# Sun-Sir/BSARec

Measured on AMD Instinct MI355X. Metric: train sequences/sec, ML-1M L=50 d=64 2-layer, higher is better.
Workload: dtype f32

## Files before the change

bsarec_amd/_lib.py:

```python
import ctypes as C
import os

HERE = os.path.dirname(os.path.abspath(__file__))
LIB_PATH = os.environ.get("BSAREC_LIB") or os.path.join(HERE, "libbsarec_hip.so")
MAX_LAYERS = 16
ABI_VERSION = 10
TOPK_MAX = 1024
NEG_MAX = 1024
NEG_MAX_DRAWS = 1 << 20
TRAIN_NEG_MAX = 8192
TRAIN_NEG_SITE = 0x4E454753

(BUF_LAYER_OUT, BUF_LOGITS, BUF_LOSS, BUF_DSP, BUF_HMIX, BUF_PROBS, BUF_DLAYER_IN, BUF_LOSS_ROWS, BUF_CTX,
 BUF_DLOGITS, BUF_TRAIN_CAND, BUF_TRAIN_CORR, BUF_TRAIN_LOGITS, BUF_TRAIN_DLOGITS) = range(14)
K_NONE, K_FFN1, K_FFN2, K_QKV, K_LOGITS, K_DU, K_DW1, K_FUSED_FWD, K_FUSED_BWD = range(9)

LAYER_FIELDS = ["sqrt_beta", "filter_ln_w", "filter_ln_b", "query_w", "query_b", "key_w", "key_b", "value_w", "value_b",
                "dense_w", "dense_b", "attn_ln_w", "attn_ln_b", "ffn1_w", "ffn1_b", "ffn2_w", "ffn2_b", "ffn_ln_w",
                "ffn_ln_b"]
LAYER_KEYS = {
    "sqrt_beta": "layer.filter_layer.sqrt_beta",
    "filter_ln_w": "layer.filter_layer.LayerNorm.weight", "filter_ln_b": "layer.filter_layer.LayerNorm.bias",
    "query_w": "layer.attention_layer.query.weight", "query_b": "layer.attention_layer.query.bias",
    "key_w": "layer.attention_layer.key.weight", "key_b": "layer.attention_layer.key.bias",
    "value_w": "layer.attention_layer.value.weight", "value_b": "layer.attention_layer.value.bias",
    "dense_w": "layer.attention_layer.dense.weight", "dense_b": "layer.attention_layer.dense.bias",
    "attn_ln_w": "layer.attention_layer.LayerNorm.weight", "attn_ln_b": "layer.attention_layer.LayerNorm.bias",
    "ffn1_w": "feed_forward.dense_1.weight", "ffn1_b": "feed_forward.dense_1.bias",
    "ffn2_w": "feed_forward.dense_2.weight", "ffn2_b": "feed_forward.dense_2.bias",
    "ffn_ln_w": "feed_forward.LayerNorm.weight", "ffn_ln_b": "feed_forward.LayerNorm.bias",
}
OPTIONAL_LAYER_KEYS = {"filter_cw": "layer.filter_layer.complex_weight"}
TOP_KEYS = {"item_emb": "item_embeddings.weight", "pos_emb": "position_embeddings.weight",
            "ln_w": "LayerNorm.weight", "ln_b": "LayerNorm.bias"}


class Config(C.Structure):
    _fields_ = [("batch", C.c_int), ("seq_len", C.c_int), ("hidden", C.c_int), ("heads", C.c_int), ("layers", C.c_int),
                ("item_size", C.c_int), ("cutoff_bins", C.c_int), ("alpha", C.c_float), ("ln_eps", C.c_float),
                ("p_hidden", C.c_float), ("p_attn", C.c_float), ("filter_kind", C.c_int),
                ("hidden_act", C.c_int), ("storage", C.c_int), ("no_fused", C.c_int), ("no_prune_top", C.c_int),
                ("dw_tiled", C.c_int), ("splits", C.c_int), ("top_slabs", C.c_int), ("separate_embed", C.c_int),
                ("separate_top", C.c_int), ("chain_kernels", C.c_int), ("x3_products", C.c_int),
                ("train_negatives", C.c_int), ("train_sampler", C.c_int), ("train_no_logq", C.c_int),
                ("train_lazy_adam", C.c_int),
                ("weight_image", C.c_int)]


TRAIN_FIELDS = ("train_negatives", "train_sampler", "train_no_logq")
TRAIN_SAMPLERS = {"uniform": 0, "popularity": 1}


OPTION_FIELDS = ("storage", "no_fused", "no_prune_top", "dw_tiled", "splits", "top_slabs", "separate_embed", "separate_top", "chain_kernels", "x3_products",
                 "weight_image")
HIDDEN_ACTS = {"gelu": 0, "relu": 1, "swish": 2, "tanh": 3, "sigmoid": 4}

_defaults = {k: 0 for k in OPTION_FIELDS}
_defaults["weight_image"] = 1


def _env_defaults():
    e = os.environ
    d = {}
    if e.get("BSAREC_DW") == "tiled":
        d["dw_tiled"] = 1
    if e.get("BSAREC_PRUNE_TOP") == "0":
        d["no_prune_top"] = 1
    if e.get("BSAREC_EMBED_IN_BLOCK") == "0":
        d["separate_embed"] = 1
    if e.get("BSAREC_TOP_TAIL") == "0":
        d["separate_top"] = 1
    if e.get("BSAREC_FUSED") == "0":
        d["no_fused"] = 1
    if e.get("BSAREC_BLOCK_KERNELS") == "chain":
        d["chain_kernels"] = 1
    if e.get("BSAREC_PRODUCTS") == "bf16x3":
        d["x3_products"] = 1
    for env, key, hi in (("BSAREC_TOP_SLABS", "top_slabs", 16), ("BSAREC_SPLITS", "splits", 1024)):
        if e.get(env, "").isdigit() and 1 <= int(e[env]) <= hi:
            d[key] = int(e[env])
    if e.get("BSAREC_STORAGE") == "bf16":
        d["storage"] = 1
    if e.get("BSAREC_WEIGHT_IMAGE") == "0":
        d["weight_image"] = 0
    return d


def set_default_options(**kw):
    old = {}
    for k, v in kw.items():
        if k not in _defaults:
            raise KeyError(k)
        old[k] = _defaults[k]
        _defaults[k] = int(v)
    return old


def default_options():
    d = dict(_defaults)
    d.update(_env_defaults())
    return d


class Layer(C.Structure):
    _fields_ = [(f, C.c_void_p) for f in LAYER_FIELDS] + [("filter_cw", C.c_void_p)]


class Tensors(C.Structure):
    _fields_ = [("item_emb", C.c_void_p), ("pos_emb", C.c_void_p), ("ln_w", C.c_void_p), ("ln_b", C.c_void_p),
                ("layer", Layer * MAX_LAYERS)]


class Adam(C.Structure):
    _fields_ = [("params", C.c_void_p), ("grads", C.c_void_p), ("exp_avg", C.c_void_p), ("exp_avg_sq", C.c_void_p),
                ("n", C.c_long), ("lr", C.c_float), ("beta1", C.c_float), ("beta2", C.c_float), ("eps", C.c_float),
                ("weight_decay", C.c_float), ("grad_scale", C.c_float), ("shadow_bf16", C.c_void_p), ("shadow_from", C.c_long),
                ("grads2", C.c_void_p), ("grads2_n", C.c_long), ("n_grad_srcs", C.c_int), ("grad_srcs", C.c_void_p * 8),
                ("wimage_plan", C.c_void_p)]


class Comm(C.Structure):
    _fields_ = [("rank", C.c_int), ("world", C.c_int), ("flags", C.c_void_p * 8), ("epoch", C.c_void_p),
                ("error", C.c_void_p), ("timeout_ms", C.c_int)]


HOOK = C.CFUNCTYPE(None, C.c_void_p, C.c_void_p)


EXPORTS = {
    "bsarec_abi_version": (C.c_int, []),
    "bsarec_workspace_bytes": (C.c_size_t, [C.POINTER(Config)]),
    "bsarec_plan_create": (C.c_int, [C.POINTER(C.c_void_p), C.POINTER(Config), C.POINTER(Tensors), C.POINTER(Tensors),
                                     C.POINTER(Tensors), C.c_void_p, C.c_size_t, C.c_void_p, C.c_void_p, C.c_void_p]),
    "bsarec_shadow_refresh": (C.c_int, [C.c_void_p, C.c_void_p]),
    "bsarec_wimage_refresh": (C.c_int, [C.c_void_p, C.c_void_p]),
    "bsarec_wimage_floats": (C.c_long, [C.POINTER(Config)]),
    "bsarec_wimage_offset": (C.c_long, [C.c_int] * 5),
    "bsarec_plan_set_dense_grad_hook": (C.c_int, [C.c_void_p, HOOK, C.c_void_p, C.c_void_p]),
    "bsarec_plan_set_train_sampler": (C.c_int, [C.c_void_p, C.c_void_p]),
    "bsarec_buffer_is_bf16": (C.c_int, [C.c_void_p, C.c_int, C.c_int]),
    "bsarec_plan_is_fused": (C.c_int, [C.c_void_p]),
    "bsarec_config_is_fused": (C.c_int, [C.c_void_p]),
    "bsarec_plan_destroy": (None, [C.c_void_p]),
    "bsarec_buffer_offset": (C.c_long, [C.c_void_p, C.c_int, C.c_int]),
    "bsarec_step_begin": (C.c_int, [C.c_void_p, C.c_void_p]),
    "bsarec_forward": (C.c_int, [C.c_void_p, C.c_void_p, C.c_int, C.c_void_p]),
    "bsarec_forward_last": (C.c_int, [C.c_void_p, C.c_void_p, C.c_int, C.c_void_p]),
    "bsarec_loss": (C.c_int, [C.c_void_p, C.c_void_p, C.c_void_p]),
    "bsarec_loss_bce": (C.c_int, [C.c_void_p, C.c_void_p, C.c_void_p, C.c_void_p]),
    "bsarec_loss_logsig": (C.c_int, [C.c_void_p, C.c_void_p, C.c_void_p, C.c_void_p]),
    "bsarec_logits": (C.c_int, [C.c_void_p, C.c_void_p]),
    "bsarec_backward": (C.c_int, [C.c_void_p, C.c_void_p]),
    "bsarec_backward_seq": (C.c_int, [C.c_void_p, C.c_void_p, C.c_void_p]),
    "bsarec_backward_seq_multi": (C.c_int, [C.c_void_p, C.c_void_p, C.c_void_p]),
    "bsarec_adam_step": (C.c_int, [C.POINTER(Adam), C.c_void_p, C.c_void_p]),
    "bsarec_train_step": (C.c_int, [C.c_void_p, C.c_void_p, C.c_void_p, C.POINTER(Adam), C.c_void_p]),
    "bsarec_gather_batch": (C.c_int, [C.c_void_p, C.c_void_p, C.c_void_p, C.c_long, C.c_void_p, C.c_int, C.c_int,
                                      C.c_void_p, C.c_void_p, C.c_void_p]),
    "bsarec_train_step_indexed": (C.c_int, [C.c_void_p] * 4 + [C.c_long] + [C.c_void_p] * 3 + [C.POINTER(Adam), C.c_void_p]),
    "bsarec_grad_step_indexed": (C.c_int, [C.c_void_p] * 4 + [C.c_long] + [C.c_void_p] * 3 + [C.c_float] * 3 + [C.c_void_p]),
    "bsarec_adam_apply": (C.c_int, [C.POINTER(Adam), C.c_void_p, C.c_void_p]),
    "bsarec_mask_seen": (C.c_int, [C.c_void_p, C.c_long, C.c_int, C.c_void_p, C.c_void_p, C.c_void_p, C.c_void_p]),
    "bsarec_topk_seen": (C.c_int, [C.c_void_p, C.c_long, C.c_int, C.c_int, C.c_void_p, C.c_void_p, C.c_void_p, C.c_int, C.c_void_p,
                                   C.c_void_p, C.c_void_p]),
    "bsarec_sampled_rank": (C.c_int, [C.c_void_p, C.c_long, C.c_void_p, C.c_int, C.c_int, C.c_int] + [C.c_void_p] * 5 +
                            [C.c_int, C.c_uint64, C.c_uint32] + [C.c_void_p] * 4),
    "bsarec_topk_full_workspace_bytes": (C.c_long, [C.c_int] * 5),
    "bsarec_topk_full": (C.c_int, [C.c_void_p, C.c_long, C.c_void_p, C.c_int, C.c_int, C.c_int] + [C.c_void_p] * 3 +
                         [C.c_int, C.c_int, C.c_void_p, C.c_long, C.c_void_p, C.c_void_p, C.c_void_p]),
    "bsarec_topk_full_range": (C.c_int, [C.c_void_p, C.c_long, C.c_void_p, C.c_int, C.c_int, C.c_long, C.c_int] + [C.c_void_p] * 3 +
                               [C.c_int, C.c_int, C.c_void_p, C.c_long, C.c_void_p, C.c_void_p, C.c_void_p]),
    "bsarec_answer_rank": (C.c_int, [C.c_void_p, C.c_long, C.c_void_p, C.c_int, C.c_int, C.c_int] + [C.c_void_p] * 7),
    "bsarec_answer_rank_range": (C.c_int, [C.c_void_p, C.c_long, C.c_void_p, C.c_int, C.c_int, C.c_long, C.c_int] +
                                 [C.c_void_p] * 8),
    "bsarec_answer_score_range": (C.c_int, [C.c_void_p, C.c_long, C.c_void_p, C.c_int, C.c_int, C.c_long, C.c_int] +
                                  [C.c_void_p] * 6),
    "bsarec_info_nce_workspace_bytes": (C.c_long, [C.c_int] * 3),
    "bsarec_info_nce_fwd": (C.c_int, [C.c_void_p, C.c_long, C.c_void_p, C.c_long, C.c_int, C.c_int, C.c_float, C.c_int,
                                      C.c_void_p, C.c_void_p, C.c_void_p, C.c_long, C.c_void_p]),
    "bsarec_info_nce_bwd": (C.c_int, [C.c_void_p, C.c_long, C.c_void_p, C.c_long, C.c_int, C.c_int, C.c_float, C.c_int,
                                      C.c_void_p, C.c_void_p, C.c_long, C.c_void_p, C.c_void_p, C.c_void_p]),
    "bsarec_freq_layer_fwd": (C.c_int, [C.c_void_p] * 5 + [C.c_int] * 4 + [C.c_float, C.c_float, C.c_void_p, C.c_int,
                                                                          C.c_void_p, C.c_void_p, C.c_void_p, C.c_void_p]),
    "bsarec_freq_layer_bwd_scratch_floats": (C.c_long, [C.c_int, C.c_int, C.c_int]),
    "bsarec_freq_layer_bwd": (C.c_int, [C.c_void_p] * 7 + [C.c_int] * 4 + [C.c_float, C.c_void_p, C.c_int] +
                              [C.c_void_p] * 6),
    "bsarec_profile_select": (C.c_int, [C.c_void_p, C.c_int]),
    "bsarec_debug_stamps": (C.c_int, [C.c_void_p, C.c_void_p]),
    "bsarec_profile_read": (C.c_int, [C.c_void_p, C.POINTER(C.c_double), C.POINTER(C.c_int)]),
    "bsarec_profile_event_overhead": (C.c_int, [C.c_void_p, C.c_int, C.POINTER(C.c_double)]),
}

COMM_EXPORTS = {
    "bsarec_comm_alloc": (C.c_int, [C.POINTER(C.c_void_p), C.c_size_t, C.c_int]),
    "bsarec_comm_free": (C.c_int, [C.c_void_p]),
    "bsarec_comm_export": (C.c_int, [C.c_void_p, C.c_char_p]),
    "bsarec_comm_import": (C.c_int, [C.c_char_p, C.POINTER(C.c_void_p)]),
    "bsarec_comm_release": (C.c_int, [C.c_void_p]),
    "bsarec_comm_barrier": (C.c_int, [C.POINTER(Comm), C.c_void_p]),
}

PTRS8 = C.c_void_p * 8
SHARD_EXPORTS = {
    "bsarec_shard_gather_rows": (C.c_int, [C.c_void_p, C.c_long, C.POINTER(PTRS8), C.c_int, C.c_long, C.c_long, C.c_int,
                                           C.c_void_p, C.c_void_p, C.c_void_p]),
    "bsarec_shard_logits": (C.c_int, [C.c_void_p, C.c_long, C.c_int, C.c_void_p, C.c_int, C.c_int, C.c_void_p, C.c_long,
                                      C.c_void_p]),
    "bsarec_shard_ce_stats": (C.c_int, [C.c_void_p, C.c_long, C.c_int, C.c_int, C.c_void_p, C.c_long, C.c_long, C.c_void_p,
                                        C.c_void_p]),
    "bsarec_shard_ce_grad": (C.c_int, [C.c_void_p, C.c_long, C.c_int, C.c_int, C.c_void_p, C.c_long, C.c_long, C.c_void_p,
                                       C.c_int, C.c_void_p, C.c_void_p, C.c_void_p]),
    "bsarec_shard_head_bwd_scratch_floats": (C.c_long, [C.c_int, C.c_int, C.c_int]),
    "bsarec_shard_head_bwd": (C.c_int, [C.c_void_p, C.c_long, C.c_int, C.c_int, C.c_void_p, C.c_long, C.c_void_p, C.c_int,
                                        C.c_void_p, C.c_void_p, C.c_void_p, C.c_void_p]),
    "bsarec_shard_scatter_rows": (C.c_int, [C.c_void_p, C.c_long, C.c_int, C.POINTER(PTRS8), C.c_long, C.c_long, C.c_long,
                                            C.c_int, C.c_void_p, C.c_void_p]),
    "bsarec_shard_ssm_draw": (C.c_int, [C.c_uint64, C.c_void_p, C.c_int, C.c_long, C.c_void_p, C.c_int, C.c_void_p, C.c_void_p,
                                        C.c_void_p, C.c_void_p]),
    "bsarec_shard_ssm_gather": (C.c_int, [C.c_void_p, C.c_int, C.c_void_p, C.c_int, C.POINTER(PTRS8), C.c_int, C.c_long, C.c_long,
                                          C.c_int, C.c_void_p, C.c_void_p]),
    "bsarec_shard_ssm_head": (C.c_int, [C.c_void_p, C.c_long, C.c_int, C.c_int, C.c_void_p, C.c_void_p, C.c_void_p, C.c_void_p,
                                        C.c_int, C.c_long, C.c_void_p, C.c_int, C.c_int, C.c_void_p, C.c_void_p, C.c_void_p,
                                        C.c_void_p]),
    "bsarec_shard_ssm_loss": (C.c_int, [C.c_void_p, C.c_int, C.c_void_p, C.c_void_p]),
    "bsarec_shard_ssm_bwd_scratch_floats": (C.c_long, [C.c_int, C.c_int, C.c_int]),
    "bsarec_shard_ssm_bwd": (C.c_int, [C.c_void_p, C.c_int, C.c_int, C.c_void_p, C.c_long, C.c_void_p, C.c_int, C.c_void_p,
                                       C.c_long, C.c_void_p, C.c_void_p, C.c_void_p]),
    "bsarec_shard_ssm_pull": (C.c_int, [C.c_void_p, C.c_int, C.c_int, C.c_void_p, C.c_int, C.POINTER(PTRS8), C.c_long, C.c_long,
                                        C.c_long, C.c_int, C.c_void_p, C.c_void_p]),
    "bsarec_shard_lazy_mark": (C.c_int, [C.c_void_p, C.c_long, C.c_void_p, C.c_int, C.c_void_p, C.c_int, C.c_long, C.c_long,
                                         C.c_long, C.c_void_p, C.c_void_p, C.c_void_p, C.c_int, C.c_void_p]),
    "bsarec_shard_lazy_adam": (C.c_int, [C.c_void_p, C.c_void_p, C.c_void_p, C.c_void_p, C.c_int, C.c_float, C.c_float, C.c_float,
                                         C.c_float, C.c_void_p, C.c_void_p, C.c_void_p, C.c_int, C.c_void_p, C.c_void_p]),
}

_lib = None


def source_sha16() -> str:
    import hashlib
    h = hashlib.sha256()
    src = os.path.join(HERE, "csrc")
    for f in sorted(os.listdir(src)) + [os.path.join(os.path.dirname(HERE), "include", "bsarec_hip.h"),
                                         os.path.join(HERE, "build.py")]:
        with open(f if os.path.isabs(f) else os.path.join(src, f), "rb") as fh:
            h.update(fh.read())
    return h.hexdigest()[:16]


def load():
    global _lib
    if _lib is not None:
        return _lib
    if not os.path.exists(LIB_PATH):
        raise RuntimeError(
            f"{LIB_PATH} is missing: build it with `python -m bsarec_amd.build` (hipcc, gfx950). "
            "bsarec_amd has no fallback path.")
    lib = C.CDLL(LIB_PATH)
    for name, (res, args) in list(EXPORTS.items()) + list(COMM_EXPORTS.items()) + list(SHARD_EXPORTS.items()):
        fn = getattr(lib, name)
        fn.restype = res
        fn.argtypes = args
    if lib.bsarec_abi_version() != ABI_VERSION:
        raise RuntimeError("libbsarec_hip.so ABI version mismatch: rebuild with `python -m bsarec_amd.build --force`")
    _lib = lib
    return lib


def check(rc, what):
    if rc != 0:
        kind = "invalid argument / unsupported shape" if rc < 0 else "hipError_t"
        raise RuntimeError(f"{what} failed: {kind} {rc}")
```

bsarec_amd/csrc/bsarec_hip.hip:

```cpp
#include <cmath>
#include "../../include/bsarec_hip.h"
#include "../../include/bsarec_shard.h"
#include "epilogues.h"
#include "kernels.h"
#include "fused_layer.h"
#include "dw_direct.h"
#include "fused_top.h"
#include "fused_chain.h"
#include "comm.h"
#include "catalogue_shard.h"
#include "rank.h"
#include "sampled_rank.h"
#include "full_rank.h"
#include "answer_rank.h"
#include "info_nce.h"
#include "sampled_softmax.h"
#include "lazy_adam.h"

#include <hip/hip_runtime.h>
#include <math.h>
#include <stdio.h>
#include <stdlib.h>
#include <string.h>
#include <vector>
#include <algorithm>

#define HIPCHK(x) do { hipError_t e_ = (x); if (e_ != hipSuccess) return (int)e_; } while (0)
#define RET(x) do { int r_ = (x); if (r_ != 0) return r_; } while (0)

static thread_local bool g_dry = false;
#define LAUNCH(...) do { if (!g_dry) hipLaunchKernelGGL(__VA_ARGS__); } while (0)

struct bsarec_plan;
static thread_local bsarec_plan* t_plan = nullptr;

static inline int cdiv(long a, long b) { return (int)((a + b - 1) / b); }
static inline long rup(long a, long b) { return (a + b - 1) / b * b; }

struct ProfState {
    int kclass = BSAREC_K_NONE;
    std::vector<std::pair<hipEvent_t, hipEvent_t>> events;
    size_t used = 0;
    ~ProfState() { for (auto& e : events) { (void)hipEventDestroy(e.first); (void)hipEventDestroy(e.second); } }
};

struct LayerBufs {
    float *dsp, *xhat_f, *rstd_f, *q, *k, *v, *probs, *ctx, *xhat_a, *rstd_a, *hmix, *u, *xhat_ff, *rstd_ff;
    float* gp;
};

struct bsarec_plan {
    bsarec_config_t cfg;
    bsarec_tensors_t P, G, S;
    bool bf;
    bool bf_products;
    char* ws; size_t ws_bytes;
    uint64_t* state;
    const float* twiddle;
    int T, Lp, Vp, dh, nblk, rows_pb, nsplit, kchunk, vsplit, vchunk;
    bool fused;
    bool train;
    int* ids32;
    float* X[BSAREC_MAX_LAYERS + 1];
    float *xhat0, *rstd0;
    LayerBufs lb[BSAREC_MAX_LAYERS];
    float *logits, *dlogits, *loss_rows, *loss;
    float *dXa, *dXb, *dz, *dT, *dU, *dH, *dXacc, *dO, *dF, *dC, *dS, *dq, *dk, *dv, *dXtmp, *dlast_slab;
    float *slab_wL[BSAREC_MAX_LAYERS], *slab_bL[BSAREC_MAX_LAYERS], *part_lnL[BSAREC_MAX_LAYERS], *part_betaL[BSAREC_MAX_LAYERS];
    float *part_ln0, *part_pos, *trash;
    int pos_slices;
    ReduceJob* jobs; int jobs_per_layer;
    ReduceJob* jobs_pruned;
    bool prune_ok;
    bool pruned;
    int loss_kind;
    const float* ext_dy = nullptr;
    const float* ext_mid[BSAREC_MAX_LAYERS] = {};
    const int64_t *bce_pos, *bce_neg;
    float *part_kvb, *slab_dummy;
    float* part_cwL[BSAREC_MAX_LAYERS];
    float *top_dq, *top_dO, *top_dT, *top_dU, *top_ak, *top_rk, *top_av, *top_rv;
    int* blockmap; int red_blocks;
    long red_elems; const float *red_lo, *red_hi;
    int top_slabs; bool embed_in_block, direct_dw;
    bool scatter_in_block;
    ProfState prof;
    long long* stamps = nullptr;
    bsarec_hook_t dense_hook = nullptr; void* dense_hook_user = nullptr;
    float* lookup_grad = nullptr;
    unsigned long long* lookup_acc = nullptr;
    int* ssm_cand = nullptr; float *ssm_corr = nullptr, *ssm_logits = nullptr, *ssm_dlogits = nullptr;
    const int64_t* pop_cum = nullptr;
    const int64_t* ssm_answers = nullptr;
    int ssm_nslab = 0;
    LazyRows lazy = {};
    bool lazy_now = false;
    float* wimg = nullptr;
};
struct PlanScope {
    bsarec_plan* prev;
    explicit PlanScope(bsarec_plan* p) : prev(t_plan) { t_plan = p; }
    ~PlanScope() { t_plan = prev; }
};

struct ProfScope {
    hipStream_t s; bool on; hipEvent_t stop;
    ProfScope(int kclass, hipStream_t st) : s(st), on(false) {
        ProfState* ps = t_plan ? &t_plan->prof : nullptr;
        on = ps && kclass != BSAREC_K_NONE && kclass == ps->kclass;
        if (!on) return;
        if (ps->used == ps->events.size()) {
            hipEvent_t a, b;
            (void)hipEventCreate(&a); (void)hipEventCreate(&b);
            ps->events.push_back({a, b});
        }
        (void)hipEventRecord(ps->events[ps->used].first, s);
        stop = ps->events[ps->used].second;
        ++ps->used;
    }
    ~ProfScope() { if (on) (void)hipEventRecord(stop, s); }
};

template <auto Kernel, class... A>
static int launch_lds(dim3 grid, dim3 block, size_t smem, hipStream_t s, const A&... a) {
    static size_t raised = 0;
    if (smem > 48 * 1024 && smem > raised) {
        HIPCHK(hipFuncSetAttribute(reinterpret_cast<const void*>(Kernel), hipFuncAttributeMaxDynamicSharedMemorySize, (int)smem));
        raised = smem;
    }
    if (g_dry) return 0;
    hipLaunchKernelGGL(Kernel, grid, block, smem, s, a...);
    return (int)hipGetLastError();
}

static GemmP gemm_defaults(int M, int N, int K) {
    GemmP P;
    memset(&P, 0, sizeof(P));
    P.M = M; P.N = N; P.K = K; P.Nb = N; P.Kv = K;
    P.nseg = 1; P.nprob = 1; P.nsplit = 1; P.kchunk = K; P.nh = 1;
    return P;
}

template <int BM, int BN, int WM, int WN, bool AKM, bool BKM, int AXF, int BXF, bool BG, bool BF, class Epi>
static int launch_gemm_as(const GemmP& P, const XformP& X, const Epi& epi, float* bgrad, int nbatch, hipStream_t s, int kclass) {
    if (P.M <= 0 || P.N <= 0) return 0;
    const dim3 grid(cdiv(P.M, BM), cdiv(P.N, BN), nbatch * P.nprob * P.nsplit);
    ProfScope prof(g_dry ? BSAREC_K_NONE : kclass, s);
    return launch_lds<gemm_kernel<BM, BN, WM, WN, AKM, BKM, AXF, BXF, BG, BF, Epi>>(grid, dim3(64 * WM * WN),
                                                                                  GemmSmem<BM, BN, AKM, BKM, BF>::BYTES, s, P, X, epi, bgrad);
}

template <int BM, int BN, int WM, int WN, bool AKM, bool BKM, int AXF, int BXF, bool BG, class Epi>
static int launch_gemm(const GemmP& P, const XformP& X, const Epi& epi, float* bgrad, int nbatch, hipStream_t s,
                       int kclass = BSAREC_K_NONE, bool fp32_only = false) {
    if (!fp32_only && t_plan && t_plan->bf_products) {
        if constexpr (BM == 64 && BN == 64 && !BG)
            if (P.M >= 8192 && P.N >= 128 && nbatch == 1)
                return launch_gemm_as<128, 128, WM, WN, AKM, BKM, AXF, BXF, BG, true, Epi>(P, X, epi, bgrad, nbatch, s, kclass);
        return launch_gemm_as<BM, BN, WM, WN, AKM, BKM, AXF, BXF, BG, true, Epi>(P, X, epi, bgrad, nbatch, s, kclass);
    }
    if constexpr (BN == 256 && WM * WN == 4)
        return launch_gemm_as<BM, BN, 2, 4, AKM, BKM, AXF, BXF, BG, false, Epi>(P, X, epi, bgrad, nbatch, s, kclass);
    else
        return launch_gemm_as<BM, BN, WM, WN, AKM, BKM, AXF, BXF, BG, false, Epi>(P, X, epi, bgrad, nbatch, s, kclass);
}

static XformP no_xform() { XformP X; memset(&X, 0, sizeof(X)); return X; }

template <bool BIAS, bool ADD, bool GGRAD>
static EpiLinear<BIAS, ADD, GGRAD> epi_linear(float* C, long ldc) {
    EpiLinear<BIAS, ADD, GGRAD> e;
    memset(&e, 0, sizeof(e));
    e.C[0] = C; e.ldc = ldc;
    return e;
}

struct Carver {
    char* base; size_t off;
    explicit Carver(char* b) : base(b), off(0) {}
    template <class T> T* take(size_t n) {
        T* p = base ? reinterpret_cast<T*>(base + off) : nullptr;
        off += rup((long)(n * sizeof(T)), 256);
        return p;
    }
};

static int check_cfg(const bsarec_config_t& c) {
    if (c.batch < 1 || c.seq_len < 1 || c.seq_len > 256) return -1;
    if (c.hidden < 4 || c.hidden > 256 || c.hidden % 4) return -2;
    if (c.heads < 1 || c.hidden % c.heads || (c.hidden / c.heads) % 4) return -3;
    if (c.layers < 1 || c.layers > BSAREC_MAX_LAYERS) return -4;
    if (c.item_size < 2) return -5;
    if (c.cutoff_bins < 1 || c.cutoff_bins > c.seq_len / 2 + 1) return -6;
    if ((long)c.cutoff_bins * c.hidden > 8192) return -7;
    if (c.p_hidden < 0.f || c.p_hidden >= 1.f || c.p_attn < 0.f || c.p_attn >= 1.f) return -8;
    if (c.filter_kind != 0 && c.filter_kind != 1) return -9;
    if (c.filter_kind == 1 && c.cutoff_bins != c.seq_len / 2 + 1) return -9;
    if (c.hidden_act < 0 || c.hidden_act > 4) return -14;
    if (c.storage < 0 || c.storage > 1) return -15;
    if (c.splits < 0 || c.splits > 1024 || c.top_slabs < 0 || c.top_slabs > 16) return -16;
    if (c.train_negatives < 0 || c.train_negatives > BSAREC_TRAIN_NEG_MAX) return -17;
    if (c.train_sampler < 0 || c.train_sampler > 1 || c.train_no_logq < 0 || c.train_no_logq > 1) return -17;
    if (c.train_negatives > 0 && c.storage != 0) return -18;
    if (c.train_lazy_adam < 0 || c.train_lazy_adam > 1 || (c.train_lazy_adam && c.train_negatives == 0)) return -19;
    if (c.weight_image < 0 || c.weight_image > 1) return -20;
    return 0;
}

static bool fused_shape_ok(const bsarec_config_t& c);
static bool wimage_wanted(const bsarec_config_t& c) {
    return c.weight_image && fused_shape_ok(c) && c.storage == 0 && !c.x3_products && !c.chain_kernels && c.filter_kind == 0;
}

static bool fused_shape_ok(const bsarec_config_t& c) {
    const int dh = c.hidden / c.heads;
    if (c.no_fused || c.hidden_act != 0 || c.hidden != 64 || c.seq_len > 64 || !(dh == 16 || dh == 32 || dh == 64)) return false;
    if (c.filter_kind == 1) return c.storage == 0 && c.alpha == 1.0f && c.cutoff_bins <= 36;
    return c.cutoff_bins <= FUSED_MAX_CB;
}

#define SSM_SLAB_MAX 32
static void ssm_split(int N, int cap, int* nslab, int* chunk) {
    const int want = std::max(1, std::min(cap, N / 256));
    *chunk = (int)rup(cdiv(N, want), SSM_KS);
    *nslab = cdiv(N, *chunk);
}

static void derive(bsarec_plan& p) {
    const bsarec_config_t& c = p.cfg;
    p.fused = fused_shape_ok(c);
    p.bf = c.storage == 1 && p.fused;
    p.bf_products = c.storage == 1 && !p.fused;
    p.T = c.batch * c.seq_len;
    p.Lp = (int)rup(c.seq_len, 4);
    p.Vp = (int)rup(c.item_size, 4);
    p.dh = c.hidden / c.heads;
    p.nblk = p.fused ? c.batch : cdiv(p.T, 64);
    p.rows_pb = p.fused ? c.seq_len : 64;
    const int want_splits = c.splits > 0 ? c.splits : (p.fused ? 32 : 40);
    p.top_slabs = c.top_slabs > 0 ? c.top_slabs : 2;
    p.embed_in_block = !c.separate_embed || p.bf;
    p.direct_dw = !c.dw_tiled && (long)p.T * 4 * c.hidden * 4 < (1L << 31);
    p.scatter_in_block = p.fused && p.direct_dw && !c.separate_embed;
    long ch = rup(cdiv(p.T, want_splits), p.bf ? 2 * GEMM_BK : GEMM_BK);
    if (ch < 64) ch = 64;
    if (ch > 2048) ch = 2048;
    p.kchunk = (int)ch;
    p.nsplit = cdiv(p.T, p.kchunk);
    long vc = rup(cdiv(p.Vp, p.fused ? 32 : 16), GEMM_BK);
    if (vc < 64) vc = 64;
    p.vchunk = (int)vc;
    p.vsplit = cdiv(p.Vp, p.vchunk);
    int chunk;
    if (c.train_negatives > 0) ssm_split(c.train_negatives, std::min(p.vsplit, SSM_SLAB_MAX), &p.ssm_nslab, &chunk);
}

static void carve(bsarec_plan& p, char* base, size_t* total) {
    const bsarec_config_t& c = p.cfg;
    const long T = p.T, d = c.hidden, B = c.batch, L = c.seq_len, h = c.heads, N = c.layers;
    const long Td = T * d;
    Carver cv(base);
    p.jobs = cv.take<ReduceJob>((size_t)(N * 20 + 3));
    p.jobs_pruned = cv.take<ReduceJob>((size_t)(N * 20 + 3));
    p.blockmap = cv.take<int>((size_t)(N * (12 * cdiv(d * d, 64) + 16 * cdiv(4 * d, 64) + cdiv((long)c.cutoff_bins * d * 2, 64)) +
                                       cdiv(L * d, 64) + 2 * cdiv(d, 64) + 64));
    p.ids32 = cv.take<int>(T);
    for (int l = 0; l <= N; ++l) p.X[l] = cv.take<float>(Td);
    p.xhat0 = cv.take<float>(Td); p.rstd0 = cv.take<float>(T);
    for (int l = 0; l < N; ++l) {
        LayerBufs& b = p.lb[l];
        b.dsp = cv.take<float>(Td); b.xhat_f = cv.take<float>(Td); b.rstd_f = cv.take<float>(T);
        b.q = cv.take<float>(Td); b.k = cv.take<float>(Td); b.v = cv.take<float>(Td);
        b.probs = cv.take<float>(B * h * L * p.Lp); b.ctx = cv.take<float>(Td);
        b.xhat_a = cv.take<float>(Td); b.rstd_a = cv.take<float>(T); b.hmix = cv.take<float>(Td);
        b.u = cv.take<float>(4 * Td); b.xhat_ff = cv.take<float>(Td); b.rstd_ff = cv.take<float>(T);
        b.gp = p.fused ? cv.take<float>(4 * Td) : nullptr;
    }
    p.logits = cv.take<float>(B * p.Vp); p.dlogits = cv.take<float>(B * p.Vp);
    p.loss_rows = cv.take<float>(B); p.loss = cv.take<float>(4);
    p.dXa = cv.take<float>(Td); p.dXb = cv.take<float>(Td); p.dz = cv.take<float>(Td); p.dT = cv.take<float>(Td);
    p.dU = cv.take<float>(4 * Td); p.dH = cv.take<float>(Td); p.dXacc = cv.take<float>(Td); p.dO = cv.take<float>(Td);
    p.dF = cv.take<float>(Td); p.dC = cv.take<float>(Td); p.dS = cv.take<float>(B * h * L * p.Lp);
    p.dq = cv.take<float>(Td); p.dk = cv.take<float>(Td); p.dv = cv.take<float>(Td); p.dXtmp = cv.take<float>(Td);
    p.dlast_slab = cv.take<float>((long)p.vsplit * B * d);
    for (int l = 0; l < N; ++l) {
        p.slab_wL[l] = cv.take<float>((long)p.nsplit * 12 * d * d);
        p.slab_bL[l] = cv.take<float>((long)p.nsplit * 9 * d);
        p.part_lnL[l] = cv.take<float>((long)p.nblk * 6 * d);
        p.part_betaL[l] = cv.take<float>(B * d);
    }
    p.part_ln0 = cv.take<float>((long)p.nblk * 2 * d);
    p.pos_slices = cdiv(B, 64);
    p.part_pos = cv.take<float>((long)p.pos_slices * L * d);
    p.trash = cv.take<float>(1024);
    p.lookup_acc = cv.take<unsigned long long>((long)c.item_size * d);
    p.part_kvb = cv.take<float>(2 * B * d);
    for (int l = 0; l < N; ++l) p.part_cwL[l] = c.filter_kind == 1 ? cv.take<float>(B * c.cutoff_bins * d * 2) : nullptr;
    p.top_dq = cv.take<float>(B * d); p.top_dO = cv.take<float>(B * d); p.top_dT = cv.take<float>(B * d);
    p.top_dU = cv.take<float>(4 * B * d);
    p.top_ak = cv.take<float>(B * h * d); p.top_rk = cv.take<float>(B * h * d);
    p.top_av = cv.take<float>(B * h * d); p.top_rv = cv.take<float>(B * h * d);
    p.slab_dummy = cv.take<float>((long)p.nsplit * 4 * d);
    if (c.train_negatives > 0) {
        const long Nn = c.train_negatives;
        p.ssm_cand = cv.take<int>(Nn); p.ssm_corr = cv.take<float>(Nn);
        p.ssm_logits = cv.take<float>(B * (Nn + 1)); p.ssm_dlogits = cv.take<float>(B * (Nn + 1));
    }
    if (c.train_lazy_adam) {
        p.lazy.cap = (int)std::min<long>(c.item_size, T + B + c.train_negatives);
        p.lazy.d4 = (int)(d / 4);
        p.lazy.mark = cv.take<int>(c.item_size); p.lazy.rows = cv.take<int>(p.lazy.cap); p.lazy.count = cv.take<int>(1);
    }
    *total = cv.off;
}

extern "C" int bsarec_abi_version(void) { return BSAREC_ABI_VERSION; }

extern "C" size_t bsarec_workspace_bytes(const bsarec_config_t* cfg) {
    if (!cfg || check_cfg(*cfg) != 0) return 0;
    bsarec_plan p;
    p.cfg = *cfg;
    derive(p);
    size_t total = 0;
    carve(p, nullptr, &total);
    return total;
}

struct SlabMap { long wq, wk, wv, wo, w1, w2, wtot, bq, bk, bv, bo, b1, b2, btot; };
static SlabMap slab_map(long d) {
    SlabMap m;
    m.wq = 0; m.wk = d * d; m.wv = 2 * d * d; m.wo = 3 * d * d; m.w1 = 4 * d * d; m.w2 = 8 * d * d; m.wtot = 12 * d * d;
    m.bq = 0; m.bk = d; m.bv = 2 * d; m.bo = 3 * d; m.b1 = 4 * d; m.b2 = 8 * d; m.btot = 9 * d;
    return m;
}

static float* slab_w_ptr(const bsarec_plan& p, int l, long tensor_off) { return p.slab_wL[l] + tensor_off * p.nsplit; }
static float* slab_b_ptr(const bsarec_plan& p, int l, long tensor_off) { return p.slab_bL[l] + tensor_off * p.nsplit; }

enum LnPart { LN_FF_G, LN_FF_B, LN_A_G, LN_A_B, LN_F_G, LN_F_B };
enum Ln0Part { LN_E_G, LN_E_B };
static float* ln_part(const bsarec_plan& p, int l, LnPart k) { return p.part_lnL[l] + (long)k * p.nblk * p.cfg.hidden; }
static float* ln0_part(const bsarec_plan& p, Ln0Part k) { return p.part_ln0 + (long)k * p.nblk * p.cfg.hidden; }

static const float* h_last(const bsarec_plan& p) { return p.X[p.cfg.layers] + (long)(p.cfg.seq_len - 1) * p.cfg.hidden; }
static long h_last_stride(const bsarec_plan& p) { return (long)p.cfg.seq_len * p.cfg.hidden; }

static float* wimage_weight(const bsarec_plan& p, int l, int which, bool transposed) {
    const long d = p.cfg.hidden;
    return p.wimg + l * wimage_layer_floats(d) + (transposed ? 12 * d * d : 0) + wimage_weight_off(which, d);
}
static bsarec_layer_t wimage_layer(const bsarec_plan& p, int l, bool transposed) {
    bsarec_layer_t w;
    memset(&w, 0, sizeof(w));
    w.query_w = wimage_weight(p, l, WIMAGE_WQ, transposed); w.key_w = wimage_weight(p, l, WIMAGE_WK, transposed);
    w.value_w = wimage_weight(p, l, WIMAGE_WV, transposed); w.dense_w = wimage_weight(p, l, WIMAGE_WO, transposed);
    w.ffn1_w = wimage_weight(p, l, WIMAGE_W1, transposed); w.ffn2_w = wimage_weight(p, l, WIMAGE_W2, transposed);
    return w;
}

extern "C" int bsarec_plan_create(bsarec_plan_t** out, const bsarec_config_t* cfg, const bsarec_tensors_t* params,
                                  const bsarec_tensors_t* grads, const bsarec_tensors_t* shadow, void* workspace,
                                  size_t workspace_bytes, void* state, const float* twiddle, void* stream) {
    if (!out || !cfg || !params || !workspace || !state || !twiddle) return -10;
    RET(check_cfg(*cfg));
    if (cfg->storage == 1 && fused_shape_ok(*cfg) && !shadow) return -15;
    if (wimage_wanted(*cfg) && (!shadow || !shadow->layer[0].query_w || ((uintptr_t)shadow->layer[0].query_w & 255))) return -15;
    if (((uintptr_t)workspace & 255) != 0) return -11;
    bsarec_plan* p = new bsarec_plan();
    p->cfg = *cfg;
    p->P = *params;
    if (grads) p->G = *grads; else memset(&p->G, 0, sizeof(p->G));
    if (shadow) p->S = *shadow; else memset(&p->S, 0, sizeof(p->S));
    p->ws = (char*)workspace; p->ws_bytes = workspace_bytes;
    p->state = (uint64_t*)state; p->twiddle = twiddle; p->train = false;
    p->wimg = wimage_wanted(*cfg) ? shadow->layer[0].query_w : nullptr;
    derive(*p);
    size_t total = 0;
    carve(*p, p->ws, &total);
    if (total > workspace_bytes) { delete p; return -12; }
    if (hipMemset(p->lookup_acc, 0, (size_t)cfg->item_size * cfg->hidden * sizeof(unsigned long long)) != hipSuccess) {
        delete p; return -12;
    }
    if (cfg->train_lazy_adam && (hipMemset(p->lazy.mark, 0, (size_t)cfg->item_size * sizeof(int)) != hipSuccess ||
                                 hipMemset(p->lazy.count, 0, sizeof(int)) != hipSuccess)) {
        delete p; return -12;
    }

    const long d = cfg->hidden;
    const SlabMap sm = slab_map(d);
    std::vector<ReduceJob> jobs;
    auto add = [&](const float* src, float* dst, int nsplit, long len) {
        ReduceJob j; j.src = src; j.dst = dst; j.nsplit = nsplit; j.len = (int)len; j.stride = len; j.scale = 1.f; j.pad = 0;
        jobs.push_back(j);
    };
    const int ns = p->nsplit, nb = p->nblk;
    auto add_w = [&](int l, int which, const float* src, float* dst) {
        add(src, dst, ns, (which >= WIMAGE_W1 ? 4 : 1) * d * d);
        if (!p->wimg) return;
        ReduceJob& j = jobs.back();
        j.img_f = wimage_weight(*p, l, which, false); j.img_t = wimage_weight(*p, l, which, true);
        j.wn = (int)(which == WIMAGE_W1 ? 4 * d : d); j.wk = (int)(which == WIMAGE_W2 ? 4 * d : d);
    };
    for (int l = 0; l < cfg->layers; ++l) {
        const bsarec_layer_t& g = p->G.layer[l];
        add(p->part_betaL[l], g.sqrt_beta, cfg->batch, d);
        add(ln_part(*p, l, LN_F_G), g.filter_ln_w, nb, d);
        add(ln_part(*p, l, LN_F_B), g.filter_ln_b, nb, d);
        add_w(l, WIMAGE_WQ, slab_w_ptr(*p, l, sm.wq), g.query_w); add(slab_b_ptr(*p, l, sm.bq), g.query_b, ns, d);
        add_w(l, WIMAGE_WK, slab_w_ptr(*p, l, sm.wk), g.key_w);   add(slab_b_ptr(*p, l, sm.bk), g.key_b, ns, d);
        add_w(l, WIMAGE_WV, slab_w_ptr(*p, l, sm.wv), g.value_w); add(slab_b_ptr(*p, l, sm.bv), g.value_b, ns, d);
        add_w(l, WIMAGE_WO, slab_w_ptr(*p, l, sm.wo), g.dense_w); add(slab_b_ptr(*p, l, sm.bo), g.dense_b, ns, d);
        add(ln_part(*p, l, LN_A_G), g.attn_ln_w, nb, d);
        add(ln_part(*p, l, LN_A_B), g.attn_ln_b, nb, d);
        add_w(l, WIMAGE_W1, slab_w_ptr(*p, l, sm.w1), g.ffn1_w); add(slab_b_ptr(*p, l, sm.b1), g.ffn1_b, ns, 4 * d);
        add_w(l, WIMAGE_W2, slab_w_ptr(*p, l, sm.w2), g.ffn2_w); add(slab_b_ptr(*p, l, sm.b2), g.ffn2_b, ns, d);
        add(ln_part(*p, l, LN_FF_G), g.ffn_ln_w, nb, d);
        add(ln_part(*p, l, LN_FF_B), g.ffn_ln_b, nb, d);
    }
    add(ln0_part(*p, LN_E_G), p->G.ln_w, nb, d);
    add(ln0_part(*p, LN_E_B), p->G.ln_b, nb, d);
    if (p->scatter_in_block) {
        ReduceJob j; j.src = p->dz; j.dst = p->G.pos_emb; j.nsplit = cfg->batch; j.len = (int)((long)cfg->seq_len * d);
        j.stride = (long)cfg->seq_len * d; j.scale = 1.f; j.pad = 0;
        jobs.push_back(j);
    } else add(p->part_pos, p->G.pos_emb, p->pos_slices, (long)cfg->seq_len * d);
    if (cfg->filter_kind == 1)
        for (int l = 0; l < cfg->layers; ++l)
            add(p->part_cwL[l], p->G.layer[l].filter_cw, cfg->batch, (long)cfg->cutoff_bins * d * 2);
    p->jobs_per_layer = 19;
    p->prune_ok = p->fused && cfg->layers >= 2 && !cfg->no_prune_top && cfg->filter_kind == 0;
    p->pruned = false;
    p->loss_kind = 0; p->bce_pos = nullptr; p->bce_neg = nullptr;
    std::vector<ReduceJob> jobs_pr = jobs;
    {
        const size_t base = (size_t)(cfg->layers - 1) * 19;
        ReduceJob& jk = jobs_pr[base + 6]; jk.src = p->part_kvb; jk.nsplit = cfg->batch; jk.stride = d;
        ReduceJob& jv = jobs_pr[base + 8]; jv.src = p->part_kvb + (long)cfg->batch * d; jv.nsplit = cfg->batch; jv.stride = d;
        for (int j : {3, 4, 5, 7, 9, 10, 13, 14, 15, 16})
            jobs_pr[base + j].nsplit = std::min(p->top_slabs, ns);
    }
    std::vector<int> bmap;
    for (size_t j = 0; j < jobs.size(); ++j)
        for (int ch = 0; ch < cdiv(jobs[j].len, 64); ++ch) bmap.push_back((int)(j << 16) | ch);
    p->red_blocks = (int)bmap.size();
    p->red_elems = 0; p->red_lo = nullptr; p->red_hi = nullptr;
    for (const ReduceJob& j : jobs) {
        p->red_elems += j.len;
        if (!p->red_lo || j.dst < p->red_lo) p->red_lo = j.dst;
        if (!p->red_hi || j.dst + j.len > p->red_hi) p->red_hi = j.dst + j.len;
    }
    hipError_t e = hipMemcpyAsync(p->jobs, jobs.data(), jobs.size() * sizeof(ReduceJob), hipMemcpyHostToDevice,
                                  (hipStream_t)stream);
    if (e == hipSuccess) e = hipMemcpyAsync(p->blockmap, bmap.data(), bmap.size() * sizeof(int), hipMemcpyHostToDevice,
                                            (hipStream_t)stream);
    if (e == hipSuccess) e = hipMemcpyAsync(p->jobs_pruned, jobs_pr.data(), jobs_pr.size() * sizeof(ReduceJob),
                                            hipMemcpyHostToDevice, (hipStream_t)stream);
    if (e == hipSuccess) e = hipStreamSynchronize((hipStream_t)stream);
    if (e != hipSuccess) { delete p; return (int)e; }
    g_dry = true;
    int rc = 0;
    for (int last = 0; last < 2 && rc == 0; ++last) {
        rc = last ? bsarec_forward_last(p, reinterpret_cast<const int64_t*>(p->ws), 1, stream)
                  : bsarec_forward(p, reinterpret_cast<const int64_t*>(p->ws), 1, stream);
        if (rc == 0) rc = bsarec_loss(p, reinterpret_cast<const int64_t*>(p->ws), stream);
        if (rc == 0 && p->G.item_emb) rc = bsarec_backward(p, stream);
    }
    g_dry = false;
    p->pruned = false;
    p->train = false;
    if (rc != 0) { delete p; return rc; }
    *out = p;
    return 0;
}

extern "C" void bsarec_plan_destroy(bsarec_plan_t* plan) { delete plan; }

extern "C" long bsarec_buffer_offset(const bsarec_plan_t* p, int buffer, int layer) {
    if (!p) return -1;
    const int N = p->cfg.layers;
    const void* ptr = nullptr;
    if (buffer >= BSAREC_BUF_TRAIN_CAND && p->cfg.train_negatives == 0) return -1;
    switch (buffer) {
        case BSAREC_BUF_LAYER_OUT: if (layer < 0 || layer > N) return -1; ptr = p->X[layer]; break;
        case BSAREC_BUF_LOGITS: ptr = p->logits; break;
        case BSAREC_BUF_DLOGITS: ptr = p->dlogits; break;
        case BSAREC_BUF_LOSS: ptr = p->loss; break;
        case BSAREC_BUF_LOSS_ROWS: ptr = p->loss_rows; break;
        case BSAREC_BUF_DSP: if (layer < 0 || layer >= N) return -1; ptr = p->lb[layer].dsp; break;
        case BSAREC_BUF_HMIX: if (layer < 0 || layer >= N) return -1; ptr = p->lb[layer].hmix; break;
        case BSAREC_BUF_PROBS: if (layer < 0 || layer >= N) return -1; ptr = p->lb[layer].probs; break;
        case BSAREC_BUF_CTX: if (layer < 0 || layer >= N) return -1; ptr = p->lb[layer].ctx; break;
        case BSAREC_BUF_DLAYER_IN: if (layer < 0 || layer > N) return -1; ptr = (layer & 1) ? p->dXb : p->dXa; break;
        case BSAREC_BUF_TRAIN_CAND: ptr = p->ssm_cand; break;
        case BSAREC_BUF_TRAIN_CORR: ptr = p->ssm_corr; break;
        case BSAREC_BUF_TRAIN_LOGITS: ptr = p->ssm_logits; break;
        case BSAREC_BUF_TRAIN_DLOGITS: ptr = p->ssm_dlogits; break;
        default: return -1;
    }
    return (long)((const char*)ptr - p->ws);
}

extern "C" int bsarec_plan_set_dense_grad_hook(bsarec_plan_t* p, bsarec_hook_t hook, void* user, float* lookup_grad) {
    if (!p) return -10;
    if (p->cfg.train_negatives > 0 && (hook || lookup_grad)) return -22;
    p->dense_hook = hook; p->dense_hook_user = user; p->lookup_grad = lookup_grad;
    return 0;
}

extern "C" int bsarec_plan_set_train_sampler(bsarec_plan_t* p, const int64_t* pop_cum) {
    if (!p) return -10;
    if (p->cfg.train_negatives == 0 || p->cfg.train_sampler != 1) return -22;
    p->pop_cum = pop_cum;
    return 0;
}

static int sampled_refusal(const bsarec_plan& p) {
    if (p.cfg.train_negatives == 0) return 0;
    if (p.dense_hook || p.lookup_grad) return -22;
    if (p.cfg.train_sampler == 1 && !p.pop_cum && !g_dry) return -23;
    return 0;
}

static int head_nsplit(const bsarec_plan& p) { return p.loss_kind == 1 ? 1 : (p.loss_kind == 2 ? p.ssm_nslab : p.vsplit); }

extern "C" int bsarec_plan_is_fused(const bsarec_plan_t* p) { return p && p->fused ? 1 : 0; }
extern "C" int bsarec_config_is_fused(const bsarec_config_t* cfg) {
    if (!cfg) return -10;
    RET(check_cfg(*cfg));
    return fused_shape_ok(*cfg) ? 1 : 0;
}

extern "C" int bsarec_buffer_is_bf16(const bsarec_plan_t* p, int buffer, int layer) {
    if (!p || !p->bf) return 0;
    switch (buffer) {
        case BSAREC_BUF_LAYER_OUT: return layer < p->cfg.layers ? 1 : 0;
        case BSAREC_BUF_HMIX: case BSAREC_BUF_PROBS: case BSAREC_BUF_CTX: return 1;
        case BSAREC_BUF_DLAYER_IN: return 1;
        default: return 0;
    }
}

extern "C" int bsarec_wimage_refresh(bsarec_plan_t* p, void* stream) {
    if (!p) return -10;
    if (!p->wimg) return 0;
    WImageP W;
    memset(&W, 0, sizeof(W));
    for (int l = 0; l < p->cfg.layers; ++l) {
        const bsarec_layer_t& w = p->P.layer[l];
        const float* src[WIMAGE_NW] = {w.query_w, w.key_w, w.value_w, w.dense_w, w.ffn1_w, w.ffn2_w};
        for (int i = 0; i < WIMAGE_NW; ++i) W.w[l][i] = src[i];
    }
    W.img = p->wimg; W.d = p->cfg.hidden;
    LAUNCH(wimage_refresh_kernel, dim3(cdiv(12L * W.d * W.d, ROW_THREADS), p->cfg.layers), dim3(ROW_THREADS), 0, (hipStream_t)stream, W);
    return g_dry ? 0 : (int)hipGetLastError();
}

extern "C" long bsarec_wimage_floats(const bsarec_config_t* cfg) {
    if (!cfg || check_cfg(*cfg) != 0) return -10;
    return wimage_wanted(*cfg) ? cfg->layers * wimage_layer_floats(cfg->hidden) : 0;
}

extern "C" long bsarec_wimage_offset(int which, int transposed, int d, int n, int k) {
    if (which < 0 || which >= WIMAGE_NW || d < 32 || d % 32 || transposed < 0 || transposed > 1) return -1;
    const int wn = which == WIMAGE_W1 ? 4 * d : d, wk = which == WIMAGE_W2 ? 4 * d : d;
    if (n < 0 || n >= wn || k < 0 || k >= wk) return -1;
    return (transposed ? 12L * d * d : 0) + wimage_weight_off(which, d) + (transposed ? wimage_off(k, n, wn) : wimage_off(n, k, wk));
}

extern "C" int bsarec_shadow_refresh(bsarec_plan_t* p, void* stream) {
    if (!p) return -10;
    if (!p->bf) return 0;
    const long d = p->cfg.hidden;
    for (int l = 0; l < p->cfg.layers; ++l) {
        const bsarec_layer_t& w = p->P.layer[l];
        const bsarec_layer_t& sh = p->S.layer[l];
        CastJobs6 J;
        const float* src[6] = {w.query_w, w.key_w, w.value_w, w.dense_w, w.ffn1_w, w.ffn2_w};
        float* dst[6] = {sh.query_w, sh.key_w, sh.value_w, sh.dense_w, sh.ffn1_w, sh.ffn2_w};
        for (int i = 0; i < 6; ++i) { J.src[i] = src[i]; J.dst[i] = (unsigned short*)dst[i]; J.n4[i] = (i < 4 ? d * d : 4 * d * d) / 4; }
        hipLaunchKernelGGL(cast_bf16_kernel, dim3(cdiv(4 * d * d / 4, ROW_THREADS), 6), dim3(ROW_THREADS), 0, (hipStream_t)stream, J);
        HIPCHK(hipGetLastError());
    }
    return 0;
}

static uint32_t drop_thresh(float p) {
    double t = (double)p * 4294967296.0;
    if (t <= 0) return 0;
    if (t >= 4294967295.0) return 0xFFFFFFFFu;
    return (uint32_t)t;
}
static DropP make_drop(const bsarec_plan& p, float prob, int site, bool train) {
    DropP d;
    d.thresh = train ? drop_thresh(prob) : 0;
    d.scale = (train && prob > 0.f) ? (float)(1.0 / (1.0 - (double)prob)) : 1.0f;
    d.rng = p.state; d.site = (uint32_t)site;
    return d;
}
static int lpr_for(int d) { return d <= 64 ? 16 : (d <= 128 ? 32 : 64); }

#define DISPATCH_LPR(d, ...) \
    do { switch (lpr_for(d)) { case 16: { constexpr int LPR = 16; __VA_ARGS__; } break; \
                               case 32: { constexpr int LPR = 32; __VA_ARGS__; } break; \
                               default: { constexpr int LPR = 64; __VA_ARGS__; } break; } } while (0)

#define DISPATCH_BN(n, ...) \
    do { if ((n) <= 64) { constexpr int BN = 64; __VA_ARGS__; } \
         else if ((n) <= 128) { constexpr int BN = 128; __VA_ARGS__; } \
         else { constexpr int BN = 256; __VA_ARGS__; } } while (0)

static size_t freq_smem(int L, int d, int cb, int nsrc, int kc = FREQ_KC) {
    return (size_t)(rup(2 * L, 4) + (long)nsrc * cb * 2 * d + (long)nsrc * kc * 2048) * 4;
}
#define LDS_BYTES_MAX 163840

template <int LPR>
static int launch_freq_fwd(const float* X, const float* sb, const float* g, const float* be, float eps, DropP drop,
                           const float* tw, int B, int L, int d, int cb, float* dsp, float* xhat, float* rstd, hipStream_t s,
                           const float* cw = nullptr) {
    return launch_lds<freq_fwd_kernel<LPR>>(dim3(B), dim3(ROW_THREADS), freq_smem(L, d, cb, 1), s, X, sb, g, be, eps, drop, tw, L, d,
                                            cb, dsp, xhat, rstd, cw);
}

template <int LPR>
static int launch_freq_bwd(const float* X, const float* dF, const float* dXin, const float* sb, const float* tw, int B, int L,
                           int d, int cb, float* dX, float* pbeta, hipStream_t s, const float* cw = nullptr, float* pcw = nullptr) {
    if (freq_smem(L, d, cb, 2) > LDS_BYTES_MAX)
        return launch_lds<freq_bwd_kernel<LPR, 1>>(dim3(B), dim3(ROW_THREADS), freq_smem(L, d, cb, 2, 1), s, X, dF, dXin, sb, tw, L, d, cb,
                                                   dX, pbeta, cw, pcw);
    return launch_lds<freq_bwd_kernel<LPR>>(dim3(B), dim3(ROW_THREADS), freq_smem(L, d, cb, 2), s, X, dF, dXin, sb, tw, L, d, cb, dX,
                                            pbeta, cw, pcw);
}

static bool dw_problem_ok(const DwProblem& q) {
    if (!q.A || !q.B || !q.slab) return false;
    if (q.K < 1 || q.M < 1 || q.N < 1 || q.kchunk < 8 || (q.kchunk & 7) || q.nslab < 1) return false;
    if (q.lda < q.M || q.ldb < q.N) return false;
    const long esz = q.bf16 ? 2 : 4;
    if (((long)(q.K - 1) * q.lda + q.M) * esz >= (1L << 31) || ((long)(q.K - 1) * q.ldb + q.N) * esz >= (1L << 31)) return false;
    return true;
}
static bool dh_problem_ok(const DhP& h) {
    if (!h.A || !h.E || !h.slab) return false;
    if (h.B < 1 || h.V < 1 || h.kchunk < 8 || (h.kchunk & 7) || h.nsplit < 1 || h.lda < h.V) return false;
    if ((long)h.B * h.lda * 4 >= (1L << 31) || (long)h.V * 256 >= (1L << 31)) return false;
    return true;
}

#define DISPATCH_DH(dh, ...) \
    do { switch (dh) { case 16: { constexpr int DH = 16; __VA_ARGS__; } break; \
                       case 32: { constexpr int DH = 32; __VA_ARGS__; } break; \
                       default: { constexpr int DH = 64; __VA_ARGS__; } break; } } while (0)
#define DISPATCH_BLOCK(p, ...) \
    do { if ((p).bf) { constexpr bool BF = true, X3 = false; DISPATCH_DH((p).dh, __VA_ARGS__); } \
         else if ((p).cfg.x3_products) { constexpr bool BF = false, X3 = true; DISPATCH_DH((p).dh, __VA_ARGS__); } \
         else { constexpr bool BF = false, X3 = false; DISPATCH_DH((p).dh, __VA_ARGS__); } } while (0)

template <bool FWD, class BlockP>
static void fill_block(const bsarec_plan& p, int l, bool tr, const bsarec_layer_t& wm, BlockP& F) {
    const bsarec_config_t& c = p.cfg;
    const bsarec_layer_t& w = p.P.layer[l];
    const LayerBufs& b = p.lb[l];
    memset(&F, 0, sizeof(F));
    F.X = p.X[l];
    F.sqrt_beta = w.sqrt_beta; F.f_g = w.filter_ln_w; F.wq = wm.query_w; F.wk = wm.key_w; F.wv = wm.value_w; F.wo = wm.dense_w;
    F.a_g = w.attn_ln_w; F.w1 = wm.ffn1_w; F.w2 = wm.ffn2_w; F.ff_g = w.ffn_ln_w; F.tw = p.twiddle;
    F.xhat_f = b.xhat_f; F.rstd_f = b.rstd_f; F.q = b.q; F.k = b.k; F.v = b.v; F.probs = b.probs;
    F.xhat_a = b.xhat_a; F.rstd_a = b.rstd_a; F.xhat_ff = b.xhat_ff; F.rstd_ff = b.rstd_ff;
    F.L = c.seq_len; F.Lp = p.Lp; F.cb = c.cutoff_bins; F.heads = c.heads;
    F.alpha = c.alpha; F.oma = (float)(1.0 - (double)c.alpha);
    F.drop_f = make_drop(p, c.p_hidden, 1 + 4 * l, tr); F.drop_p = make_drop(p, c.p_attn, 2 + 4 * l, tr);
    F.drop_o = make_drop(p, c.p_hidden, 3 + 4 * l, tr); F.drop_ff = make_drop(p, c.p_hidden, 4 + 4 * l, tr);
    F.stamps = p.stamps ? p.stamps + 32 * (2 * l + (FWD ? 0 : 1)) : nullptr;
    if constexpr (FWD) {
        F.Xout = p.X[l + 1];
        F.f_b = w.filter_ln_b; F.bq = w.query_b; F.bk = w.key_b; F.bv = w.value_b; F.bo = w.dense_b; F.a_b = w.attn_ln_b;
        F.b1 = w.ffn1_b; F.b2 = w.ffn2_b; F.ff_b = w.ffn_ln_b;
        F.ids32 = p.ids32; F.ctx = b.ctx; F.hmix = b.hmix; F.u = b.u;
        F.eps = c.ln_eps;
    }
}

template <class BlockP>
static void fill_block_partials(const bsarec_plan& p, int l, BlockP& F) {
    F.pg_ff = ln_part(p, l, LN_FF_G); F.pb_ff = ln_part(p, l, LN_FF_B); F.pg_a = ln_part(p, l, LN_A_G);
    F.pb_a = ln_part(p, l, LN_A_B); F.pg_f = ln_part(p, l, LN_F_G); F.pb_f = ln_part(p, l, LN_F_B);
    F.pbeta = p.part_betaL[l];
}

static void fill_top_fwd(bsarec_plan& p, int l, bool tr, TopFwdP& F) {
    fill_block<true>(p, l, tr, p.P.layer[l], F);
    F.low = p.lb[l].dsp;
    F.wk_sh = p.S.layer[l].key_w; F.wv_sh = p.S.layer[l].value_w;
}

static int launch_fused_fwd(bsarec_plan& p, int l, bool tr, hipStream_t s, const int64_t* ids = nullptr, const GatherP* gp = nullptr,
                            bool top_tail = false ) {
    const bsarec_config_t& c = p.cfg;
    FusedFwdP F;
    fill_block<true>(p, l, tr, p.bf ? p.S.layer[l] : p.wimg ? wimage_layer(p, l, false) : p.P.layer[l], F);
    F.xout_f32 = (l == c.layers - 1);
    F.gp = p.lb[l].gp;
    F.dsp = nullptr;
    if (l == 0 && gp) {
        F.e_E = p.P.item_emb; F.e_pos = p.P.pos_emb; F.e_g = p.P.ln_w; F.e_b = p.P.ln_b; F.e_ids = ids; F.e_gp = *gp;
        F.e_drop = make_drop(p, c.p_hidden, 0, tr); F.e_V = c.item_size;
        F.e_X0 = p.X[0]; F.e_xhat = p.xhat0; F.e_rstd = p.rstd0; F.e_ids32 = p.ids32;
    }
    F.trash = p.trash;
    TopFwdP TF;
    if (top_tail) {
        fill_top_fwd(p, l + 1, tr, TF);
        if (p.wimg) { TF.wk_sh = wimage_weight(p, l + 1, WIMAGE_WK, false); TF.wv_sh = wimage_weight(p, l + 1, WIMAGE_WV, false); }
    }
    const dim3 grid(c.batch), block(512);
    ProfScope prof(BSAREC_K_FUSED_FWD, s);
    if (c.filter_kind == 1) {
        F.filter_cw = p.P.layer[l].filter_cw;
        return launch_lds<fused_layer_fwd_kernel<32, false, NoTail, false, true>>(grid, block, fused_fwd_smem_bytes(), s, F, NoTail());
    }
    int rc = 0;
    if (!p.bf && c.chain_kernels && !c.x3_products) {
        const size_t csm = fused_chain_fwd_smem_bytes(top_tail);
        DISPATCH_DH(p.dh, rc = top_tail ? launch_lds<fused_chain_fwd_kernel<DH, TopFwdP>>(grid, block, csm, s, F, TF)
                                        : launch_lds<fused_chain_fwd_kernel<DH, NoTail>>(grid, block, csm, s, F, NoTail()));
        return rc;
    }
    const size_t smem = fused_fwd_smem_bytes();
    if (p.wimg) {
        DISPATCH_DH(p.dh, rc = top_tail ? launch_lds<fused_layer_fwd_kernel<DH, false, TopFwdP, false, false, true>>(grid, block, smem, s, F, TF)
                                        : launch_lds<fused_layer_fwd_kernel<DH, false, NoTail, false, false, true>>(grid, block, smem, s, F, NoTail()));
        return rc;
    }
    DISPATCH_BLOCK(p, rc = top_tail ? launch_lds<fused_layer_fwd_kernel<DH, BF, TopFwdP, X3>>(grid, block, smem, s, F, TF)
                                    : launch_lds<fused_layer_fwd_kernel<DH, BF, NoTail, X3>>(grid, block, smem, s, F, NoTail()));
    return rc;
}

static int launch_fused_bwd(bsarec_plan& p, int l, bool tr, const float* dY, float* dXout, hipStream_t s, bool top,
                            const TopBwdP* head = nullptr ) {
    const bsarec_config_t& c = p.cfg;
    FusedBwdP F;
    fill_block<false>(p, l, tr, p.bf ? p.S.layer[l] : p.wimg ? wimage_layer(p, l, true) : p.P.layer[l], F);
    fill_block_partials(p, l, F);
    F.dY = dY; F.dX = dXout;
    F.u = p.lb[l].gp;
    if (top) { F.dh_slabs = p.dlast_slab; F.dh_nsplit = head_nsplit(p); F.dh_stride = (long)c.batch * c.hidden; }
    if (l == 0) {
        F.e_dz = p.dz; F.e_xhat = p.xhat0; F.e_rstd = p.rstd0; F.e_g = p.P.ln_w;
        F.e_pg = ln0_part(p, LN_E_G); F.e_pb = ln0_part(p, LN_E_B); F.e_drop = make_drop(p, c.p_hidden, 0, tr);
        F.e_dx_extra = p.ext_dy ? p.ext_mid[0] : nullptr;
    }
    F.dT = p.dT; F.dU = p.dU; F.dO = p.dO; F.dq = p.dq; F.dk = p.dk; F.dv = p.dv;
    F.trash = p.trash;
    const dim3 grid(c.batch), block(512);
    const size_t smem = fused_bwd_smem_bytes();
    ProfScope prof(BSAREC_K_FUSED_BWD, s);
    if (c.filter_kind == 1) {
        F.filter_cw = p.P.layer[l].filter_cw; F.pcw = p.part_cwL[l];
        return launch_lds<fused_layer_bwd_kernel<32, false, NoTail, false, true>>(grid, block, smem, s, F, NoTail());
    }
    int rc = 0;
    if (p.wimg) {
        DISPATCH_DH(p.dh, rc = head ? launch_lds<fused_layer_bwd_kernel<DH, false, TopBwdP, false, false, true>>(grid, block, smem, s, F, *head)
                                    : launch_lds<fused_layer_bwd_kernel<DH, false, NoTail, false, false, true>>(grid, block, smem, s, F, NoTail()));
        return rc;
    }
    DISPATCH_BLOCK(p, rc = head ? launch_lds<fused_layer_bwd_kernel<DH, BF, TopBwdP, X3>>(grid, block, smem, s, F, *head)
                                : launch_lds<fused_layer_bwd_kernel<DH, BF, NoTail, X3>>(grid, block, smem, s, F, NoTail()));
    return rc;
}

static int launch_top_fwd(bsarec_plan& p, int l, bool tr, hipStream_t s) {
    TopFwdP F;
    fill_top_fwd(p, l, tr, F);
    int rc = 0;
    DISPATCH_BLOCK(p, rc = launch_lds<top_fwd_kernel<DH, BF>>(dim3(p.cfg.batch), dim3(256), top_fwd_smem_bytes(), s, F));
    return rc;
}

static void fill_top_bwd(bsarec_plan& p, int l, bool tr, float* dXout, TopBwdP& F) {
    const bsarec_config_t& c = p.cfg;
    fill_block<false>(p, l, tr, p.P.layer[l], F);
    fill_block_partials(p, l, F);
    F.dX = dXout;
    F.u = p.lb[l].u; F.low = p.lb[l].dsp;
    F.dh_slabs = p.dlast_slab; F.dh_nsplit = head_nsplit(p); F.dh_stride = (long)c.batch * c.hidden;
    F.dT = p.top_dT; F.dU = p.top_dU; F.dO = p.top_dO; F.dq = p.top_dq;
    F.ak = p.top_ak; F.rk = p.top_rk; F.av = p.top_av; F.rv = p.top_rv;
    F.pbk = p.part_kvb; F.pbv = p.part_kvb + (long)c.batch * c.hidden;
}

static int launch_top_bwd(bsarec_plan& p, int l, bool tr, float* dXout, hipStream_t s) {
    TopBwdP F;
    fill_top_bwd(p, l, tr, dXout, F);
    int rc = 0;
    DISPATCH_BLOCK(p, rc = launch_lds<top_bwd_kernel<DH, BF>>(dim3(p.cfg.batch), dim3(256), top_bwd_smem_bytes(), s, F));
    return rc;
}

extern "C" int bsarec_debug_stamps(bsarec_plan_t* p, void* dev_buf) { if (!p) return -10; p->stamps = (long long*)dev_buf; return 0; }

#ifdef BSAREC_DW_STAMPS
extern "C" int bsarec_debug_dw_stamps(long long* host_out, int n) {
    if (!host_out || n < 1 || n > DW_STAMP_MAX) return -10;
    HIPCHK(hipDeviceSynchronize());
    HIPCHK(hipMemcpyFromSymbol(host_out, HIP_SYMBOL(g_dw_stamps), (size_t)n * 8 * sizeof(long long)));
    return 0;
}
#endif

extern "C" int bsarec_step_begin(bsarec_plan_t* p, void* stream) {
    if (!p) return -10;
    LAUNCH(step_begin_kernel, dim3(1), dim3(1), 0, (hipStream_t)stream, p->state, (long long*)nullptr, 0);
    return (int)hipGetLastError();
}

static int forward_impl(bsarec_plan_t* p, const int64_t* ids, int train, void* stream, const GatherP& gp, bool last_only);

extern "C" int bsarec_forward(bsarec_plan_t* p, const int64_t* ids, int train, void* stream) {
    GatherP none;
    memset(&none, 0, sizeof(none));
    return forward_impl(p, ids, train, stream, none, false);
}

extern "C" int bsarec_forward_last(bsarec_plan_t* p, const int64_t* ids, int train, void* stream) {
    GatherP none;
    memset(&none, 0, sizeof(none));
    return forward_impl(p, ids, train, stream, none, true);
}

static int generic_layer_fwd(bsarec_plan& p, int l, bool tr, hipStream_t s) {
    const bsarec_config_t& c = p.cfg;
    const int T = p.T, d = c.hidden, L = c.seq_len, B = c.batch, h = c.heads, dh = p.dh, Lp = p.Lp;
    const bsarec_layer_t& w = p.P.layer[l];
    LayerBufs& b = p.lb[l];
    const float* X = p.X[l];
    const XformP nox = no_xform();
    DISPATCH_LPR(d, RET(launch_freq_fwd<LPR>(X, w.sqrt_beta, w.filter_ln_w, w.filter_ln_b, c.ln_eps,
                                             make_drop(p, c.p_hidden, 1 + 4 * l, tr), p.twiddle, B, L, d,
                                             c.cutoff_bins, b.dsp, b.xhat_f, b.rstd_f, s,
                                             c.filter_kind == 1 ? w.filter_cw : nullptr)));
    {
        GemmP g = gemm_defaults(T, d, d);
        g.nprob = 3; g.lda = d; g.ldb = d;
        g.A[0] = g.A[1] = g.A[2] = X;
        g.B[0] = w.query_w; g.B[1] = w.key_w; g.B[2] = w.value_w;
        auto e = epi_linear<true, false, false>(b.q, d);
        e.C[1] = b.k; e.C[2] = b.v;
        e.bias[0] = w.query_b; e.bias[1] = w.key_b; e.bias[2] = w.value_b;
        RET((launch_gemm<64, 64, 2, 2, false, false, XF_NONE, XF_NONE, false>(g, nox, e, nullptr, 1, s, BSAREC_K_QKV)));
    }
    {
        GemmP g = gemm_defaults(L, Lp, dh);
        g.Nb = L; g.lda = d; g.ldb = d; g.nh = h;
        g.A[0] = b.q; g.B[0] = b.k;
        g.a_sb = (long)L * d; g.a_sh = dh; g.b_sb = (long)L * d; g.b_sh = dh;
        EpiSoftmax e; e.ids = p.ids32; e.L = L; e.Lp = Lp; e.sqrt_dh = sqrtf((float)dh); e.P = b.probs;
        DISPATCH_BN(Lp, RET((launch_gemm<64, BN, 2, 2, false, false, XF_NONE, XF_NONE, false>(g, nox, e, nullptr, B * h, s))));
    }
    {
        GemmP g = gemm_defaults(L, dh, Lp);
        g.Kv = L; g.lda = Lp; g.ldb = d; g.nh = h;
        g.A[0] = b.probs; g.B[0] = b.v;
        g.a_sb = (long)h * L * Lp; g.a_sh = (long)L * Lp; g.b_sb = (long)L * d; g.b_sh = dh;
        XformP xf = nox; xf.drop = make_drop(p, c.p_attn, 2 + 4 * l, tr); xf.L = L; xf.Lp = Lp;
        auto e = epi_linear<false, false, false>(b.ctx, d);
        e.c_sb = (long)L * d; e.c_sh = dh;
        RET((launch_gemm<64, 64, 2, 2, false, true, XF_DROP, XF_NONE, false>(g, xf, e, nullptr, B * h, s)));
    }
    {
        GemmP g = gemm_defaults(T, d, d);
        g.lda = d; g.ldb = d; g.A[0] = b.ctx; g.B[0] = w.dense_w;
        EpiLN<true> e;
        e.bias = w.dense_b; e.R = X; e.drop = make_drop(p, c.p_hidden, 3 + 4 * l, tr);
        e.gamma = w.attn_ln_w; e.beta = w.attn_ln_b; e.eps = c.ln_eps;
        e.Y = b.hmix; e.xhat = b.xhat_a; e.rstd = b.rstd_a;
        e.dsp = b.dsp; e.alpha = c.alpha; e.oma = (float)(1.0 - (double)c.alpha);
        DISPATCH_BN(d, RET((launch_gemm<64, BN, 2, 2, false, false, XF_NONE, XF_NONE, false>(g, nox, e, nullptr, 1, s))));
    }
    {
        GemmP g = gemm_defaults(T, 4 * d, d);
        g.lda = d; g.ldb = d; g.A[0] = b.hmix; g.B[0] = w.ffn1_w;
        auto e = epi_linear<true, false, false>(b.u, 4 * d);
        e.bias[0] = w.ffn1_b;
        RET((launch_gemm<64, 64, 2, 2, false, false, XF_NONE, XF_NONE, false>(g, nox, e, nullptr, 1, s, BSAREC_K_FFN1)));
    }
    {
        GemmP g = gemm_defaults(T, d, 4 * d);
        g.lda = 4 * d; g.ldb = 4 * d; g.A[0] = b.u; g.B[0] = w.ffn2_w;
        EpiLN<false> e;
        e.bias = w.ffn2_b; e.R = b.hmix; e.drop = make_drop(p, c.p_hidden, 4 + 4 * l, tr);
        e.gamma = w.ffn_ln_w; e.beta = w.ffn_ln_b; e.eps = c.ln_eps;
        e.Y = p.X[l + 1]; e.xhat = b.xhat_ff; e.rstd = b.rstd_ff;
        e.dsp = nullptr; e.alpha = 0.f; e.oma = 1.f;
        XformP xa = nox; xa.act = c.hidden_act;
        DISPATCH_BN(d, RET((launch_gemm<64, BN, 2, 2, false, false, XF_GELU, XF_NONE, false>(g, xa, e, nullptr, 1, s, BSAREC_K_FFN2))));
    }
    return 0;
}

static int forward_impl(bsarec_plan_t* p, const int64_t* ids, int train, void* stream, const GatherP& gp, bool last_only) {
    if (!p || (!ids && !gp.table)) return -10;
    PlanScope scope(p);
    hipStream_t s = (hipStream_t)stream;
    const bsarec_config_t& c = p->cfg;
    const int T = p->T, d = c.hidden, L = c.seq_len;
    const bool tr = train != 0;
    p->train = tr;
    p->pruned = last_only && p->prune_ok;

    const bool embed_in_block = p->fused && p->embed_in_block;
    if (!embed_in_block)
    DISPATCH_LPR(d, {
        constexpr int RPB = ROW_THREADS / LPR;
        LAUNCH(embed_fwd_kernel<LPR>, dim3(cdiv(T, RPB)), dim3(ROW_THREADS), 0, s, ids, gp, p->P.item_emb,
                           p->P.pos_emb, p->P.ln_w, p->P.ln_b, c.ln_eps, make_drop(*p, c.p_hidden, 0, tr), T, L, d,
                           c.item_size, p->X[0], p->xhat0, p->rstd0, p->ids32);
        HIPCHK(hipGetLastError());
    });

    const bool tail = p->pruned && c.layers >= 2 && !c.separate_top;
    for (int l = 0; l < c.layers; ++l) {
        if (!p->fused) RET(generic_layer_fwd(*p, l, tr, s));
        else if (p->pruned && l == c.layers - 1) { if (!tail) RET(launch_top_fwd(*p, l, tr, s)); }
        else RET(launch_fused_fwd(*p, l, tr, s, ids, (l == 0 && embed_in_block) ? &gp : nullptr, tail && l == c.layers - 2));
    }
    return 0;
}

extern "C" int bsarec_logits(bsarec_plan_t* p, void* stream) {
    if (!p) return -10;
    PlanScope scope(p);
    hipStream_t s = (hipStream_t)stream;
    const bsarec_config_t& c = p->cfg;
    const int d = c.hidden;
    if (p->fused && d == 64 && p->Vp <= 4096 && c.batch <= 512 && !g_dry) {
        LogitsP G;
        G.H = h_last(*p); G.ldh = h_last_stride(*p); G.E = p->P.item_emb; G.C = p->logits;
        G.B = c.batch; G.V = c.item_size; G.Vp = p->Vp;
        const long units = (long)cdiv(c.batch, 32) * cdiv(p->Vp, 32);
        ProfScope prof(BSAREC_K_LOGITS, s);
        hipLaunchKernelGGL(logits_direct_kernel, dim3((unsigned)cdiv(units, 4)), dim3(256), 0, s, G);
        return (int)hipGetLastError();
    }
    GemmP g = gemm_defaults(c.batch, p->Vp, d);
    g.Nb = c.item_size; g.lda = h_last_stride(*p); g.ldb = d;
    g.A[0] = h_last(*p); g.B[0] = p->P.item_emb;
    auto e = epi_linear<false, false, false>(p->logits, p->Vp);
    return launch_gemm<64, 64, 2, 2, false, false, XF_NONE, XF_NONE, false>(g, no_xform(), e, nullptr, 1, s, BSAREC_K_LOGITS, true);
}

static SsmP ssm_params(const float* h, long ldh, int B, int Bg, const float* E, const int64_t* answers, const int* cand,
                       const float* corr, int N, long V, const int64_t* pop_cum, int logq, int d, int slab_cap) {
    SsmP P;
    memset(&P, 0, sizeof(P));
    P.H = h; P.ldh = ldh; P.E = E; P.answers = answers; P.pop_cum = pop_cum;
    P.B = B; P.V = (int)V; P.d = d; P.N = N; P.logq = logq ? 1 : 0; P.inv_b = 1.0f / (float)Bg;
    P.cand = const_cast<int*>(cand); P.corr = const_cast<float*>(corr);
    ssm_split(N, slab_cap, &P.nslab, &P.chunk);
    const int dt = cdiv(d, SSM_TILE);
    P.tilesA = cdiv(N, SSM_TILE) * dt;
    P.tilesB = P.nslab * cdiv(B, SSM_TILE) * dt;
    return P;
}

static SsmP plan_ssm_params(const bsarec_plan& p, const int64_t* answers) {
    const bsarec_config_t& c = p.cfg;
    SsmP P = ssm_params(h_last(p), h_last_stride(p), c.batch, c.batch, p.P.item_emb, answers, p.ssm_cand, p.ssm_corr,
                        c.train_negatives, c.item_size, c.train_sampler == 1 ? p.pop_cum : nullptr, !c.train_no_logq, c.hidden,
                        std::min(p.vsplit, SSM_SLAB_MAX));
    P.state = p.state; P.logits = p.ssm_logits; P.dlogits = p.ssm_dlogits; P.loss_rows = p.loss_rows;
    P.slab = p.dlast_slab; P.acc = p.lookup_acc;
    if (p.lazy_now) {
        P.lazy = p.lazy; P.ids32 = p.ids32; P.nids = p.T;
        P.tilesM = (int)std::min<long>(cdiv((long)p.T + c.batch + c.train_negatives, ROW_THREADS), 64);
    }
    return P;
}

static int loss_impl(bsarec_plan_t* p, const int64_t* answers, void* stream, bool with_mean) {
    if (!p || !answers) return -10;
    hipStream_t s = (hipStream_t)stream;
    if (p->cfg.train_negatives > 0) {
        RET(sampled_refusal(*p));
        p->loss_kind = 2; p->ssm_answers = answers;
        const SsmP P = plan_ssm_params(*p, answers);
        LAUNCH(ssm_logits_kernel<false>, dim3(cdiv(P.N, SSM_TILE), cdiv(P.B, SSM_TILE)), dim3(ROW_THREADS), 0, s, P);
        HIPCHK(hipGetLastError());
        LAUNCH(ssm_ce_kernel<false>, dim3(P.B), dim3(ROW_THREADS), 0, s, P);
        HIPCHK(hipGetLastError());
        if (with_mean) LAUNCH(loss_mean_kernel, dim3(1), dim3(ROW_THREADS), 0, s, p->loss_rows, P.B, p->loss);
        return (int)hipGetLastError();
    }
    RET(bsarec_logits(p, stream));
    p->loss_kind = 0;
    const bsarec_config_t& c = p->cfg;
    const int V = c.item_size;
    const float inv_b = 1.0f / (float)c.batch;
#define CE_VEC(N4) LAUNCH(ce_rows_vec_kernel<N4>, dim3(c.batch), dim3(ROW_THREADS), 0, s, p->logits, answers, V, p->Vp, inv_b, p->dlogits, p->loss_rows)
    if (V <= CE_MAX_PER_THREAD * ROW_THREADS || V > 24 * 4 * ROW_THREADS)
        LAUNCH(ce_rows_kernel, dim3(c.batch), dim3(ROW_THREADS), 0, s, p->logits, answers, V, p->Vp, inv_b, p->dlogits, p->loss_rows);
    else if (V <= 8 * 4 * ROW_THREADS) CE_VEC(8);
    else if (V <= 12 * 4 * ROW_THREADS) CE_VEC(12);
    else if (V <= 16 * 4 * ROW_THREADS) CE_VEC(16);
    else if (V <= 20 * 4 * ROW_THREADS) CE_VEC(20);
    else CE_VEC(24);
#undef CE_VEC
    HIPCHK(hipGetLastError());
    if (with_mean) LAUNCH(loss_mean_kernel, dim3(1), dim3(ROW_THREADS), 0, s, p->loss_rows, c.batch, p->loss);
    return (int)hipGetLastError();
}

extern "C" int bsarec_loss(bsarec_plan_t* p, const int64_t* answers, void* stream) { return loss_impl(p, answers, stream, true); }

static int loss_pair(bsarec_plan_t* p, const int64_t* pos_ids, const int64_t* neg_ids, void* stream, int logsig);

extern "C" int bsarec_loss_bce(bsarec_plan_t* p, const int64_t* pos_ids, const int64_t* neg_ids, void* stream) {
    return loss_pair(p, pos_ids, neg_ids, stream, 0);
}
extern "C" int bsarec_loss_logsig(bsarec_plan_t* p, const int64_t* pos_ids, const int64_t* neg_ids, void* stream) {
    return loss_pair(p, pos_ids, neg_ids, stream, 1);
}

static int loss_pair(bsarec_plan_t* p, const int64_t* pos_ids, const int64_t* neg_ids, void* stream, int logsig) {
    if (!p || !pos_ids || !neg_ids) return -10;
    hipStream_t s = (hipStream_t)stream;
    const bsarec_config_t& c = p->cfg;
    p->loss_kind = 1; p->bce_pos = pos_ids; p->bce_neg = neg_ids;
    LAUNCH(bce_rows_kernel, dim3(1), dim3(ROW_THREADS), 0, s, h_last(*p), h_last_stride(*p), p->P.item_emb,
           pos_ids, neg_ids, c.batch, c.hidden, c.item_size, p->dlogits, p->loss, logsig);
    return (int)hipGetLastError();
}

static int backward_impl(bsarec_plan_t* p, void* stream, const TickP& tick, const bsarec_adam_t* fuse_adam = nullptr);

extern "C" int bsarec_backward(bsarec_plan_t* p, void* stream) {
    TickP none;
    memset(&none, 0, sizeof(none));
    return backward_impl(p, stream, none);
}

extern "C" int bsarec_backward_seq(bsarec_plan_t* p, const float* d_out, void* stream) {
    if (!p || !d_out) return -10;
    if (p->pruned) return -13;
    if (p->cfg.train_negatives > 0) return -22;
    TickP none;
    memset(&none, 0, sizeof(none));
    p->ext_dy = d_out;
    const int rc = backward_impl(p, stream, none);
    p->ext_dy = nullptr;
    return rc;
}

extern "C" int bsarec_backward_seq_multi(bsarec_plan_t* p, const float* const* d_outs, void* stream) {
    if (!p || !d_outs) return -10;
    const int N = p->cfg.layers;
    if (!d_outs[N]) return -10;
    if (p->pruned) return -13;
    for (int l = 0; l < N; ++l) p->ext_mid[l] = d_outs[l];
    const int rc = bsarec_backward_seq(p, d_outs[N], stream);
    for (int l = 0; l < N; ++l) p->ext_mid[l] = nullptr;
    return rc;
}

static bool can_fuse_adam(const bsarec_plan& p, const bsarec_adam_t& a) {
    if (!p.fused || !p.direct_dw || p.loss_kind == 1) return false;
    if (a.grads2 || a.n_grad_srcs > 0 || a.grad_scale != 1.0f) return false;
    if (!p.G.item_emb || p.G.item_emb < a.grads) return false;
    const long item = (long)p.cfg.item_size * p.cfg.hidden;
    const long off = p.G.item_emb - a.grads;
    if (off < 0 || off + item > a.n || (off & 3) || (item & 3)) return false;
    return p.red_elems + item == a.n && p.red_lo >= a.grads && p.red_hi <= a.grads + a.n;
}

static int head_bwd(bsarec_plan& p, hipStream_t s) {
    const bsarec_config_t& c = p.cfg;
    const int d = c.hidden, B = c.batch;
    const float* hlast = h_last(p);
    const long ldh = h_last_stride(p);
    const XformP nox = no_xform();
    const bool direct_logits = p.fused && p.direct_dw && p.loss_kind == 0 && (long)B * p.Vp * 4 < (1L << 30) &&
                               (long)c.item_size * d * 4 < (1L << 31);
    if (p.ext_dy) {
        if (!g_dry) HIPCHK(hipMemsetAsync(p.G.item_emb, 0, (size_t)c.item_size * d * sizeof(float), s));
    } else if (p.loss_kind == 1) {
        if (!g_dry) HIPCHK(hipMemsetAsync(p.G.item_emb, 0, (size_t)c.item_size * d * sizeof(float), s));
        LAUNCH(bce_bwd_kernel, dim3(B), dim3(64), 0, s, hlast, ldh, p.P.item_emb, p.bce_pos, p.bce_neg, p.dlogits, B, d,
               c.item_size, p.dlast_slab, p.G.item_emb);
        HIPCHK(hipGetLastError());
    } else if (p.loss_kind == 2) {
        const SsmP P = plan_ssm_params(p, p.ssm_answers);
        const int tilesC = std::max(1, std::min(cdiv((long)B * d, ROW_THREADS), 64));
        LAUNCH(ssm_bwd_kernel<false>, dim3(P.tilesA + P.tilesB + tilesC + P.tilesM), dim3(ROW_THREADS), 0, s, P);
        HIPCHK(hipGetLastError());
    } else if (direct_logits) {
        DwProblem q;
        memset(&q, 0, sizeof(q));
        q.A = p.dlogits; q.B = hlast; q.lda = p.Vp; q.ldb = ldh; q.M = c.item_size; q.N = d; q.K = B;
        q.kchunk = (int)rup(B, 32); q.nslab = 1; q.slab = p.G.item_emb; q.bslab = nullptr; q.gelu = 0;
        DhP H;
        memset(&H, 0, sizeof(H));
        H.A = p.dlogits; H.lda = p.Vp; H.E = p.P.item_emb; H.B = B; H.V = c.item_size; H.kchunk = p.vchunk;
        H.nsplit = p.vsplit; H.slab = p.dlast_slab;
        const int tiles = cdiv(c.item_size, 64);
        if (!dw_problem_ok(q) || !dh_problem_ok(H)) return -21;
        const dim3 lb_grid(tiles + cdiv(cdiv(B, 32) * p.vsplit, 4));
        if (p.bf) LAUNCH(logits_bwd_direct_kernel<true>, lb_grid, dim3(256), 0, s, q, tiles, H);
        else LAUNCH(logits_bwd_direct_kernel<false>, lb_grid, dim3(256), 0, s, q, tiles, H);
        HIPCHK(hipGetLastError());
    } else {
        PairP G;
        memset(&G, 0, sizeof(G));
        G.A = gemm_defaults(c.item_size, d, B);
        G.A.lda = p.Vp; G.A.ldb = ldh; G.A.A[0] = p.dlogits; G.A.B[0] = hlast;
        G.EA = epi_linear<false, false, false>(p.G.item_emb, d);
        G.B = gemm_defaults(B, d, p.Vp);
        G.B.Kv = c.item_size; G.B.lda = p.Vp; G.B.ldb = d; G.B.A[0] = p.dlogits; G.B.B[0] = p.P.item_emb;
        G.B.nsplit = p.vsplit; G.B.kchunk = p.vchunk;
        G.EB = epi_linear<false, false, false>(p.dlast_slab, d);
        G.EB.c_split = (long)B * d;
        G.tilesA = cdiv(c.item_size, 64) * cdiv(d, 64);
        G.tilesB_m = cdiv(B, 64);
        if (d <= 64) {
            constexpr size_t smem = GemmSmem<64, 64, true, true>::BYTES > GemmSmem<64, 64, false, true>::BYTES
                                        ? GemmSmem<64, 64, true, true>::BYTES : GemmSmem<64, 64, false, true>::BYTES;
            LAUNCH(gemm_logits_bwd_kernel, dim3(G.tilesA + G.tilesB_m * p.vsplit), dim3(GEMM_THREADS), smem, s, G);
            HIPCHK(hipGetLastError());
        } else {
            RET((launch_gemm<64, 64, 2, 2, true, true, XF_NONE, XF_NONE, false>(G.A, nox, G.EA, nullptr, 1, s, BSAREC_K_NONE, true)));
            RET((launch_gemm<64, 64, 2, 2, false, true, XF_NONE, XF_NONE, false>(G.B, nox, G.EB, nullptr, 1, s, BSAREC_K_NONE, true)));
        }
    }
    return 0;
}

static int top_grad(bsarec_plan& p, float*& dY, hipStream_t s) {
    const bsarec_config_t& c = p.cfg;
    const int T = p.T, d = c.hidden;
    if (p.ext_dy) {
        if (p.bf) {
            CastJobs6 J;
            memset(&J, 0, sizeof(J));
            J.src[0] = p.ext_dy; J.dst[0] = (unsigned short*)dY; J.n4[0] = (long)T * d / 4;
            LAUNCH(cast_bf16_kernel, dim3(cdiv((long)T * d / 4, ROW_THREADS), 1), dim3(ROW_THREADS), 0, s, J);
            HIPCHK(hipGetLastError());
        } else dY = const_cast<float*>(p.ext_dy);
    } else if (!p.fused) {
        LAUNCH(dlast_kernel, dim3(cdiv((long)T * d / 4, ROW_THREADS)), dim3(ROW_THREADS), 0, s, p.dlast_slab,
               head_nsplit(p), (long)c.batch * d, T, c.seq_len, d, dY);
        HIPCHK(hipGetLastError());
    }
    return 0;
}

static int generic_layer_bwd(bsarec_plan& p, int l, const float* dY, hipStream_t s) {
    const bsarec_config_t& c = p.cfg;
    const int T = p.T, d = c.hidden, L = c.seq_len, B = c.batch, h = c.heads, dh = p.dh, Lp = p.Lp, nb = p.nblk;
    const bool tr = p.train;
    const bsarec_layer_t& w = p.P.layer[l];
    const LayerBufs& b = p.lb[l];
    const XformP nox = no_xform();
    {
        LnBranch a; memset(&a, 0, sizeof(a));
        a.xhat = b.xhat_ff; a.rstd = b.rstd_ff; a.gamma = w.ffn_ln_w; a.in_scale = 1.f;
        a.drop = make_drop(p, c.p_hidden, 4 + 4 * l, tr); a.dT = p.dT;
        a.pgamma = ln_part(p, l, LN_FF_G); a.pbeta = ln_part(p, l, LN_FF_B);
        DISPATCH_LPR(d, LAUNCH((ln_bwd_kernel<LPR, 0>), dim3(nb), dim3(ROW_THREADS), 0, s, dY, a, a, p.dz, T, d, p.rows_pb));
        HIPCHK(hipGetLastError());
    }
    {
        GemmP g = gemm_defaults(T, 4 * d, d);
        g.lda = d; g.ldb = 4 * d; g.A[0] = p.dT; g.B[0] = w.ffn2_w;
        auto e = epi_linear<false, false, true>(p.dU, 4 * d);
        e.U = b.u; e.ldu = 4 * d; e.act = c.hidden_act;
        RET((launch_gemm<64, 64, 2, 2, false, true, XF_NONE, XF_NONE, false>(g, nox, e, nullptr, 1, s, BSAREC_K_DU)));
    }
    {
        GemmP g = gemm_defaults(T, d, 4 * d);
        g.lda = 4 * d; g.ldb = d; g.A[0] = p.dU; g.B[0] = w.ffn1_w;
        auto e = epi_linear<false, true, false>(p.dH, d);
        e.R = p.dz; e.ldr = d;
        RET((launch_gemm<64, 64, 2, 2, false, true, XF_NONE, XF_NONE, false>(g, nox, e, nullptr, 1, s)));
    }
    {
        LnBranch a; memset(&a, 0, sizeof(a));
        a.xhat = b.xhat_a; a.rstd = b.rstd_a; a.gamma = w.attn_ln_w; a.in_scale = (float)(1.0 - (double)c.alpha);
        a.drop = make_drop(p, c.p_hidden, 3 + 4 * l, tr); a.dT = p.dO;
        a.pgamma = ln_part(p, l, LN_A_G); a.pbeta = ln_part(p, l, LN_A_B);
        LnBranch f; memset(&f, 0, sizeof(f));
        f.xhat = b.xhat_f; f.rstd = b.rstd_f; f.gamma = w.filter_ln_w; f.in_scale = c.alpha;
        f.drop = make_drop(p, c.p_hidden, 1 + 4 * l, tr); f.dT = p.dF;
        f.pgamma = ln_part(p, l, LN_F_G); f.pbeta = ln_part(p, l, LN_F_B);
        DISPATCH_LPR(d, LAUNCH((ln_bwd_kernel<LPR, 1>), dim3(nb), dim3(ROW_THREADS), 0, s, p.dH, a, f, p.dXacc, T, d, p.rows_pb));
        HIPCHK(hipGetLastError());
    }
    {
        GemmP g = gemm_defaults(T, d, d);
        g.lda = d; g.ldb = d; g.A[0] = p.dO; g.B[0] = w.dense_w;
        auto e = epi_linear<false, false, false>(p.dC, d);
        RET((launch_gemm<64, 64, 2, 2, false, true, XF_NONE, XF_NONE, false>(g, nox, e, nullptr, 1, s)));
    }
    XformP xfa = nox; xfa.drop = make_drop(p, c.p_attn, 2 + 4 * l, tr); xfa.L = L; xfa.Lp = Lp;
    {
        GemmP g = gemm_defaults(L, Lp, dh);
        g.Nb = L; g.lda = d; g.ldb = d; g.nh = h; g.A[0] = p.dC; g.B[0] = b.v;
        g.a_sb = (long)L * d; g.a_sh = dh; g.b_sb = (long)L * d; g.b_sh = dh;
        EpiDS e; e.P = b.probs; e.drop = xfa.drop; e.L = L; e.Lp = Lp; e.sqrt_dh = sqrtf((float)dh); e.dS = p.dS;
        DISPATCH_BN(Lp, RET((launch_gemm<64, BN, 2, 2, false, false, XF_NONE, XF_NONE, false>(g, nox, e, nullptr, B * h, s))));
    }
    {
        GemmP g = gemm_defaults(L, dh, L);
        g.lda = Lp; g.ldb = d; g.nh = h; g.A[0] = b.probs; g.B[0] = p.dC;
        g.a_sb = (long)h * L * Lp; g.a_sh = (long)L * Lp; g.b_sb = (long)L * d; g.b_sh = dh;
        auto e = epi_linear<false, false, false>(p.dv, d);
        e.c_sb = (long)L * d; e.c_sh = dh;
        RET((launch_gemm<64, 64, 2, 2, true, true, XF_DROP, XF_NONE, false>(g, xfa, e, nullptr, B * h, s)));
    }
    {
        GemmP g = gemm_defaults(L, dh, L);
        g.lda = Lp; g.ldb = d; g.nh = h; g.A[0] = p.dS; g.B[0] = b.q;
        g.a_sb = (long)h * L * Lp; g.a_sh = (long)L * Lp; g.b_sb = (long)L * d; g.b_sh = dh;
        auto e = epi_linear<false, false, false>(p.dk, d);
        e.c_sb = (long)L * d; e.c_sh = dh;
        RET((launch_gemm<64, 64, 2, 2, true, true, XF_NONE, XF_NONE, false>(g, nox, e, nullptr, B * h, s)));
    }
    {
        GemmP g = gemm_defaults(L, dh, Lp);
        g.Kv = L; g.lda = Lp; g.ldb = d; g.nh = h; g.A[0] = p.dS; g.B[0] = b.k;
        g.a_sb = (long)h * L * Lp; g.a_sh = (long)L * Lp; g.b_sb = (long)L * d; g.b_sh = dh;
        auto e = epi_linear<false, false, false>(p.dq, d);
        e.c_sb = (long)L * d; e.c_sh = dh;
        RET((launch_gemm<64, 64, 2, 2, false, true, XF_NONE, XF_NONE, false>(g, nox, e, nullptr, B * h, s)));
    }
    {
        GemmP g = gemm_defaults(T, d, d);
        g.lda = d; g.ldb = d; g.nseg = 3;
        g.A[0] = p.dq; g.A[1] = p.dk; g.A[2] = p.dv;
        g.B[0] = w.query_w; g.B[1] = w.key_w; g.B[2] = w.value_w;
        auto e = epi_linear<false, true, false>(p.dXtmp, d);
        e.R = p.dXacc; e.ldr = d;
        RET((launch_gemm<64, 64, 2, 2, false, true, XF_NONE, XF_NONE, false>(g, nox, e, nullptr, 1, s)));
    }
    return 0;
}

static int dw_tile(const bsarec_plan& p) { return (p.bf_products && p.cfg.hidden >= 128) ? 128 : 64; }

static void build_dw_problems(const bsarec_plan& p, int l, bool top_pruned, GroupedTN& G) {
    const bsarec_config_t& c = p.cfg;
    const int T = p.T, d = c.hidden, L = c.seq_len, B = c.batch, h = c.heads, N = c.layers, ns = p.nsplit;
    const SlabMap sm = slab_map(d);
    const LayerBufs& b = p.lb[l];
    const float* X = p.X[l];
    memset(&G, 0, sizeof(G));
    struct Spec { const float* A; long lda; const float* B; long ldb; int M, N; long woff, boff; int gelu; };
    const Spec sp[6] = {
        {p.dq, d, X, d, d, d, sm.wq, sm.bq, 0},        {p.dk, d, X, d, d, d, sm.wk, sm.bk, 0},
        {p.dv, d, X, d, d, d, sm.wv, sm.bv, 0},        {p.dO, d, b.ctx, d, d, d, sm.wo, sm.bo, 0},
        {p.dU, 4 * d, b.hmix, d, 4 * d, d, sm.w1, sm.b1, 0},
        {p.dT, d, b.u, 4 * d, d, 4 * d, sm.w2, sm.b2, (p.fused && !top_pruned) ? 0 : 1}};
    int tiles = 0;
    const int gts = dw_tile(p);
    const bool top = (l == N - 1) && !p.ext_dy;
    for (int i = 0; i < 6; ++i) {
        const bool last_only = top && i != 1 && i != 2;
        GemmP g = gemm_defaults(sp[i].M, sp[i].N, last_only ? B : T);
        g.lda = sp[i].lda; g.ldb = sp[i].ldb; g.A[0] = sp[i].A; g.B[0] = sp[i].B; g.nsplit = ns; g.kchunk = p.kchunk;
        if (last_only) {
            const long esz = p.bf ? 2 : 4;
            g.A[0] = (const float*)((const char*)g.A[0] + (long)(L - 1) * sp[i].lda * esz);
            g.B[0] = (const float*)((const char*)g.B[0] + (long)(L - 1) * sp[i].ldb * esz);
            g.lda *= L; g.ldb *= L;
            g.kchunk = (int)rup(cdiv(B, ns), GEMM_BK);
            if (top_pruned) {
                g.A[0] = i == 0 ? p.top_dq : i == 3 ? p.top_dO : i == 4 ? p.top_dU : p.top_dT;
                g.lda = sp[i].M;
                g.nsplit = std::min(p.top_slabs, ns); g.kchunk = (int)rup(cdiv(B, g.nsplit), GEMM_BK);
            }
        }
        const bool compact = top_pruned && (i == 1 || i == 2);
        if (compact) {
            g = gemm_defaults(d, d, B * h);
            g.A[0] = i == 1 ? p.top_ak : p.top_av; g.B[0] = i == 1 ? p.top_rk : p.top_rv; g.lda = d; g.ldb = d;
            g.nsplit = std::min(p.top_slabs, ns); g.kchunk = (int)rup(cdiv(B * h, g.nsplit), GEMM_BK);
        }
        G.P[i] = g;
        G.E[i] = epi_linear<false, false, false>(slab_w_ptr(p, l, sp[i].woff), sp[i].N);
        G.E[i].c_split = (long)sp[i].M * sp[i].N;
        G.bgrad[i] = compact ? p.slab_dummy : slab_b_ptr(p, l, sp[i].boff);
        G.tile0[i] = tiles;
        G.tiles_n[i] = cdiv(sp[i].N, gts);
        G.b_gelu[i] = sp[i].gelu;
        tiles += cdiv(sp[i].M, gts) * G.tiles_n[i];
    }
    G.tile0[6] = tiles; G.nprob = 6; G.act = c.hidden_act;
}

struct DwPending { DwP DW; int np, nu; TopBwdP top_head; bool have_head; };

static int launch_dw_direct(bsarec_plan& p, int l, bool top_pruned, const GroupedTN& G, DwPending& Q, const TickP* tick,
                            hipStream_t s) {
    const int T = p.T, ns = p.nsplit;
    for (int i = 0; i < 6; ++i) {
        const GemmP& g = G.P[i];
        DwProblem& q = Q.DW.P[Q.np];
        q.A = g.A[0]; q.B = g.B[0]; q.lda = g.lda; q.ldb = g.ldb; q.M = g.M; q.N = g.N; q.K = g.K;
        q.kchunk = g.kchunk; q.nslab = g.nsplit; q.slab = G.E[i].C[0]; q.bslab = G.bgrad[i]; q.gelu = G.b_gelu[i];
        q.bf16 = p.bf ? 1 : 0;
        for (int m0 = 0; m0 < q.M; m0 += 64)
            for (int n0 = 0; n0 < q.N; n0 += 64) Q.DW.U[Q.nu++] = DwUnit{(short)Q.np, (short)m0, (short)n0, 0};
        ++Q.np;
    }
    if (top_pruned) { Q.DW.nsmall = Q.nu; Q.DW.small_slabs = std::min(p.top_slabs, ns); }
    else {
        Q.DW.nunits = Q.nu; Q.DW.nslab = ns;
        TickP tk_here;
        memset(&tk_here, 0, sizeof(tk_here));
        if (tick) tk_here = *tick;
        ScatterP sc;
        memset(&sc, 0, sizeof(sc));
        if (p.scatter_in_block && l == 0) {
            sc.de = p.dz; sc.ids32 = p.ids32; sc.T = T; sc.dA = p.lookup_acc;
            sc.nblocks = cdiv(T, SCATTER_FLOATS / 64);
        }
        for (int i = 0; i < Q.np; ++i) if (!dw_problem_ok(Q.DW.P[i])) return -21;
        if (sc.nblocks && (!sc.de || !sc.ids32 || !sc.dA)) return -21;
        ProfScope prof(BSAREC_K_DW1, s);
        const dim3 dw_grid(8 * cdiv(ns, 8) * (Q.nu - Q.DW.nsmall) + Q.DW.nsmall * Q.DW.small_slabs + sc.nblocks + (tk_here.state ? 1 : 0));
        LAUNCH(dw_direct_kernel, dw_grid, dim3(256), 0, s, Q.DW, tk_here, sc);
        HIPCHK(hipGetLastError());
        Q.np = 0; Q.nu = 0; Q.DW.nsmall = 0; Q.DW.small_slabs = 0;
    }
    return 0;
}

static int launch_dw_grouped(const bsarec_plan& p, const GroupedTN& G, hipStream_t s) {
    ProfScope prof(BSAREC_K_DW1, s);
    const dim3 grid(G.tile0[6], p.nsplit), block(GEMM_THREADS);
    if (!p.bf_products)
        return launch_lds<gemm_grouped_tn_kernel<false, 64>>(grid, block, GemmSmem<64, 64, true, true, false>::BYTES, s, G);
    if (dw_tile(p) == 128)
        return launch_lds<gemm_grouped_tn_kernel<true, 128>>(grid, block, GemmSmem<128, 128, true, true, true>::BYTES, s, G);
    return launch_lds<gemm_grouped_tn_kernel<true, 64>>(grid, block, GemmSmem<64, 64, true, true, true>::BYTES, s, G);
}

static int embed_bwd(bsarec_plan& p, const float* dY, hipStream_t s) {
    const bsarec_config_t& c = p.cfg;
    const int T = p.T, d = c.hidden, L = c.seq_len, B = c.batch;
    if (!p.fused) {
        LnBranch a; memset(&a, 0, sizeof(a));
        a.xhat = p.xhat0; a.rstd = p.rstd0; a.gamma = p.P.ln_w; a.in_scale = 1.f;
        a.drop = make_drop(p, c.p_hidden, 0, p.train); a.dT = nullptr;
        a.pgamma = ln0_part(p, LN_E_G); a.pbeta = ln0_part(p, LN_E_B);
        DISPATCH_LPR(d, LAUNCH((ln_bwd_kernel<LPR, 2>), dim3(p.nblk), dim3(ROW_THREADS), 0, s, dY, a, a, p.dz, T, d, p.rows_pb));
        HIPCHK(hipGetLastError());
    }
    if (!p.scatter_in_block)
    DISPATCH_LPR(d, {
        constexpr int CHUNK = SCATTER_FLOATS / (LPR * 4);
        const int sb = cdiv(T, CHUNK);
        RET(launch_lds<embed_bwd_kernel<LPR>>(dim3(sb + L * p.pos_slices), dim3(ROW_THREADS), SCATTER_FLOATS * 8 + 2 * CHUNK * 4, s,
                                              p.dz, p.ids32, B, L, d, p.lookup_acc, p.part_pos, sb));
    });
    return 0;
}

static bool adam_on_masters(const bsarec_plan& p, const bsarec_adam_t& a) {
    return p.G.item_emb && a.params + (p.G.item_emb - a.grads) == p.P.item_emb;
}
static int wimage_after_adam(bsarec_plan& p, const bsarec_adam_t& a, hipStream_t s) {
    return (p.wimg && !a.wimage_plan && adam_on_masters(p, a)) ? bsarec_wimage_refresh(&p, s) : 0;
}

static int final_reduce(bsarec_plan& p, const TickP& tick, const bsarec_adam_t* fuse_adam, hipStream_t s) {
    const bsarec_config_t& c = p.cfg;
    LookupAcc la;
    memset(&la, 0, sizeof(la));
    la.acc = p.lookup_acc; la.dst = p.lookup_grad ? p.lookup_grad : p.G.item_emb; la.n4 = (long)c.item_size * c.hidden / 4;
    la.nblocks = (int)std::min<long>(cdiv(la.n4, ROW_THREADS), 1024);
    la.dense_zero = (!p.ext_dy && p.loss_kind == 2) ? 1 : 0;
    const bool lazy = p.lazy_now && !p.ext_dy && p.loss_kind == 2;
    if (lazy) {
        la.lazy = p.lazy;
        la.nblocks = (int)std::min<long>(cdiv((long)p.lazy.cap * p.lazy.d4, ROW_THREADS), 1024);
    }
    const ReduceJob* jobs = p.pruned ? p.jobs_pruned : p.jobs;
    if (fuse_adam) {
        const bsarec_adam_t& a = *fuse_adam;
        AdamFuseP A;
        memset(&A, 0, sizeof(A));
        A.w = a.params; A.g = const_cast<float*>(a.grads); A.m = a.exp_avg; A.v = a.exp_avg_sq;
        A.b1 = a.beta1; A.b2 = a.beta2; A.eps = a.eps; A.wd = a.weight_decay;
        A.shadow = (unsigned short*)a.shadow_bf16; A.shadow_from = a.shadow_bf16 ? a.shadow_from : a.n;
        A.item_off = p.G.item_emb - a.grads; A.item_n4 = la.n4; A.lookup_acc = la.acc;
        A.dense_zero = la.dense_zero;
        A.wimage = (p.wimg && adam_on_masters(p, a)) ? 1 : 0;
        if (lazy) A.lazy = p.lazy;
        int ab = lazy ? la.nblocks : cdiv(A.item_n4, ROW_THREADS);
        if (ab > 1024) ab = 1024;
        LAUNCH(reduce_adam_kernel, dim3(p.red_blocks + ab), dim3(ROW_THREADS), 0, s, jobs, p.blockmap, p.red_blocks,
               (const uint64_t*)p.state, A);
    } else
        LAUNCH(multi_reduce_flat_kernel, dim3(p.red_blocks + la.nblocks + (tick.state ? 1 : 0)), dim3(ROW_THREADS), 0, s, jobs,
               p.blockmap, p.red_blocks, tick, la);
    return (int)hipGetLastError();
}

static int backward_impl(bsarec_plan_t* p, void* stream, const TickP& tick, const bsarec_adam_t* fuse_adam) {
    if (!p) return -10;
    if (!p->G.item_emb) return -13;
    if (fuse_adam && p->lookup_grad) return -21;
    PlanScope scope(p);
    hipStream_t s = (hipStream_t)stream;
    const bsarec_config_t& c = p->cfg;
    const int T = p->T, d = c.hidden, L = c.seq_len, B = c.batch, N = c.layers;
    const bool tr = p->train;

    RET(head_bwd(*p, s));
    if (p->dense_hook && !g_dry && !p->ext_dy) p->dense_hook(p->dense_hook_user, stream);
    float* dY = (N & 1) ? p->dXb : p->dXa;
    RET(top_grad(*p, dY, s));

    DwPending pend;
    memset(&pend, 0, sizeof(pend));
    for (int l = N - 1; l >= 0; --l) {
        float* dXout = (dY == p->dXa) ? p->dXb : p->dXa;
        const bool top_pruned = p->fused && p->pruned && l == N - 1;
        if (top_pruned) {
            if (N >= 2 && !c.separate_top && p->direct_dw) { fill_top_bwd(*p, l, tr, dXout, pend.top_head); pend.have_head = true; }
            else RET(launch_top_bwd(*p, l, tr, dXout, s));
        } else if (p->fused) {
            RET(launch_fused_bwd(*p, l, tr, dY, dXout, s, l == N - 1 && !p->ext_dy,
                                 (pend.have_head && l == N - 2) ? &pend.top_head : nullptr));
        } else RET(generic_layer_bwd(*p, l, dY, s));
        GroupedTN G;
        build_dw_problems(*p, l, top_pruned, G);
        if (p->fused && p->direct_dw) RET(launch_dw_direct(*p, l, top_pruned, G, pend, (fuse_adam && l == 0) ? &tick : nullptr, s));
        else RET(launch_dw_grouped(*p, G, s));
        if (!p->fused) {
            const bsarec_layer_t& w = p->P.layer[l];
            DISPATCH_LPR(d, RET(launch_freq_bwd<LPR>(p->X[l], p->dF, p->dXtmp, w.sqrt_beta, p->twiddle, B, L, d, c.cutoff_bins,
                                                     dXout, p->part_betaL[l], s, c.filter_kind == 1 ? w.filter_cw : nullptr,
                                                     c.filter_kind == 1 ? p->part_cwL[l] : nullptr)));
        }
        dY = dXout;
        if (p->ext_dy && p->ext_mid[l] && !(p->fused && l == 0)) {
            const long n4 = (long)T * d / 4;
            LAUNCH(grad_join_kernel, dim3((unsigned)std::min<long>(cdiv(n4, ROW_THREADS), 2048)), dim3(ROW_THREADS), 0, s, dXout,
                   p->ext_mid[l], n4, p->bf ? 1 : 0);
            HIPCHK(hipGetLastError());
        }
    }
    RET(embed_bwd(*p, dY, s));
    return final_reduce(*p, tick, fuse_adam, s);
}

static TickP make_tick(void* state, int adam, float lr, float b1, float b2, const float* loss_rows, int B, float* loss_out,
                       void* cursor, int advance, int bump_step) {
    TickP t;
    memset(&t, 0, sizeof(t));
    t.state = (uint64_t*)state; t.adam = adam; t.lr = lr; t.b1 = b1; t.b2 = b2;
    t.loss_rows = loss_rows; t.B = B; t.loss_out = loss_out;
    t.cursor = (long long*)cursor; t.advance = advance; t.bump_step = bump_step;
    return t;
}

static int adam_check(const bsarec_adam_t* a) {
    if (!a || !a->params || !a->grads || !a->exp_avg || !a->exp_avg_sq || a->n <= 0 || (a->n & 3)) return -10;
    if (a->shadow_bf16 && (a->shadow_from < 0 || (a->shadow_from & 3))) return -10;
    if (a->grads2 && (a->grads2_n < 0 || a->grads2_n > a->n || (a->grads2_n & 3))) return -10;
    if (a->n_grad_srcs < 0 || a->n_grad_srcs > 8) return -10;
    for (int r = 0; r < a->n_grad_srcs; ++r) if (!a->grad_srcs[r]) return -10;
    return 0;
}

static int adam_launch(const bsarec_adam_t& a, void* state, hipStream_t s) {
    const long n4 = a.n / 4;
    int blocks = cdiv(n4, ROW_THREADS);
    if (blocks > 2048) blocks = 2048;
    GradSrcs S;
    memset(&S, 0, sizeof(S));
    S.nsrc = a.n_grad_srcs;
    for (int r = 0; r < a.n_grad_srcs; ++r) S.src[r] = a.grad_srcs[r];
    S.g2 = a.grads2; S.n2_4 = a.grads2 ? a.grads2_n / 4 : 0;
    LAUNCH(adam_kernel, dim3(blocks), dim3(ROW_THREADS), 0, s, a.params, a.grads, a.exp_avg, a.exp_avg_sq, n4,
           (const uint64_t*)state, a.beta1, a.beta2, a.eps, a.weight_decay, a.grad_scale, (unsigned short*)a.shadow_bf16,
           a.shadow_bf16 ? a.shadow_from / 4 : n4, S);
    HIPCHK(hipGetLastError());
    return a.wimage_plan ? bsarec_wimage_refresh(a.wimage_plan, s) : 0;
}

extern "C" int bsarec_adam_step(const bsarec_adam_t* a, void* state, void* stream) {
    RET(adam_check(a));
    if (!state) return -10;
    hipStream_t s = (hipStream_t)stream;
    LAUNCH(adam_tick_kernel, dim3(1), dim3(ROW_THREADS), 0, s, make_tick(state, 1, a->lr, a->beta1, a->beta2, nullptr, 0, nullptr, nullptr, 0, 0));
    HIPCHK(hipGetLastError());
    return adam_launch(*a, state, s);
}

extern "C" int bsarec_adam_apply(const bsarec_adam_t* a, void* state, void* stream) {
    RET(adam_check(a));
    if (!state) return -10;
    return adam_launch(*a, state, (hipStream_t)stream);
}

static int lazy_check(const bsarec_plan& p, const bsarec_adam_t& a) {
    if (!p.cfg.train_lazy_adam) return 0;
    if (a.grads2 || a.n_grad_srcs > 0 || a.shadow_bf16) return -24;
    const long item = (long)p.cfg.item_size * p.cfg.hidden;
    if (!p.G.item_emb || p.G.item_emb < a.grads) return -24;
    const long off = p.G.item_emb - a.grads;
    if (off + item > a.n || (off & 3)) return -24;
    return 0;
}

static int lazy_adam_launch(const bsarec_plan& p, const bsarec_adam_t& a, hipStream_t s) {
    LazyAdamP A;
    memset(&A, 0, sizeof(A));
    A.w = a.params; A.g = a.grads; A.m = a.exp_avg; A.v = a.exp_avg_sq;
    A.n = a.n; A.item_off = p.G.item_emb - a.grads; A.item_n = (long)p.cfg.item_size * p.cfg.hidden;
    A.b1 = a.beta1; A.b2 = a.beta2; A.eps = a.eps; A.wd = a.weight_decay; A.gscale = a.grad_scale;
    A.T = p.lazy;
    A.dense_blocks = (int)std::max<long>(1, std::min<long>(cdiv((A.n - A.item_n) / 4, ROW_THREADS), 2048));
    const int lb = (int)std::min<long>(cdiv((long)p.lazy.cap * p.lazy.d4, ROW_THREADS), 1024);
    LAUNCH(lazy_adam_kernel, dim3(A.dense_blocks + lb), dim3(ROW_THREADS), 0, s, (const uint64_t*)p.state, A);
    return (int)hipGetLastError();
}

struct LazyStep {
    bsarec_plan* p;
    explicit LazyStep(bsarec_plan* q) : p(q) { p->lazy_now = p->cfg.train_lazy_adam != 0; }
    ~LazyStep() { p->lazy_now = false; }
};

extern "C" int bsarec_gather_batch(const int64_t* table, const int64_t* answers_table, const int64_t* perm, long n_samples,
                                   const void* cursor, int B, int L, int64_t* ids_out, int64_t* answers_out, void* stream) {
    if (!table || !answers_table || !perm || !cursor || !ids_out || !answers_out || B < 1 || L < 1) return -10;
    LAUNCH(gather_batch_kernel, dim3(cdiv((long)B * L, ROW_THREADS)), dim3(ROW_THREADS), 0, (hipStream_t)stream, table,
           answers_table, perm, n_samples, (const long long*)cursor, B, L, ids_out, answers_out);
    return (int)hipGetLastError();
}

extern "C" int bsarec_train_step_indexed(bsarec_plan_t* p, const int64_t* table, const int64_t* answers_table,
                                         const int64_t* perm, long n_samples, void* cursor, int64_t* ids_buf,
                                         int64_t* answers_buf, const bsarec_adam_t* a, void* stream) {
    if (!p) return -10;
    RET(adam_check(a));
    RET(sampled_refusal(*p));
    RET(lazy_check(*p, *a));
    hipStream_t s = (hipStream_t)stream;
    if (!table || !answers_table || !perm || !cursor || !ids_buf || !answers_buf) return -10;
    LazyStep lazy(p);
    GatherP gp{table, answers_table, perm, n_samples, (const long long*)cursor, ids_buf, answers_buf};
    RET(forward_impl(p, ids_buf, 1, stream, gp, true));
    RET(loss_impl(p, answers_buf, stream, false));
    const TickP tk = make_tick(p->state, 1, a->lr, a->beta1, a->beta2, p->loss_rows, p->cfg.batch, p->loss, cursor, p->cfg.batch, 1);
    if (can_fuse_adam(*p, *a) && !p->cfg.separate_embed)
        return backward_impl(p, stream, tk, a);
    RET(backward_impl(p, stream, tk));
    RET(p->lazy_now ? lazy_adam_launch(*p, *a, s) : adam_launch(*a, p->state, s));
    return wimage_after_adam(*p, *a, s);
}

extern "C" int bsarec_grad_step_indexed(bsarec_plan_t* p, const int64_t* table, const int64_t* answers_table,
                                        const int64_t* perm, long n_samples, void* cursor, int64_t* ids_buf,
                                        int64_t* answers_buf, float lr, float b1, float b2, void* stream) {
    if (!p || !table || !answers_table || !perm || !cursor || !ids_buf || !answers_buf) return -10;
    RET(sampled_refusal(*p));
    if (p->cfg.train_lazy_adam) return -22;
    GatherP gp{table, answers_table, perm, n_samples, (const long long*)cursor, ids_buf, answers_buf};
    RET(forward_impl(p, ids_buf, 1, stream, gp, true));
    RET(bsarec_loss(p, answers_buf, stream));
    return backward_impl(p, stream, make_tick(p->state, lr > 0.f ? 1 : 0, lr, b1, b2, nullptr, 0, nullptr, cursor, p->cfg.batch, 1));
}

extern "C" int bsarec_train_step(bsarec_plan_t* p, const int64_t* ids, const int64_t* answers, const bsarec_adam_t* a,
                                 void* stream) {
    if (!p) return -10;
    RET(adam_check(a));
    RET(sampled_refusal(*p));
    RET(lazy_check(*p, *a));
    if (p->cfg.train_lazy_adam) {
        LazyStep lazy(p);
        RET(bsarec_step_begin(p, stream));
        RET(bsarec_forward_last(p, ids, 1, stream));
        RET(bsarec_loss(p, answers, stream));
        TickP tk = make_tick(p->state, 1, a->lr, a->beta1, a->beta2, nullptr, 0, nullptr, nullptr, 0, 0);
        RET(backward_impl(p, stream, tk));
        RET(lazy_adam_launch(*p, *a, (hipStream_t)stream));
        return wimage_after_adam(*p, *a, (hipStream_t)stream);
    }
    RET(bsarec_step_begin(p, stream));
    RET(bsarec_forward_last(p, ids, 1, stream));
    RET(bsarec_loss(p, answers, stream));
    RET(bsarec_backward(p, stream));
    RET(bsarec_adam_step(a, p->state, stream));
    return wimage_after_adam(*p, *a, (hipStream_t)stream);
}

extern "C" int bsarec_mask_seen(float* scores, long ld, int B, const int64_t* users, const int64_t* indptr,
                                const int64_t* indices, void* stream) {
    if (!scores || !users || !indptr || !indices || B < 1 || ld < 1) return -10;
    hipLaunchKernelGGL(mask_seen_kernel, dim3(B), dim3(ROW_THREADS), 0, (hipStream_t)stream, scores, ld, users, indptr, indices);
    return (int)hipGetLastError();
}

extern "C" int bsarec_topk_seen(float* scores, long ld, int B, int V, const int64_t* users, const int64_t* indptr,
                                const int64_t* indices, int k, int64_t* out_idx, float* out_val, void* stream) {
    static_assert(BSAREC_TOPK_MAX == TOPK_MAX && ROW_THREADS == 256, "topk_seen_kernel: one thread per digit bin");
    if (!scores || !out_idx || B < 1 || V < 1 || ld < V || k < 1 || k > BSAREC_TOPK_MAX || k > V) return -10;
    if (indptr && (!users || !indices)) return -10;
    hipLaunchKernelGGL(topk_seen_kernel, dim3(B), dim3(ROW_THREADS), 0, (hipStream_t)stream, scores, ld, V, users, indptr, indices, k,
                       out_idx, out_val);
    return (int)hipGetLastError();
}

extern "C" int bsarec_sampled_rank(const float* h, long ldh, const float* item_emb, int B, int V, int d, const int64_t* users,
                                   const int64_t* answers, const int64_t* indptr, const int64_t* indices, const int64_t* pop_cum,
                                   int n_neg, uint64_t seed, uint32_t tag, int32_t* rank_out, int64_t* cand_out, float* score_out,
                                   void* stream) {
    static_assert(BSAREC_NEG_MAX == NEG_MAX && BSAREC_NEG_MAX_DRAWS == NEG_MAX_DRAWS, "sampled_rank_kernel: the header's limits");
    if (!h || !item_emb || !users || !answers || !rank_out || (indptr && !indices)) return -10;
    if (B < 1 || V < 2 || d < 4 || d > 256 || d % 4 != 0 || ldh < d || n_neg < 1 || n_neg > BSAREC_NEG_MAX) return -10;
    if ((uintptr_t)item_emb % 16 != 0) return -10;
    hipLaunchKernelGGL(sampled_rank_kernel, dim3(B), dim3(ROW_THREADS), 0, (hipStream_t)stream, h, ldh, item_emb, V, d, users, answers,
                       indptr, indices, pop_cum, n_neg, (uint32_t)seed, (uint32_t)(seed >> 32), tag, rank_out, cand_out, score_out);
    return (int)hipGetLastError();
}

struct FrShape { long s, stride, cap; };
static bool fr_shape(int B, int V, int d, int k, int cand_cap, FrShape* out) {
    if (B < 1 || k < 1 || k > BSAREC_TOPK_MAX || V < k || d < 4 || d > 256 || d % 4 != 0) return false;
    if (cand_cap < 0 || (cand_cap > 0 && cand_cap < k) || cand_cap > (1 << 30)) return false;
    const long kv = (long)k * V;
    long s = 4 * (long)std::sqrt((double)kv);
    if (s < 4L * k) s = 4L * k;
    if (s > V) s = V;
    long cap = cand_cap;
    if (cap == 0) {
        cap = (4 * kv + s - 1) / s;
        cap = (cap + 255) / 256 * 256;
        if (cap < k) cap = k;
    }
    out->s = s; out->stride = V / s; out->cap = cap;
    return true;
}
static long fr_align(long x) { return (x + 255) / 256 * 256; }

extern "C" long bsarec_topk_full_workspace_bytes(int B, int V, int d, int k, int cand_cap) {
    FrShape f;
    if (!fr_shape(B, V, d, k, cand_cap, &f)) return -10;
    return fr_align((long)B * 8) + fr_align((long)B * 4) + fr_align((long)B * f.s * 4) + (long)B * f.cap * 8;
}

extern "C" int bsarec_topk_full_range(const float* h, long ldh, const float* item_emb, int B, int V, long col_base, int d,
                                      const int64_t* users, const int64_t* indptr, const int64_t* indices, int k, int cand_cap,
                                      void* workspace, long workspace_bytes, int64_t* out_idx, float* out_val, void* stream) {
    static_assert(BSAREC_TOPK_MAX == TOPK_MAX && ROW_THREADS == 256 && FR_ROWS == 128, "full_rank.h: the header's limits");
    FrShape f;
    if (!fr_shape(B, V, d, k, cand_cap, &f)) return -10;
    if (col_base < 0 || col_base + V > 0x7fffffffL) return -10;
    if (!h || !item_emb || !workspace || !out_idx || ldh < d || (indptr && (!users || !indices))) return -10;
    if ((uintptr_t)h % 16 != 0 || (uintptr_t)item_emb % 16 != 0 || (uintptr_t)workspace % 16 != 0) return -10;
    if (workspace_bytes < bsarec_topk_full_workspace_bytes(B, V, d, k, cand_cap)) return -10;
    char* ws = (char*)workspace;
    unsigned long long* tau = (unsigned long long*)ws;           ws += fr_align((long)B * 8);
    unsigned* count = (unsigned*)ws;                             ws += fr_align((long)B * 4);
    unsigned* skeys = (unsigned*)ws;                             ws += fr_align((long)B * f.s * 4);
    unsigned long long* list = (unsigned long long*)ws;
    const int cap = (int)f.cap;
    hipStream_t st = (hipStream_t)stream;
    const int tiles = (B + FR_ROWS - 1) / FR_ROWS, nblk = (V + FR_ITEMS - 1) / FR_ITEMS;
    int groups = (1024 + tiles - 1) / tiles;
    if (groups > nblk) groups = nblk;
    const size_t smem = (size_t)FR_ROWS * (d + 4) * sizeof(float);
    static bool attr = false;
    if (!attr) {
        const hipError_t e = hipFuncSetAttribute(reinterpret_cast<const void*>(full_rank_filter_kernel),
                                                 hipFuncAttributeMaxDynamicSharedMemorySize, (int)((size_t)FR_ROWS * 260 * sizeof(float)));
        if (e != hipSuccess) return (int)e;
        attr = true;
    }
    hipLaunchKernelGGL(full_rank_sample_kernel, dim3(B), dim3(ROW_THREADS), 0, st, h, ldh, item_emb, V, col_base, d, users, indptr,
                       indices, k, (int)f.s, (int)f.stride, skeys, tau, count);
    for (int round = 0; round <= FR_ROUNDS; ++round) {
        if (round > 0)
            hipLaunchKernelGGL(full_rank_rethreshold_kernel, dim3(B), dim3(ROW_THREADS), 0, st, k, cap, tau, count, list);
        hipLaunchKernelGGL(full_rank_filter_kernel, dim3(tiles, groups), dim3(ROW_THREADS), smem, st, h, ldh, item_emb, B, V, d, cap,
                           tau, count, list);
    }
    hipLaunchKernelGGL(full_rank_select_kernel, dim3(B), dim3(ROW_THREADS), 0, st, V, col_base, k, cap, users, indptr, indices, count,
                       list, out_idx, out_val);
    hipLaunchKernelGGL(full_rank_fallback_kernel, dim3(B), dim3(ROW_THREADS), 0, st, h, ldh, item_emb, V, col_base, d, k, cap, users,
                       indptr, indices, count, out_idx, out_val);
    return (int)hipGetLastError();
}

extern "C" int bsarec_topk_full(const float* h, long ldh, const float* item_emb, int B, int V, int d, const int64_t* users,
                                const int64_t* indptr, const int64_t* indices, int k, int cand_cap, void* workspace,
                                long workspace_bytes, int64_t* out_idx, float* out_val, void* stream) {
    return bsarec_topk_full_range(h, ldh, item_emb, B, V, 0, d, users, indptr, indices, k, cand_cap, workspace, workspace_bytes,
                                  out_idx, out_val, stream);
}

static int answer_rank_check(const float* h, long ldh, const float* E, int B, int V, long col_base, int d, const int64_t* users,
                             const int64_t* indptr, const int64_t* indices, const int64_t* answers, const void* out) {
    if (B < 1 || V < 1 || d < 4 || d > 256 || d % 4 != 0 || ldh < d) return -10;
    if (col_base < 0 || col_base + V > 0x7fffffffL) return -10;
    if (!h || !E || !answers || !out || (indptr && (!users || !indices))) return -10;
    if ((uintptr_t)h % 16 != 0 || (uintptr_t)E % 16 != 0) return -10;
    return 0;
}

extern "C" int bsarec_answer_rank_range(const float* h, long ldh, const float* item_rows, int B, int Vs, long col_base, int d,
                                        const int64_t* users, const int64_t* indptr, const int64_t* indices, const int64_t* answers,
                                        const float* answer_score, int32_t* rank_out, float* score_out, void* stream) {
    RET(answer_rank_check(h, ldh, item_rows, B, Vs, col_base, d, users, indptr, indices, answers, rank_out));
    hipStream_t st = (hipStream_t)stream;
    const int tiles = (B + FR_ROWS - 1) / FR_ROWS, nblk = (Vs + FR_ITEMS - 1) / FR_ITEMS;
    int groups = (1024 + tiles - 1) / tiles;
    if (groups > nblk) groups = nblk;
    const size_t smem = (size_t)FR_ROWS * (d + 4) * sizeof(float);
    static bool attr = false;
    if (!attr) {
        const hipError_t e = hipFuncSetAttribute(reinterpret_cast<const void*>(answer_rank_count_kernel),
                                                 hipFuncAttributeMaxDynamicSharedMemorySize, (int)((size_t)FR_ROWS * 260 * sizeof(float)));
        if (e != hipSuccess) return (int)e;
        attr = true;
    }
    hipLaunchKernelGGL(answer_rank_row_kernel<false>, dim3(B), dim3(ROW_THREADS), 0, st, h, ldh, item_rows, Vs, col_base, d, users,
                       indptr, indices, answers, answer_score, rank_out, score_out);
    hipLaunchKernelGGL(answer_rank_count_kernel, dim3(tiles, groups), dim3(ROW_THREADS), smem, st, h, ldh, item_rows, B, Vs, col_base,
                       d, users, indptr, indices, answers, answer_score, (const float*)score_out, rank_out);
    return (int)hipGetLastError();
}

extern "C" int bsarec_answer_rank(const float* h, long ldh, const float* item_emb, int B, int V, int d, const int64_t* users,
                                  const int64_t* indptr, const int64_t* indices, const int64_t* answers, int32_t* rank_out,
                                  float* score_out, void* stream) {
    return bsarec_answer_rank_range(h, ldh, item_emb, B, V, 0, d, users, indptr, indices, answers, nullptr, rank_out, score_out,
                                    stream);
}

extern "C" int bsarec_answer_score_range(const float* h, long ldh, const float* item_rows, int B, int Vs, long col_base, int d,
                                         const int64_t* users, const int64_t* indptr, const int64_t* indices,
                                         const int64_t* answers, float* score_out, void* stream) {
    RET(answer_rank_check(h, ldh, item_rows, B, Vs, col_base, d, users, indptr, indices, answers, score_out));
    hipLaunchKernelGGL(answer_rank_row_kernel<true>, dim3(B), dim3(ROW_THREADS), 0, (hipStream_t)stream, h, ldh, item_rows, Vs,
                       col_base, d, users, indptr, indices, answers, (const float*)nullptr, (int32_t*)nullptr, score_out);
    return (int)hipGetLastError();
}

static int info_nce_shape_check(int B, int d, int sim) {
    if (B < 1 || B > 4096 || d < 4 || d > 256 || d % 4 != 0 || (sim != 0 && sim != 1)) return -10;
    return 0;
}

extern "C" long bsarec_info_nce_workspace_bytes(int B, int d, int sim) {
    if (info_nce_shape_check(B, d, sim)) return -10;
    return nce_workspace_floats(B, d) * (long)sizeof(float);
}

static int info_nce_params(NceP& P, const float* z_i, long ld_i, const float* z_j, long ld_j, int B, int d, float inv_tau, int sim,
                           void* workspace, long workspace_bytes) {
    RET(info_nce_shape_check(B, d, sim));
    if (ld_i < d || ld_j < d || ld_i % 4 != 0 || ld_j % 4 != 0) return -10;
    if (!(inv_tau > 0.f) || !std::isfinite(inv_tau)) return -10;
    if (!z_i || !z_j || !workspace || (uintptr_t)z_i % 16 != 0 || (uintptr_t)z_j % 16 != 0 || (uintptr_t)workspace % 16 != 0) return -10;
    if (workspace_bytes < bsarec_info_nce_workspace_bytes(B, d, sim)) return -10;
    const long n = 2L * B;
    P.zi = z_i; P.zj = z_j; P.ldi = ld_i; P.ldj = ld_j;
    P.B = B; P.n = (int)n; P.d = d; P.cos = sim; P.S = nce_splits((int)n); P.T = cdiv(n, NCE_TILE);
    P.inv_tau = inv_tau;
    float* w = (float*)workspace;
    P.lse = w; P.spos = w + n; P.norm = w + 2 * n; P.pm = w + 3 * n; P.pl = P.pm + P.S * n; P.slab = w + nce_stat_floats(n, P.S);
    return 0;
}

extern "C" int bsarec_info_nce_fwd(const float* z_i, long ld_i, const float* z_j, long ld_j, int B, int d, float inv_tau, int sim,
                                   float* loss_out, float* rows_out, void* workspace, long workspace_bytes, void* stream) {
    NceP P;
    RET(info_nce_params(P, z_i, ld_i, z_j, ld_j, B, d, inv_tau, sim, workspace, workspace_bytes));
    if (!loss_out) return -10;
    hipStream_t st = (hipStream_t)stream;
    if (P.cos) hipLaunchKernelGGL(nce_norm_kernel, dim3(cdiv(P.n, ROW_THREADS / 64)), dim3(ROW_THREADS), 0, st, P);
    hipLaunchKernelGGL(nce_fwd_kernel, dim3(P.S, P.T), dim3(ROW_THREADS), 0, st, P);
    hipLaunchKernelGGL(nce_stat_kernel, dim3(1), dim3(1024), 0, st, P, loss_out, rows_out);
    return (int)hipGetLastError();
}

extern "C" int bsarec_info_nce_bwd(const float* z_i, long ld_i, const float* z_j, long ld_j, int B, int d, float inv_tau, int sim,
                                   const float* gout, void* workspace, long workspace_bytes, float* dz_i, float* dz_j,
                                   void* stream) {
    NceP P;
    RET(info_nce_params(P, z_i, ld_i, z_j, ld_j, B, d, inv_tau, sim, workspace, workspace_bytes));
    if (!gout || !dz_i || !dz_j || (uintptr_t)dz_i % 16 != 0 || (uintptr_t)dz_j % 16 != 0) return -10;
    hipStream_t st = (hipStream_t)stream;
    const dim3 grid(P.S, P.T);
    switch (cdiv(d, NCE_TILE)) {
        case 1: hipLaunchKernelGGL(nce_bwd_kernel<1>, grid, dim3(ROW_THREADS), 0, st, P); break;
        case 2: hipLaunchKernelGGL(nce_bwd_kernel<2>, grid, dim3(ROW_THREADS), 0, st, P); break;
        case 3: hipLaunchKernelGGL(nce_bwd_kernel<3>, grid, dim3(ROW_THREADS), 0, st, P); break;
        default: hipLaunchKernelGGL(nce_bwd_kernel<4>, grid, dim3(ROW_THREADS), 0, st, P); break;
    }
    hipLaunchKernelGGL(nce_dz_kernel, dim3(cdiv(P.n, ROW_THREADS / 64)), dim3(ROW_THREADS), 0, st, P, gout, dz_i, dz_j);
    return (int)hipGetLastError();
}

static DropP standalone_drop(float p, const void* state, int site) {
    DropP d;
    d.thresh = drop_thresh(p);
    d.scale = p > 0.f ? (float)(1.0 / (1.0 - (double)p)) : 1.f;
    d.rng = (const uint64_t*)state; d.site = (uint32_t)site;
    return d;
}

extern "C" int bsarec_freq_layer_fwd(const float* x, const float* sqrt_beta, const float* ln_w, const float* ln_b,
                                     const float* twiddle, int B, int L, int d, int cb, float eps, float p_drop,
                                     const void* state, int site, float* y, float* xhat, float* rstd, void* stream) {
    if (!x || !y || d % 4 || d > 256 || L > 256 || (long)cb * d > 8192 || (p_drop > 0.f && !state)) return -10;
    DISPATCH_LPR(d, RET(launch_freq_fwd<LPR>(x, sqrt_beta, ln_w, ln_b, eps, standalone_drop(p_drop, state, site), twiddle,
                                             B, L, d, cb, y, xhat, rstd, (hipStream_t)stream)));
    return 0;
}

extern "C" long bsarec_freq_layer_bwd_scratch_floats(int B, int L, int d) {
    const long T = (long)B * L;
    return 3 * T * d + (long)B * d + 2L * cdiv(T, 64) * d + 64;
}

extern "C" int bsarec_freq_layer_bwd(const float* x, const float* dy, const float* xhat, const float* rstd,
                                     const float* sqrt_beta, const float* ln_w, const float* twiddle, int B, int L, int d,
                                     int cb, float p_drop, const void* state, int site, float* scratch, float* dx,
                                     float* dsqrt_beta, float* dln_w, float* dln_b, void* stream) {
    if (!x || !dy || !scratch || d % 4 || d > 256 || L > 256 || (long)cb * d > 8192 || (p_drop > 0.f && !state)) return -10;
    hipStream_t s = (hipStream_t)stream;
    const int T = B * L, nb = cdiv(T, 64);
    float* dz = scratch; float* dF = dz + (long)T * d; float* pbeta = dF + (long)T * d;
    float* pg = pbeta + (long)B * d; float* pb = pg + (long)nb * d;
    LnBranch a; memset(&a, 0, sizeof(a));
    a.xhat = xhat; a.rstd = rstd; a.gamma = ln_w; a.in_scale = 1.f; a.drop = standalone_drop(p_drop, state, site);
    a.dT = dF; a.pgamma = pg; a.pbeta = pb;
    DISPATCH_LPR(d, LAUNCH((ln_bwd_kernel<LPR, 0>), dim3(nb), dim3(ROW_THREADS), 0, s, dy, a, a, dz, T, d, 64));
    HIPCHK(hipGetLastError());
    DISPATCH_LPR(d, RET(launch_freq_bwd<LPR>(x, dF, dz, sqrt_beta, twiddle, B, L, d, cb, dx, pbeta, s)));
    ReduceJobs3 hj;
    hj.j[0] = ReduceJob{pbeta, dsqrt_beta, B, d, d, 1.f, 0};
    hj.j[1] = ReduceJob{pg, dln_w, nb, d, d, 1.f, 0};
    hj.j[2] = ReduceJob{pb, dln_b, nb, d, d, 1.f, 0};
    LAUNCH(multi_reduce3_kernel, dim3(cdiv(d, 64), 3), dim3(ROW_THREADS), 0, s, hj);
    return (int)hipGetLastError();
}

extern "C" int bsarec_profile_select(bsarec_plan_t* p, int kclass) {
    if (!p) return -10;
    p->prof.kclass = kclass;
    p->prof.used = 0;
    return 0;
}

extern "C" int bsarec_profile_read(bsarec_plan_t* p, double* ms_total, int* launches) {
    if (!p) return -10;
    ProfState& ps = p->prof;
    double tot = 0.0;
    for (size_t i = 0; i < ps.used; ++i) {
        HIPCHK(hipEventSynchronize(ps.events[i].second));
        float ms = 0.f;
        HIPCHK(hipEventElapsedTime(&ms, ps.events[i].first, ps.events[i].second));
        tot += ms;
    }
    if (ms_total) *ms_total = tot;
    if (launches) *launches = (int)ps.used;
    ps.used = 0;
    return 0;
}

extern "C" int bsarec_profile_event_overhead(void* stream, int reps, double* ms_avg) {
    hipStream_t s = (hipStream_t)stream;
    hipEvent_t a, b;
    HIPCHK(hipEventCreate(&a)); HIPCHK(hipEventCreate(&b));
    double tot = 0.0;
    for (int i = 0; i < reps; ++i) {
        HIPCHK(hipEventRecord(a, s)); HIPCHK(hipEventRecord(b, s));
        HIPCHK(hipEventSynchronize(b));
        float ms = 0.f;
        HIPCHK(hipEventElapsedTime(&ms, a, b));
        tot += ms;
    }
    (void)hipEventDestroy(a); (void)hipEventDestroy(b);
    if (ms_avg) *ms_avg = reps > 0 ? tot / reps : 0.0;
    return 0;
}

static int shard_ptrs(ShardPtrs& S, const float* const* p, int world) {
    if (!p || world < 1 || world > 8) return -10;
    memset(&S, 0, sizeof(S));
    for (int r = 0; r < world; ++r) { if (!p[r]) return -10; S.p[r] = p[r]; }
    return 0;
}

extern "C" int bsarec_shard_gather_rows(const int64_t* ids, long n, const float* const* shards, int world, long rows_per,
                                        long V, int d, float* stage, int64_t* local_ids, void* stream) {
    if (!ids || !stage || !local_ids || n < 1 || rows_per < 1 || V < 1 || d < 4 || (d & 3)) return -10;
    if ((V + rows_per - 1) / rows_per > world) return -11;
    ShardPtrs S;
    RET(shard_ptrs(S, shards, world));
    const int d4 = d / 4;
    LAUNCH(shard_gather_rows_kernel, dim3(cdiv((n + 1) * d4, 256)), dim3(256), 0, (hipStream_t)stream, ids, n, S, rows_per, V, d4,
           stage, local_ids);
    return (int)hipGetLastError();
}

extern "C" int bsarec_shard_logits(const float* h, long ldh, int Bg, const float* E, int Vs, int d, float* logits, long ld,
                                   void* stream) {
    if (!h || !logits || Bg < 1 || Vs < 0 || d < 4 || (d & 3) || ld < Vs || (ld & 3) || ldh < d) return -10;
    if (Vs == 0) return 0;
    if (!E) return -10;
    GemmP g = gemm_defaults(Bg, (int)ld, d);
    g.Nb = Vs; g.lda = ldh; g.ldb = d;
    g.A[0] = h; g.B[0] = E;
    auto e = epi_linear<false, false, false>(logits, ld);
    return launch_gemm<64, 64, 2, 2, false, false, XF_NONE, XF_NONE, false>(g, no_xform(), e, nullptr, 1, (hipStream_t)stream);
}

extern "C" int bsarec_shard_ce_stats(const float* logits, long ld, int Bg, int Vs, const int64_t* answers, long lo, long V,
                                     float* stats, void* stream) {
    if (!logits || !answers || !stats || Bg < 1 || Vs < 0 || ld < Vs || (ld & 3)) return -10;
    LAUNCH(shard_ce_stats_kernel, dim3(Bg), dim3(ROW_THREADS), 0, (hipStream_t)stream, logits, ld, Vs, answers, lo, V, stats, Bg);
    return (int)hipGetLastError();
}

extern "C" int bsarec_shard_ce_grad(float* logits, long ld, int Bg, int Vs, const int64_t* answers, long lo, long V,
                                    const float* stats_all, int world, float* loss_rows, float* loss, void* stream) {
    if (!logits || !answers || !stats_all || !loss_rows || Bg < 1 || Vs < 0 || ld < Vs || (ld & 3) || world < 1 || world > 8)
        return -10;
    hipStream_t s = (hipStream_t)stream;
    LAUNCH(shard_ce_grad_kernel, dim3(Bg), dim3(ROW_THREADS), 0, s, logits, ld, Vs, answers, lo, V, stats_all, world, Bg,
           1.0f / (float)Bg, loss_rows);
    HIPCHK(hipGetLastError());
    if (loss) LAUNCH(loss_mean_kernel, dim3(1), dim3(ROW_THREADS), 0, s, loss_rows, Bg, loss);
    return (int)hipGetLastError();
}

static void shard_split(int Bg, int Vs, int d, int* nsplit, int* kchunk) {
    const long tiles = (long)cdiv(Bg, 64) * cdiv(d, 64);
    long want = (1024 + tiles - 1) / tiles;
    if (want < 1) want = 1;
    if (want > 64) want = 64;
    long ch = rup(cdiv(Vs > 0 ? Vs : 1, want), GEMM_BK);
    if (ch < 256) ch = 256;
    *kchunk = (int)ch;
    *nsplit = cdiv(Vs > 0 ? Vs : 1, ch);
}

extern "C" long bsarec_shard_head_bwd_scratch_floats(int Bg, int Vs, int d) {
    if (Bg < 1 || Vs < 0 || d < 4) return -10;
    int ns, kc;
    shard_split(Bg, Vs, d, &ns, &kc);
    return (long)ns * Bg * d;
}

extern "C" int bsarec_shard_head_bwd(const float* dlogits, long ld, int Bg, int Vs, const float* h, long ldh, const float* E,
                                     int d, float* dE, float* dh, float* scratch, void* stream) {
    if (!dlogits || !h || !dh || !scratch || Bg < 1 || Vs < 0 || d < 4 || (d & 3) || ld < Vs || (ld & 3) || ldh < d) return -10;
    hipStream_t s = (hipStream_t)stream;
    if (Vs == 0) { if (!g_dry) HIPCHK(hipMemsetAsync(dh, 0, (size_t)Bg * d * sizeof(float), s)); return 0; }
    if (!E || !dE) return -10;
    const XformP nox = no_xform();
    {
        GemmP g = gemm_defaults(Vs, d, Bg);
        g.lda = ld; g.ldb = ldh; g.A[0] = dlogits; g.B[0] = h;
        auto e = epi_linear<false, false, false>(dE, d);
        RET((launch_gemm<64, 64, 2, 2, true, true, XF_NONE, XF_NONE, false>(g, nox, e, nullptr, 1, s)));
    }
    int ns, kc;
    shard_split(Bg, Vs, d, &ns, &kc);
    {
        GemmP g = gemm_defaults(Bg, d, (int)ld);
        g.Kv = Vs; g.lda = ld; g.ldb = d; g.A[0] = dlogits; g.B[0] = E;
        g.nsplit = ns; g.kchunk = kc;
        auto e = epi_linear<false, false, false>(scratch, d);
        e.c_split = (long)Bg * d;
        RET((launch_gemm<64, 64, 2, 2, false, true, XF_NONE, XF_NONE, false>(g, nox, e, nullptr, 1, s)));
    }
    LAUNCH(shard_slab_sum_kernel, dim3(cdiv((long)Bg * d / 4, ROW_THREADS)), dim3(ROW_THREADS), 0, s, scratch, ns, Bg, d / 4, dh,
           (long)d);
    return (int)hipGetLastError();
}

extern "C" int bsarec_shard_scatter_rows(const int64_t* ids_all, long n, int world, const float* const* stage_grads, long lo,
                                         long Vs, long V, int d, float* dE, void* stream) {
    if (!ids_all || n < 1 || Vs < 0 || d < 4 || (d & 3)) return -10;
    if (Vs == 0) return 0;
    if (!dE) return -10;
    ShardPtrs G;
    RET(shard_ptrs(G, stage_grads, world));
    const int d4 = d / 4;
    LAUNCH(shard_scatter_rows_kernel, dim3(cdiv(n * world * d4, 256)), dim3(256), 0, (hipStream_t)stream, ids_all, n, world, G, lo,
           Vs, V, d4, dE);
    return (int)hipGetLastError();
}

extern "C" int bsarec_shard_ssm_draw(uint64_t key, const uint64_t* state, int N, long V, const int64_t* pop_cum, int logq,
                                     int* cand, float* corr, int* lazy_count, void* stream) {
    if (!state || !cand || !corr || N < 1 || N > SSM_NEG_MAX || V < 2 || V > INT32_MAX) return -10;
    SsmP P = ssm_params(nullptr, 0, 1, 1, nullptr, nullptr, cand, corr, N, V, pop_cum, logq, 4, SSM_SLAB_MAX);
    P.state = state;
    LAUNCH(shard_ssm_draw_kernel, dim3(cdiv(N, ROW_THREADS)), dim3(ROW_THREADS), 0, (hipStream_t)stream, P, key, lazy_count);
    return (int)hipGetLastError();
}

extern "C" int bsarec_shard_ssm_gather(const int64_t* answers, int B, const int* cand, int N, const float* const* shards, int world,
                                       long rows_per, long V, int d, float* rows, void* stream) {
    if (!answers || !cand || !rows || B < 1 || N < 1 || N > SSM_NEG_MAX || rows_per < 1 || V < 1 || d < 4 || (d & 3)) return -10;
    if ((V + rows_per - 1) / rows_per > world) return -11;
    ShardPtrs S;
    RET(shard_ptrs(S, shards, world));
    const int d4 = d / 4;
    LAUNCH(shard_ssm_gather_kernel, dim3(cdiv(((long)B + N) * d4, 256)), dim3(256), 0, (hipStream_t)stream, answers, B, cand, N, S,
           rows_per, V, d4, rows);
    return (int)hipGetLastError();
}

extern "C" int bsarec_shard_ssm_head(const float* h, long ldh, int B, int Bg, const float* rows, const int64_t* answers,
                                     const int* cand, const float* corr, int N, long V, const int64_t* pop_cum, int logq, int d,
                                     float* logits, float* dlogits, float* loss_rows, void* stream) {
    if (!h || !rows || !answers || !cand || !corr || !logits || !dlogits || !loss_rows) return -10;
    if (B < 1 || Bg < B || N < 1 || N > SSM_NEG_MAX || V < 2 || V > INT32_MAX || d < 4 || (d & 3) || ldh < d) return -10;
    hipStream_t s = (hipStream_t)stream;
    SsmP P = ssm_params(h, ldh, B, Bg, rows, answers, cand, corr, N, V, pop_cum, logq, d, SSM_SLAB_MAX);
    P.logits = logits; P.dlogits = dlogits; P.loss_rows = loss_rows;
    LAUNCH(ssm_logits_kernel<true>, dim3(cdiv(N, SSM_TILE), cdiv(B, SSM_TILE)), dim3(ROW_THREADS), 0, s, P);
    HIPCHK(hipGetLastError());
    LAUNCH(ssm_ce_kernel<true>, dim3(B), dim3(ROW_THREADS), 0, s, P);
    return (int)hipGetLastError();
}

extern "C" int bsarec_shard_ssm_loss(const float* loss_rows_all, int Bg, float* loss, void* stream) {
    if (!loss_rows_all || !loss || Bg < 1) return -10;
    LAUNCH(loss_mean_kernel, dim3(1), dim3(ROW_THREADS), 0, (hipStream_t)stream, loss_rows_all, Bg, loss);
    return (int)hipGetLastError();
}

extern "C" long bsarec_shard_ssm_bwd_scratch_floats(int B, int N, int d) {
    if (B < 1 || N < 1 || N > SSM_NEG_MAX || d < 4) return -10;
    int ns, ch;
    ssm_split(N, SSM_SLAB_MAX, &ns, &ch);
    return (long)ns * B * d;
}

extern "C" int bsarec_shard_ssm_bwd(const float* dlogits, int B, int N, const float* h, long ldh, const float* rows, int d,
                                    float* dh, long lddh, float* grad_rows, float* scratch, void* stream) {
    if (!dlogits || !h || !rows || !dh || !grad_rows || !scratch) return -10;
    if (B < 1 || N < 1 || N > SSM_NEG_MAX || d < 4 || (d & 3) || ldh < d || lddh < d || (lddh & 3)) return -10;
    hipStream_t s = (hipStream_t)stream;
    SsmP P = ssm_params(h, ldh, B, B, rows, nullptr, nullptr, nullptr, N, 2, nullptr, 0, d, SSM_SLAB_MAX);
    P.dlogits = const_cast<float*>(dlogits); P.slab = scratch; P.G = grad_rows;
    const int tilesC = std::max(1, std::min(cdiv((long)B * d, ROW_THREADS), 64));
    LAUNCH(ssm_bwd_kernel<true>, dim3(P.tilesA + P.tilesB + tilesC), dim3(ROW_THREADS), 0, s, P);
    HIPCHK(hipGetLastError());
    LAUNCH(shard_slab_sum_kernel, dim3(cdiv((long)B * d / 4, ROW_THREADS)), dim3(ROW_THREADS), 0, s, scratch, P.nslab, B, d / 4, dh,
           lddh);
    return (int)hipGetLastError();
}

extern "C" int bsarec_shard_ssm_pull(const int64_t* answers_all, int B, int world, const int* cand, int N,
                                     const float* const* grad_rows, long lo, long Vs, long V, int d, float* dE, void* stream) {
    if (!answers_all || !cand || B < 1 || N < 1 || N > SSM_NEG_MAX || Vs < 0 || lo < 0 || V < 1 || d < 4 || (d & 3)) return -10;
    ShardPtrs G;
    RET(shard_ptrs(G, grad_rows, world));
    if (Vs == 0) return 0;
    if (!dE) return -10;
    const int d4 = d / 4;
    LAUNCH(shard_ssm_pull_kernel, dim3(cdiv(((long)N + (long)world * B) * d4, 256)), dim3(256), 0, (hipStream_t)stream, answers_all,
           B, world, cand, N, G, lo, Vs, V, d4, dE);
    return (int)hipGetLastError();
}

extern "C" int bsarec_shard_lazy_mark(const int64_t* ids_all, long nids, const int64_t* answers_all, int Bg, const int* cand, int N,
                                      long lo, long Vs, long V, int* mark, int* rows, int* count, int cap, void* stream) {
    if (!ids_all || !answers_all || !cand || nids < 0 || Bg < 1 || N < 1 || N > SSM_NEG_MAX || Vs < 0 || lo < 0 || V < 1) return -10;
    if (Vs == 0) return 0;
    if (!mark || !rows || !count || cap < (int)std::min<long>(Vs, nids + Bg + N)) return -10;
    LazyRows T;
    memset(&T, 0, sizeof(T));
    T.mark = mark; T.rows = rows; T.count = count; T.cap = cap;
    const int nb = (int)std::max<long>(1, std::min<long>(cdiv(nids + Bg + N, ROW_THREADS), 256));
    LAUNCH(shard_lazy_mark_kernel, dim3(nb), dim3(ROW_THREADS), 0, (hipStream_t)stream, ids_all, nids, answers_all, Bg, cand, N, lo,
           Vs, V, T);
    return (int)hipGetLastError();
}

extern "C" int bsarec_shard_lazy_adam(float* E, float* dE, float* m, float* v, int d, float b1, float b2, float eps, float wd,
                                      int* mark, const int* rows, const int* count, int cap, const void* state, void* stream) {
    if (!state || d < 4 || (d & 3) || cap < 0) return -10;
    if (cap == 0) return 0;
    if (!E || !dE || !m || !v || !mark || !rows || !count) return -10;
    ShardLazyAdamP A;
    memset(&A, 0, sizeof(A));
    A.w = E; A.g = dE; A.m = m; A.v = v; A.b1 = b1; A.b2 = b2; A.eps = eps; A.wd = wd;
    A.T.mark = mark; A.T.rows = const_cast<int*>(rows); A.T.count = const_cast<int*>(count); A.T.cap = cap; A.T.d4 = d / 4;
    const int nb = (int)std::min<long>(cdiv((long)cap * A.T.d4, ROW_THREADS), 1024);
    LAUNCH(shard_lazy_adam_kernel, dim3(nb), dim3(ROW_THREADS), 0, (hipStream_t)stream, (const uint64_t*)state, A);
    return (int)hipGetLastError();
}
```

bsarec_amd/csrc/dw_direct.h:

```cpp
#pragma once
#include "fused_layer.h"

#define DW_MAX_PROB 12
#define DW_MAX_UNITS 24
#define DW_STAGES 5

typedef float f32x2 __attribute__((ext_vector_type(2)));
__device__ __forceinline__ f32x2 gld2(const float* p) { return *reinterpret_cast<const AS_GLOBAL f32x2*>((const AS_GLOBAL float*)p); }
__device__ __forceinline__ void gst2(float* p, f32x2 v) { *reinterpret_cast<AS_GLOBAL f32x2*>((AS_GLOBAL float*)p) = v; }

struct DwProblem {
    const float* A; const float* B;
    long lda, ldb;
    int M, N, K, kchunk;
    int nslab;
    float* slab;
    float* bslab;
    int gelu;
    int bf16;
};

struct DwUnit { short prob, m0, n0, pad; };

struct DwP {
    DwProblem P[DW_MAX_PROB];
    DwUnit U[DW_MAX_UNITS];
    int nunits, nslab;
    int nsmall, small_slabs;
};

template <bool BF> struct DwStage;
template <> struct DwStage<false> { f32x2 a[4]; f32x2 b[4]; };
template <> struct DwStage<true> { unsigned a[4]; unsigned b[4]; };

typedef int i32x2 __attribute__((ext_vector_type(2)));
__device__ __forceinline__ f32x2 bld2(__amdgpu_buffer_rsrc_t r, int voff, int soff) {
    return __builtin_bit_cast(f32x2, __builtin_amdgcn_raw_buffer_load_b64(r, voff, soff, 0));
}
template <bool BF>
__device__ __forceinline__ void dw_issue(DwStage<BF>& st, __amdgpu_buffer_rsrc_t ra, __amdgpu_buffer_rsrc_t rb, int voa, int vob,
                                         int soa, int sob, int rowa, int rowb) {
#pragma unroll
    for (int s = 0; s < 4; ++s) {
        if constexpr (BF) {
            st.a[s] = (unsigned)__builtin_amdgcn_raw_buffer_load_b32(ra, voa, soa + s * rowa, 0);
            st.b[s] = (unsigned)__builtin_amdgcn_raw_buffer_load_b32(rb, vob, sob + s * rowb, 0);
        } else {
            st.a[s] = bld2(ra, voa, soa + s * rowa);
            st.b[s] = bld2(rb, vob, sob + s * rowb);
        }
    }
}

template <bool GELU, bool MASK, bool BF, int STAGES>
__device__ __forceinline__ void dw_loop(__amdgpu_buffer_rsrc_t ra, __amdgpu_buffer_rsrc_t rb, int voa, int vob, int soa, int sob,
                                        int rowa, int rowb, int nkb, int crow, int kend, f32x16 (&acc)[2][2], f32x2& bs) {
    DwStage<BF> st[STAGES];
#pragma unroll
    for (int u = 0; u < STAGES; ++u) {
        dw_issue(st[u], ra, rb, voa, vob, soa, sob, rowa, rowb);
        soa += 8 * rowa; sob += 8 * rowb;
    }
    for (int kb = 0; kb < nkb; kb += STAGES) {
#pragma unroll
        for (int u = 0; u < STAGES; ++u) {
            if (kb + u >= nkb) break;
            DwStage<BF>& cur = st[u];
#pragma unroll
            for (int s = 0; s < 4; ++s) {
                f32x2 a, b;
                if constexpr (BF) { a = f32x2{bf_lo(cur.a[s]), bf_hi(cur.a[s])}; b = f32x2{bf_lo(cur.b[s]), bf_hi(cur.b[s])}; }
                else { a = cur.a[s]; b = cur.b[s]; }
                if (MASK) {
                    const bool ok = crow + s < kend;
                    a.x = ok ? a.x : 0.f; a.y = ok ? a.y : 0.f; b.x = ok ? b.x : 0.f; b.y = ok ? b.y : 0.f;
                }
                if (GELU) { b.x = gelu_f(b.x); b.y = gelu_f(b.y); }
                bs += a;
                acc[0][0] = __builtin_amdgcn_mfma_f32_32x32x2f32(a.x, b.x, acc[0][0], 0, 0, 0);
                acc[0][1] = __builtin_amdgcn_mfma_f32_32x32x2f32(a.x, b.y, acc[0][1], 0, 0, 0);
                acc[1][0] = __builtin_amdgcn_mfma_f32_32x32x2f32(a.y, b.x, acc[1][0], 0, 0, 0);
                acc[1][1] = __builtin_amdgcn_mfma_f32_32x32x2f32(a.y, b.y, acc[1][1], 0, 0, 0);
            }
            crow += 8;
            __builtin_amdgcn_sched_barrier(0);
            dw_issue(st[u], ra, rb, voa, vob, soa, sob, rowa, rowb);
            soa += 8 * rowa; sob += 8 * rowb;
            __builtin_amdgcn_sched_barrier(0);
        }
    }
}

struct DwStageM { unsigned a[8]; unsigned b[8]; };
__device__ __forceinline__ void dw_issue_m(DwStageM& st, __amdgpu_buffer_rsrc_t ra, __amdgpu_buffer_rsrc_t rb, int voa, int vob,
                                           int soa, int sob, int rowa, int rowb) {
#pragma unroll
    for (int s = 0; s < 8; ++s) {
        st.a[s] = (unsigned)__builtin_amdgcn_raw_buffer_load_b32(ra, voa, soa + s * rowa, 0);
        st.b[s] = (unsigned)__builtin_amdgcn_raw_buffer_load_b32(rb, vob, sob + s * rowb, 0);
    }
}
template <bool MASK, bool BIAS, int STAGES>
__device__ __forceinline__ void dw_loop_m(__amdgpu_buffer_rsrc_t ra, __amdgpu_buffer_rsrc_t rb, int voa, int vob, int soa, int sob,
                                          int rowa, int rowb, int nkb, int crow, int kend, f32x16 (&acc)[2][2], f32x2& bs) {
    DwStageM st[STAGES];
#pragma unroll
    for (int u = 0; u < STAGES; ++u) {
        dw_issue_m(st[u], ra, rb, voa, vob, soa, sob, rowa, rowb);
        soa += 16 * rowa; sob += 16 * rowb;
    }
    for (int kb = 0; kb < nkb; kb += STAGES) {
#pragma unroll
        for (int u = 0; u < STAGES; ++u) {
            if (kb + u >= nkb) break;
            DwStageM& cur = st[u];
            u32x4 a0, a1, b0, b1;
#pragma unroll
            for (int j = 0; j < 4; ++j) {
                unsigned x0 = cur.a[2 * j], x1 = cur.a[2 * j + 1], y0 = cur.b[2 * j], y1 = cur.b[2 * j + 1];
                if (MASK) {
                    const bool ok0 = crow + 2 * j < kend, ok1 = crow + 2 * j + 1 < kend;
                    x0 = ok0 ? x0 : 0u; y0 = ok0 ? y0 : 0u; x1 = ok1 ? x1 : 0u; y1 = ok1 ? y1 : 0u;
                }
                a0[j] = (x0 & 0xFFFFu) | (x1 << 16); a1[j] = (x0 >> 16) | (x1 & 0xFFFF0000u);
                b0[j] = (y0 & 0xFFFFu) | (y1 << 16); b1[j] = (y0 >> 16) | (y1 & 0xFFFF0000u);
                if (BIAS) { bs.x += bf_lo(x0) + bf_lo(x1); bs.y += bf_hi(x0) + bf_hi(x1); }
            }
            acc[0][0] = mfma_bf16(a0, b0, acc[0][0]);
            acc[0][1] = mfma_bf16(a0, b1, acc[0][1]);
            acc[1][0] = mfma_bf16(a1, b0, acc[1][0]);
            acc[1][1] = mfma_bf16(a1, b1, acc[1][1]);
            crow += 16;
            __builtin_amdgcn_sched_barrier(0);
            dw_issue_m(st[u], ra, rb, voa, vob, soa, sob, rowa, rowb);
            soa += 16 * rowa; sob += 16 * rowb;
            __builtin_amdgcn_sched_barrier(0);
        }
    }
}
struct DwStageC { f32x2 a[8]; f32x2 b[8]; };
__device__ __forceinline__ void dw_issue_c(DwStageC& st, __amdgpu_buffer_rsrc_t ra, __amdgpu_buffer_rsrc_t rb, int voa, int vob,
                                           int soa, int sob, int rowa, int rowb) {
#pragma unroll
    for (int s = 0; s < 8; ++s) { st.a[s] = bld2(ra, voa, soa + s * rowa); st.b[s] = bld2(rb, vob, sob + s * rowb); }
}
template <bool MASK, int STAGES>
__device__ __forceinline__ void dw_loop_c(__amdgpu_buffer_rsrc_t ra, __amdgpu_buffer_rsrc_t rb, int voa, int vob, int soa, int sob,
                                          int rowa, int rowb, int nkb, int crow, int kend, f32x16 (&acc)[2][2]) {
    DwStageC st[STAGES];
#pragma unroll
    for (int u = 0; u < STAGES; ++u) {
        dw_issue_c(st[u], ra, rb, voa, vob, soa, sob, rowa, rowb);
        soa += 16 * rowa; sob += 16 * rowb;
    }
    for (int kb = 0; kb < nkb; kb += STAGES) {
#pragma unroll
        for (int u = 0; u < STAGES; ++u) {
            if (kb + u >= nkb) break;
            DwStageC& cur = st[u];
            u32x4 a0, a1, b0, b1;
#pragma unroll
            for (int j = 0; j < 4; ++j) {
                f32x2 x0 = cur.a[2 * j], x1 = cur.a[2 * j + 1], y0 = cur.b[2 * j], y1 = cur.b[2 * j + 1];
                if (MASK) {
                    const bool ok0 = crow + 2 * j < kend, ok1 = crow + 2 * j + 1 < kend;
                    if (!ok0) { x0 = f32x2{0.f, 0.f}; y0 = x0; }
                    if (!ok1) { x1 = f32x2{0.f, 0.f}; y1 = x1; }
                }
                a0[j] = pk_bf16(x0.x, x1.x); a1[j] = pk_bf16(x0.y, x1.y);
                b0[j] = pk_bf16(y0.x, y1.x); b1[j] = pk_bf16(y0.y, y1.y);
            }
            acc[0][0] = mfma_bf16(a0, b0, acc[0][0]);
            acc[0][1] = mfma_bf16(a0, b1, acc[0][1]);
            acc[1][0] = mfma_bf16(a1, b0, acc[1][0]);
            acc[1][1] = mfma_bf16(a1, b1, acc[1][1]);
            crow += 16;
            __builtin_amdgcn_sched_barrier(0);
            dw_issue_c(st[u], ra, rb, voa, vob, soa, sob, rowa, rowb);
            soa += 16 * rowa; sob += 16 * rowb;
            __builtin_amdgcn_sched_barrier(0);
        }
    }
}
#define DW_STAGES_M 3

#ifdef BSAREC_DW_STAMPS
#define DW_STAMP_MAX 2048
__device__ long long g_dw_stamps[DW_STAMP_MAX][8];
struct DwStampScope {
    long long t0; int kind;
    __device__ DwStampScope() : t0(wall_clock64()), kind(4) {}
    __device__ ~DwStampScope() {
        if (threadIdx.x == 0 && blockIdx.x < DW_STAMP_MAX) {
            long long* r = g_dw_stamps[blockIdx.x];
            r[0] = t0; r[1] = wall_clock64();
            r[2] = ((long long)__builtin_amdgcn_s_getreg((32 - 1) << 11 | 20) << 32) | (unsigned)__builtin_amdgcn_s_getreg((32 - 1) << 11 | 4);
            r[3] = kind;
        }
    }
};
#define DW_STAMP_SCOPE DwStampScope dw_stamp_
#define DW_STAMP_KIND(k) dw_stamp_.kind = (k)
#define DW_STAMP_AT(i) do { if (threadIdx.x == 0 && blockIdx.x < DW_STAMP_MAX) g_dw_stamps[blockIdx.x][i] = wall_clock64(); } while (0)
#else
#define DW_STAMP_SCOPE
#define DW_STAMP_KIND(k)
#define DW_STAMP_AT(i)
#endif

template <int STAGES = DW_STAGES, bool BFM = false, bool CVT = false>
__device__ __forceinline__ void dw_wg_body(const DwProblem& Q, int m0, int n0, int slab, float (*red)[66][64]) {
    const int wv = __builtin_amdgcn_readfirstlane((int)(threadIdx.x >> 6));
    const int lane = threadIdx.x & 63, l31 = lane & 31, half = lane >> 5;
    const int sub = Q.kchunk >> 2;
    const int kbeg = slab * Q.kchunk + wv * sub, kend = min(Q.K, kbeg + sub);
    const int nkb = kend > kbeg ? (kend - kbeg + 7) >> 3 : 0;
    f32x16 acc[2][2];
#pragma unroll
    for (int i = 0; i < 2; ++i)
#pragma unroll
        for (int jn = 0; jn < 2; ++jn)
#pragma unroll
            for (int r = 0; r < 16; ++r) acc[i][jn][r] = 0.f;
    f32x2 bs = {0.f, 0.f};
    if (nkb > 0) {
        const int esz = Q.bf16 ? 2 : 4;
        const int recs_a = (int)(((long)(Q.K - 1) * Q.lda + Q.M) * esz), recs_b = (int)(((long)(Q.K - 1) * Q.ldb + Q.N) * esz);
        const __amdgpu_buffer_rsrc_t ra = __builtin_amdgcn_make_buffer_rsrc((void*)Q.A, 0, recs_a, 0x00020000);
        const __amdgpu_buffer_rsrc_t rb = __builtin_amdgcn_make_buffer_rsrc((void*)Q.B, 0, recs_b, 0x00020000);
        const int rowa = (int)Q.lda * esz, rowb = (int)Q.ldb * esz;
        const int voa = 4 * half * rowa + (m0 + 2 * l31) * esz, vob = 4 * half * rowb + (n0 + 2 * l31) * esz;
        const int soa = kbeg * rowa, sob = kbeg * rowb;
        const int crow = kbeg + 4 * half;
        const bool full = kbeg + 8 * nkb <= kend;
        DW_STAMP_AT(4);
#define DW_RUN(BFV) \
        if (Q.gelu) { \
            if (full) dw_loop<true, false, BFV, STAGES>(ra, rb, voa, vob, soa, sob, rowa, rowb, nkb, crow, kend, acc, bs); \
            else dw_loop<true, true, BFV, STAGES>(ra, rb, voa, vob, soa, sob, rowa, rowb, nkb, crow, kend, acc, bs); \
        } else { \
            if (full) dw_loop<false, false, BFV, STAGES>(ra, rb, voa, vob, soa, sob, rowa, rowb, nkb, crow, kend, acc, bs); \
            else dw_loop<false, true, BFV, STAGES>(ra, rb, voa, vob, soa, sob, rowa, rowb, nkb, crow, kend, acc, bs); \
        }
        if constexpr (CVT) {
            const int nkb16 = (kend - kbeg + 15) >> 4;
            const int voa_c = 8 * half * rowa + (m0 + 2 * l31) * 4, vob_c = 8 * half * rowb + (n0 + 2 * l31) * 4;
            const int crow_c = kbeg + 8 * half;
            if (kbeg + 16 * nkb16 <= kend) dw_loop_c<false, STAGES>(ra, rb, voa_c, vob_c, soa, sob, rowa, rowb, nkb16, crow_c, kend, acc);
            else dw_loop_c<true, STAGES>(ra, rb, voa_c, vob_c, soa, sob, rowa, rowb, nkb16, crow_c, kend, acc);
        } else if constexpr (BFM) {
        if (Q.bf16 && !Q.gelu) {
            const int nkb16 = (kend - kbeg + 15) >> 4;
            const int voa_m = 8 * half * rowa + (m0 + 2 * l31) * 2, vob_m = 8 * half * rowb + (n0 + 2 * l31) * 2;
            const int crow_m = kbeg + 8 * half;
            const bool full16 = kbeg + 16 * nkb16 <= kend, bias = Q.bslab != nullptr && n0 == 0;
            if (full16) {
                if (bias) dw_loop_m<false, true, DW_STAGES_M>(ra, rb, voa_m, vob_m, soa, sob, rowa, rowb, nkb16, crow_m, kend, acc, bs);
                else dw_loop_m<false, false, DW_STAGES_M>(ra, rb, voa_m, vob_m, soa, sob, rowa, rowb, nkb16, crow_m, kend, acc, bs);
            } else dw_loop_m<true, true, DW_STAGES_M>(ra, rb, voa_m, vob_m, soa, sob, rowa, rowb, nkb16, crow_m, kend, acc, bs);
        } else if (Q.bf16) { DW_RUN(true) } else { DW_RUN(false) }
        } else { DW_RUN(false) }
#undef DW_RUN
    }
    DW_STAMP_AT(5);
    bs.x = xor32_sum(bs.x); bs.y = xor32_sum(bs.y);
    {
        float (*mine)[64] = red[wv];
#pragma unroll
        for (int i = 0; i < 2; ++i)
#pragma unroll
            for (int jn = 0; jn < 2; ++jn)
#pragma unroll
                for (int r = 0; r < 16; ++r) mine[(i * 2 + jn) * 16 + r][lane] = acc[i][jn][r];
        mine[64][lane] = bs.x; mine[65][lane] = bs.y;
    }
    __syncthreads();
    DW_STAMP_AT(6);
    float* C = Q.slab + (long)slab * Q.M * Q.N;
    const int qi = wv >> 1, r0 = (wv & 1) * 8;
#pragma unroll
    for (int rr = 0; rr < 8; ++rr) {
        const int r = r0 + rr;
        f32x2 v = {red[0][(qi * 2) * 16 + r][lane], red[0][(qi * 2 + 1) * 16 + r][lane]};
#pragma unroll
        for (int w = 1; w < 4; ++w) { v.x += red[w][(qi * 2) * 16 + r][lane]; v.y += red[w][(qi * 2 + 1) * 16 + r][lane]; }
        const int m = m0 + 2 * (rho(r) + 4 * half) + qi;
        if (m < Q.M) gst2(C + (long)m * Q.N + n0 + 2 * l31, v);
    }
    if (wv == 0 && Q.bslab && n0 == 0 && half == 0 && m0 + 2 * l31 + 1 < Q.M) {
        f32x2 b = {red[0][64][lane], red[0][65][lane]};
#pragma unroll
        for (int w = 1; w < 4; ++w) { b.x += red[w][64][lane]; b.y += red[w][65][lane]; }
        gst2(Q.bslab + (long)slab * Q.M + m0 + 2 * l31, b);
    }
}


struct ScatterP { const float* de; const int* ids32; int T; unsigned long long* dA; int nblocks; };
__global__ void __launch_bounds__(256)
dw_direct_kernel(const DwP G, const TickP tk, const ScatterP sc) {
    __shared__ __attribute__((aligned(16))) float red[4][66][64];
    static_assert(sizeof(red) >= (2 * SCATTER_FLOATS + 2 * (SCATTER_FLOATS / 64)) * 4, "scatter scratch fits the reduction scratch");
    DW_STAMP_SCOPE;
    {
        const int nmain = 8 * ((G.nslab + 7) >> 3) * (G.nunits - G.nsmall) + G.nsmall * G.small_slabs;
        if ((int)blockIdx.x >= nmain) {
            const int x = blockIdx.x - nmain;
            DW_STAMP_KIND(x < sc.nblocks ? 2 : 3);
            if (x < sc.nblocks) embed_scatter_block<16>(sc.de, sc.ids32, sc.T, 64, sc.dA, x, &red[0][0][0]);
            else if (tk.state) tick_body(tk, &red[0][0][0]);
            return;
        }
    }
    int slab, ui;
    const int nbig = G.nunits - G.nsmall, nbw = 8 * ((G.nslab + 7) >> 3) * nbig;
    if ((int)blockIdx.x < nbw) {
        const int xcd = blockIdx.x & 7, j = blockIdx.x >> 3;
        slab = xcd + 8 * (j / nbig);
        if (slab >= G.nslab) return;
        ui = G.nsmall + j % nbig;
        DW_STAMP_KIND(0);
    } else {
        const int bid = blockIdx.x - nbw;
        ui = bid % G.nsmall; slab = bid / G.nsmall;
        DW_STAMP_KIND(1);
    }
    const DwUnit u = G.U[ui];
    const DwProblem& Q = G.P[u.prob];
    if (slab >= Q.nslab) return;
    dw_wg_body<DW_STAGES, true>(Q, u.m0, u.n0, slab, red);
}

struct DhP {
    const float* A; long lda;
    const float* E;
    int B, V, kchunk, nsplit;
    float* slab;
};

template <int STAGES = DW_STAGES, bool CVT = false>
__device__ __forceinline__ void dh_wave_body(const DhP& G, int wg) {
    const int wv = __builtin_amdgcn_readfirstlane((int)(threadIdx.x >> 6));
    const int lane = threadIdx.x & 63, l31 = lane & 31, half = lane >> 5;
    const int mtiles = (G.B + 31) >> 5;
    const int unit = wg * 4 + wv, mt = unit % mtiles, split = unit / mtiles;
    if (split >= G.nsplit) return;
    const int kbeg = split * G.kchunk, kend = min(G.V, kbeg + G.kchunk);
    const int nkb = kend > kbeg ? (kend - kbeg + 7) >> 3 : 0;
    const int m = min(32 * mt + l31, G.B - 1);
    f32x16 acc0, acc1;
#pragma unroll
    for (int r = 0; r < 16; ++r) { acc0[r] = 0.f; acc1[r] = 0.f; }
    if (nkb > 0) {
        const __amdgpu_buffer_rsrc_t ra = __builtin_amdgcn_make_buffer_rsrc((void*)G.A, 0, (int)((long)G.B * G.lda * 4), 0x00020000);
        const __amdgpu_buffer_rsrc_t rb = __builtin_amdgcn_make_buffer_rsrc((void*)G.E, 0, (int)((long)G.V * 256), 0x00020000);
        if constexpr (CVT) {
            const int nkb16 = (kend - kbeg + 15) >> 4;
            const int voa = (int)((long)m * G.lda * 4) + 32 * half, vob = 8 * half * 256 + 8 * l31;
            int soa = kbeg * 4, sob = kbeg * 256, ccol = kbeg + 8 * half;
            f32x4 sa[STAGES][2]; f32x2 sb[STAGES][8];
            auto issue = [&](int u) {
                sa[u][0] = __builtin_bit_cast(f32x4, __builtin_amdgcn_raw_buffer_load_b128(ra, voa, soa, 0));
                sa[u][1] = __builtin_bit_cast(f32x4, __builtin_amdgcn_raw_buffer_load_b128(ra, voa + 16, soa, 0));
#pragma unroll
                for (int s = 0; s < 8; ++s) sb[u][s] = bld2(rb, vob, sob + s * 256);
                soa += 64; sob += 16 * 256;
            };
#pragma unroll
            for (int u = 0; u < STAGES; ++u) issue(u);
            for (int kb = 0; kb < nkb16; kb += STAGES) {
#pragma unroll
                for (int u = 0; u < STAGES; ++u) {
                    if (kb + u >= nkb16) break;
                    f32x4 x0 = sa[u][0], x1 = sa[u][1];
#pragma unroll
                    for (int e = 0; e < 4; ++e) {
                        if (ccol + e >= kend) x0[e] = 0.f;
                        if (ccol + 4 + e >= kend) x1[e] = 0.f;
                    }
                    const u32x4 a = pk8(x0, x1);
                    u32x4 b0, b1;
#pragma unroll
                    for (int j = 0; j < 4; ++j) {
                        b0[j] = pk_bf16(sb[u][2 * j].x, sb[u][2 * j + 1].x);
                        b1[j] = pk_bf16(sb[u][2 * j].y, sb[u][2 * j + 1].y);
                    }
                    acc0 = mfma_bf16(a, b0, acc0);
                    acc1 = mfma_bf16(a, b1, acc1);
                    ccol += 16;
                    __builtin_amdgcn_sched_barrier(0);
                    issue(u);
                    __builtin_amdgcn_sched_barrier(0);
                }
            }
        } else {
        const int voa = (int)((long)m * G.lda * 4) + 16 * half, vob = 4 * half * 256 + 8 * l31;
        int soa = kbeg * 4, sob = kbeg * 256, ccol = kbeg + 4 * half;
        f32x4 sa[STAGES]; f32x2 sb[STAGES][4];
        auto issue = [&](int u) {
            sa[u] = __builtin_bit_cast(f32x4, __builtin_amdgcn_raw_buffer_load_b128(ra, voa, soa, 0));
#pragma unroll
            for (int s = 0; s < 4; ++s) sb[u][s] = bld2(rb, vob, sob + s * 256);
            soa += 32; sob += 8 * 256;
        };
#pragma unroll
        for (int u = 0; u < STAGES; ++u) issue(u);
        for (int kb = 0; kb < nkb; kb += STAGES) {
#pragma unroll
            for (int u = 0; u < STAGES; ++u) {
                if (kb + u >= nkb) break;
#pragma unroll
                for (int s = 0; s < 4; ++s) {
                    const float a = ccol + s < kend ? sa[u][s] : 0.f;
                    const f32x2 b = sb[u][s];
                    acc0 = __builtin_amdgcn_mfma_f32_32x32x2f32(a, b.x, acc0, 0, 0, 0);
                    acc1 = __builtin_amdgcn_mfma_f32_32x32x2f32(a, b.y, acc1, 0, 0, 0);
                }
                ccol += 8;
                __builtin_amdgcn_sched_barrier(0);
                issue(u);
                __builtin_amdgcn_sched_barrier(0);
            }
        }
    }
    }
    float* C = G.slab + (long)split * G.B * 64;
#pragma unroll
    for (int r = 0; r < 16; ++r) {
        const int row = 32 * mt + rho(r) + 4 * half;
        if (row < G.B) gst2(C + (long)row * 64 + 2 * l31, f32x2{acc0[r], acc1[r]});
    }
}

template <bool BFH>
__global__ void __launch_bounds__(256)
logits_bwd_direct_kernel(const DwProblem Q, int tiles, const DhP H) {
    __shared__ __attribute__((aligned(16))) float red[4][66][64];
    if ((int)blockIdx.x < tiles) dw_wg_body<4, false, BFH>(Q, 64 * (int)blockIdx.x, 0, 0, red);
    else dh_wave_body<4, BFH>(H, (int)blockIdx.x - tiles);
}

struct LogitsP { const float* H; long ldh; const float* E; float* C; int B, V, Vp; };
__global__ void __launch_bounds__(256)
logits_direct_kernel(const LogitsP G) {
    const int wv = __builtin_amdgcn_readfirstlane((int)(threadIdx.x >> 6));
    const int lane = threadIdx.x & 63, l31 = lane & 31, half = lane >> 5;
    const int ntile = (G.Vp + 31) >> 5, mtiles = (G.B + 31) >> 5;
    const int unit = blockIdx.x * 4 + wv;
    const int nt = unit % ntile, mt = unit / ntile;
    if (mt >= mtiles) return;
    const int m = min(32 * mt + l31, G.B - 1);
    const int v = min(32 * nt + l31, G.V - 1);
    const float* ap = G.H + (long)m * G.ldh + 32 * half;
    const float* bp = G.E + (long)v * 64 + 32 * half;
    f32x4 a[8], b[8];
#pragma unroll
    for (int i = 0; i < 8; ++i) a[i] = gld4(ap + 4 * i);
#pragma unroll
    for (int i = 0; i < 8; ++i) b[i] = gld4(bp + 4 * i);
    f32x16 acc;
#pragma unroll
    for (int r = 0; r < 16; ++r) acc[r] = 0.f;
#pragma unroll
    for (int i = 0; i < 8; ++i)
#pragma unroll
        for (int j = 0; j < 4; ++j) acc = __builtin_amdgcn_mfma_f32_32x32x2f32(a[i][j], b[i][j], acc, 0, 0, 0);
    const int col = 32 * nt + l31;
    if (col >= G.Vp) return;
    const bool real = col < G.V;
#pragma unroll
    for (int r = 0; r < 16; ++r) {
        const int row = 32 * mt + rho(r) + 4 * half;
        if (row < G.B) gst(G.C + (long)row * G.Vp + col, real ? acc[r] : 0.f);
    }
}
```

include/bsarec_hip.h:

```cpp
#ifndef BSAREC_HIP_H
#define BSAREC_HIP_H

#include <stddef.h>
#include <stdint.h>

#ifdef __cplusplus
extern "C" {
#endif

#define BSAREC_MAX_LAYERS 16
#define BSAREC_ABI_VERSION 10

typedef struct {
    int batch;
    int seq_len;
    int hidden;
    int heads;
    int layers;
    int item_size;
    int cutoff_bins;
    float alpha;
    float ln_eps;
    float p_hidden;
    float p_attn;
    int filter_kind;
    int hidden_act;
    int storage;
    int no_fused;
    int no_prune_top;
    int dw_tiled;
    int splits;
    int top_slabs;
    int separate_embed;
    int separate_top;
    int chain_kernels;
    int x3_products;
    int train_negatives;
    int train_sampler;
    int train_no_logq;
    int train_lazy_adam;
    int weight_image;
} bsarec_config_t;

typedef struct {
    float *sqrt_beta, *filter_ln_w, *filter_ln_b;
    float *query_w, *query_b, *key_w, *key_b, *value_w, *value_b, *dense_w, *dense_b;
    float *attn_ln_w, *attn_ln_b;
    float *ffn1_w, *ffn1_b, *ffn2_w, *ffn2_b, *ffn_ln_w, *ffn_ln_b;
    float *filter_cw;
} bsarec_layer_t;

typedef struct {
    float *item_emb;
    float *pos_emb;
    float *ln_w, *ln_b;
    bsarec_layer_t layer[BSAREC_MAX_LAYERS];
} bsarec_tensors_t;

enum {
    BSAREC_BUF_LAYER_OUT = 0,
    BSAREC_BUF_LOGITS = 1,
    BSAREC_BUF_LOSS = 2,
    BSAREC_BUF_DSP = 3,
    BSAREC_BUF_HMIX = 4,
    BSAREC_BUF_PROBS = 5,
    BSAREC_BUF_DLAYER_IN = 6,
    BSAREC_BUF_LOSS_ROWS = 7,
    BSAREC_BUF_CTX = 8,
    BSAREC_BUF_DLOGITS = 9,
    BSAREC_BUF_TRAIN_CAND = 10,
    BSAREC_BUF_TRAIN_CORR = 11,
    BSAREC_BUF_TRAIN_LOGITS = 12,
    BSAREC_BUF_TRAIN_DLOGITS = 13
};

typedef struct bsarec_plan bsarec_plan_t;

int bsarec_abi_version(void);

size_t bsarec_workspace_bytes(const bsarec_config_t *cfg);

#define BSAREC_STATE_BYTES 64

int bsarec_plan_create(bsarec_plan_t **out, const bsarec_config_t *cfg, const bsarec_tensors_t *params,
                       const bsarec_tensors_t *grads, const bsarec_tensors_t *shadow, void *workspace,
                       size_t workspace_bytes, void *state, const float *twiddle, void *stream);
int bsarec_shadow_refresh(bsarec_plan_t *plan, void *stream);
int bsarec_wimage_refresh(bsarec_plan_t *plan, void *stream);
long bsarec_wimage_floats(const bsarec_config_t *cfg);
long bsarec_wimage_offset(int which, int transposed, int d, int n, int k);
int bsarec_buffer_is_bf16(const bsarec_plan_t *plan, int buffer, int layer);

int bsarec_plan_is_fused(const bsarec_plan_t *plan);
int bsarec_config_is_fused(const bsarec_config_t *cfg);
void bsarec_plan_destroy(bsarec_plan_t *plan);

typedef void (*bsarec_hook_t)(void *user, void *stream);
int bsarec_plan_set_dense_grad_hook(bsarec_plan_t *plan, bsarec_hook_t hook, void *user, float *lookup_grad);

#define BSAREC_TRAIN_NEG_MAX 8192
#define BSAREC_TRAIN_NEG_SITE 0x4E454753u

int bsarec_plan_set_train_sampler(bsarec_plan_t *plan, const int64_t *pop_cum);

long bsarec_buffer_offset(const bsarec_plan_t *plan, int buffer, int layer);

int bsarec_step_begin(bsarec_plan_t *plan, void *stream);

int bsarec_forward(bsarec_plan_t *plan, const int64_t *ids, int train, void *stream);

int bsarec_loss(bsarec_plan_t *plan, const int64_t *answers, void *stream);

int bsarec_forward_last(bsarec_plan_t *plan, const int64_t *ids, int train, void *stream);

int bsarec_loss_bce(bsarec_plan_t *plan, const int64_t *pos_ids, const int64_t *neg_ids, void *stream);
int bsarec_loss_logsig(bsarec_plan_t *plan, const int64_t *pos_ids, const int64_t *neg_ids, void *stream);

int bsarec_logits(bsarec_plan_t *plan, void *stream);

int bsarec_backward(bsarec_plan_t *plan, void *stream);

int bsarec_backward_seq(bsarec_plan_t *plan, const float *d_out, void *stream);

int bsarec_backward_seq_multi(bsarec_plan_t *plan, const float *const *d_outs, void *stream);

typedef struct {
    float *params;
    const float *grads;
    float *exp_avg, *exp_avg_sq;
    long n;
    float lr, beta1, beta2, eps, weight_decay;
    float grad_scale;
    void *shadow_bf16;
    long shadow_from;
    float *grads2;
    long grads2_n;
    int n_grad_srcs;
    const float *grad_srcs[8];
    bsarec_plan_t *wimage_plan;
} bsarec_adam_t;

int bsarec_adam_step(const bsarec_adam_t *adam, void *state, void *stream);
int bsarec_adam_apply(const bsarec_adam_t *adam, void *state, void *stream);

int bsarec_train_step(bsarec_plan_t *plan, const int64_t *ids, const int64_t *answers, const bsarec_adam_t *adam,
                      void *stream);

int bsarec_gather_batch(const int64_t *table, const int64_t *answers_table, const int64_t *perm, long n_samples,
                        const void *cursor, int B, int L, int64_t *ids_out, int64_t *answers_out, void *stream);

int bsarec_train_step_indexed(bsarec_plan_t *plan, const int64_t *table, const int64_t *answers_table,
                              const int64_t *perm, long n_samples, void *cursor, int64_t *ids_buf, int64_t *answers_buf,
                              const bsarec_adam_t *adam, void *stream);

int bsarec_grad_step_indexed(bsarec_plan_t *plan, const int64_t *table, const int64_t *answers_table,
                             const int64_t *perm, long n_samples, void *cursor, int64_t *ids_buf, int64_t *answers_buf,
                             float lr, float beta1, float beta2, void *stream);

int bsarec_mask_seen(float *scores, long ld, int B, const int64_t *users, const int64_t *indptr,
                     const int64_t *indices, void *stream);

#define BSAREC_TOPK_MAX 1024
int bsarec_topk_seen(float *scores, long ld, int B, int V, const int64_t *users, const int64_t *indptr,
                     const int64_t *indices, int k, int64_t *out_idx, float *out_val, void *stream);

#define BSAREC_NEG_MAX 1024
#define BSAREC_NEG_MAX_DRAWS (1 << 20)
int bsarec_sampled_rank(const float *h, long ldh, const float *item_emb, int B, int V, int d, const int64_t *users,
                        const int64_t *answers, const int64_t *indptr, const int64_t *indices, const int64_t *pop_cum,
                        int n_neg, uint64_t seed, uint32_t tag, int32_t *rank_out, int64_t *cand_out, float *score_out,
                        void *stream);

long bsarec_topk_full_workspace_bytes(int B, int V, int d, int k, int cand_cap);
int bsarec_topk_full(const float *h, long ldh, const float *item_emb, int B, int V, int d, const int64_t *users,
                     const int64_t *indptr, const int64_t *indices, int k, int cand_cap, void *workspace, long workspace_bytes,
                     int64_t *out_idx, float *out_val, void *stream);
int bsarec_topk_full_range(const float *h, long ldh, const float *item_rows, int B, int Vs, long col_base, int d,
                           const int64_t *users, const int64_t *indptr, const int64_t *indices, int k, int cand_cap,
                           void *workspace, long workspace_bytes, int64_t *out_idx, float *out_val, void *stream);

int bsarec_answer_rank(const float *h, long ldh, const float *item_emb, int B, int V, int d, const int64_t *users,
                       const int64_t *indptr, const int64_t *indices, const int64_t *answers, int32_t *rank_out,
                       float *score_out, void *stream);
int bsarec_answer_rank_range(const float *h, long ldh, const float *item_rows, int B, int Vs, long col_base, int d,
                             const int64_t *users, const int64_t *indptr, const int64_t *indices, const int64_t *answers,
                             const float *answer_score, int32_t *rank_out, float *score_out, void *stream);
int bsarec_answer_score_range(const float *h, long ldh, const float *item_rows, int B, int Vs, long col_base, int d,
                              const int64_t *users, const int64_t *indptr, const int64_t *indices, const int64_t *answers,
                              float *score_out, void *stream);

long bsarec_info_nce_workspace_bytes(int B, int d, int sim);
int bsarec_info_nce_fwd(const float *z_i, long ld_i, const float *z_j, long ld_j, int B, int d, float inv_tau, int sim,
                        float *loss_out, float *rows_out, void *workspace, long workspace_bytes, void *stream);
int bsarec_info_nce_bwd(const float *z_i, long ld_i, const float *z_j, long ld_j, int B, int d, float inv_tau, int sim,
                        const float *gout, void *workspace, long workspace_bytes, float *dz_i, float *dz_j, void *stream);

int bsarec_freq_layer_fwd(const float *x, const float *sqrt_beta, const float *ln_w, const float *ln_b,
                          const float *twiddle, int B, int L, int d, int cutoff_bins, float eps, float p_drop,
                          const void *state, int site, float *y, float *xhat, float *rstd, void *stream);
long bsarec_freq_layer_bwd_scratch_floats(int B, int L, int d);
int bsarec_freq_layer_bwd(const float *x, const float *dy, const float *xhat, const float *rstd,
                          const float *sqrt_beta, const float *ln_w, const float *twiddle, int B, int L, int d,
                          int cutoff_bins, float p_drop, const void *state, int site,
                          float *scratch ,
                          float *dx, float *dsqrt_beta, float *dln_w, float *dln_b, void *stream);

enum { BSAREC_K_NONE = 0, BSAREC_K_FFN1 = 1, BSAREC_K_FFN2 = 2, BSAREC_K_QKV = 3, BSAREC_K_LOGITS = 4,
       BSAREC_K_DU = 5, BSAREC_K_DW1 = 6, BSAREC_K_FUSED_FWD = 7, BSAREC_K_FUSED_BWD = 8 };
int bsarec_profile_select(bsarec_plan_t *plan, int kclass);
int bsarec_debug_stamps(bsarec_plan_t *plan, void *dev_buf);
int bsarec_profile_read(bsarec_plan_t *plan, double *ms_total, int *launches);
int bsarec_profile_event_overhead(void *stream, int reps, double *ms_avg);

#ifdef __cplusplus
}
#endif
#endif
```

Measured before the change: 1.718 million.

## Fold cross-entropy softmax into logits stats and backward head kernels

```diff
diff --git a/bsarec_amd/_lib.py b/bsarec_amd/_lib.py
--- a/bsarec_amd/_lib.py
+++ b/bsarec_amd/_lib.py
@@ -44,6 +44,7 @@
                 ("separate_top", C.c_int), ("chain_kernels", C.c_int), ("x3_products", C.c_int),
                 ("train_negatives", C.c_int), ("train_sampler", C.c_int), ("train_no_logq", C.c_int),
                 ("train_lazy_adam", C.c_int),
+                ("separate_ce", C.c_int),
                 ("weight_image", C.c_int)]
 
 
@@ -52,7 +53,7 @@
 
 
 OPTION_FIELDS = ("storage", "no_fused", "no_prune_top", "dw_tiled", "splits", "top_slabs", "separate_embed", "separate_top", "chain_kernels", "x3_products",
-                 "weight_image")
+                 "separate_ce", "weight_image")
 HIDDEN_ACTS = {"gelu": 0, "relu": 1, "swish": 2, "tanh": 3, "sigmoid": 4}
 
 _defaults = {k: 0 for k in OPTION_FIELDS}
@@ -81,6 +82,8 @@
             d[key] = int(e[env])
     if e.get("BSAREC_STORAGE") == "bf16":
         d["storage"] = 1
+    if e.get("BSAREC_HEAD_CE") == "separate":
+        d["separate_ce"] = 1
     if e.get("BSAREC_WEIGHT_IMAGE") == "0":
         d["weight_image"] = 0
     return d
diff --git a/bsarec_amd/csrc/bsarec_hip.hip b/bsarec_amd/csrc/bsarec_hip.hip
--- a/bsarec_amd/csrc/bsarec_hip.hip
+++ b/bsarec_amd/csrc/bsarec_hip.hip
@@ -96,6 +96,9 @@
     LazyRows lazy = {};
     bool lazy_now = false;
     float* wimg = nullptr;
+    float* head_stats = nullptr;
+    const int64_t* fold_answers = nullptr;
+    bool head_folded = false;
 };
 struct PlanScope {
     bsarec_plan* prev;
@@ -204,6 +207,7 @@
     if (c.train_negatives > 0 && c.storage != 0) return -18;
     if (c.train_lazy_adam < 0 || c.train_lazy_adam > 1 || (c.train_lazy_adam && c.train_negatives == 0)) return -19;
     if (c.weight_image < 0 || c.weight_image > 1) return -20;
+    if (c.separate_ce < 0 || c.separate_ce > 1) return -20;
     return 0;
 }
 
@@ -255,6 +259,13 @@
     if (c.train_negatives > 0) ssm_split(c.train_negatives, std::min(p.vsplit, SSM_SLAB_MAX), &p.ssm_nslab, &chunk);
 }
 
+static bool head_fold_shape(const bsarec_plan& p) {
+    return p.fused && p.cfg.hidden == 64 && p.Vp <= 4096 && p.cfg.batch <= 512 && p.direct_dw;
+}
+static long head_stats_floats(const bsarec_plan& p) {
+    return (long)cdiv(p.cfg.batch, 32) * cdiv(cdiv(p.Vp, 32), 4) * 32 * 2;
+}
+
 static void carve(bsarec_plan& p, char* base, size_t* total) {
     const bsarec_config_t& c = p.cfg;
     const long T = p.T, d = c.hidden, B = c.batch, L = c.seq_len, h = c.heads, N = c.layers;
@@ -278,6 +289,7 @@
     }
     p.logits = cv.take<float>(B * p.Vp); p.dlogits = cv.take<float>(B * p.Vp);
     p.loss_rows = cv.take<float>(B); p.loss = cv.take<float>(4);
+    p.head_stats = head_fold_shape(p) ? cv.take<float>(head_stats_floats(p)) : nullptr;
     p.dXa = cv.take<float>(Td); p.dXb = cv.take<float>(Td); p.dz = cv.take<float>(Td); p.dT = cv.take<float>(Td);
     p.dU = cv.take<float>(4 * Td); p.dH = cv.take<float>(Td); p.dXacc = cv.take<float>(Td); p.dO = cv.take<float>(Td);
     p.dF = cv.take<float>(Td); p.dC = cv.take<float>(Td); p.dS = cv.take<float>(B * h * L * p.Lp);
@@ -929,7 +941,10 @@
     return 0;
 }
 
-extern "C" int bsarec_logits(bsarec_plan_t* p, void* stream) {
+static int logits_impl(bsarec_plan_t* p, void* stream, bool stats);
+extern "C" int bsarec_logits(bsarec_plan_t* p, void* stream) { return logits_impl(p, stream, false); }
+
+static int logits_impl(bsarec_plan_t* p, void* stream, bool stats) {
     if (!p) return -10;
     PlanScope scope(p);
     hipStream_t s = (hipStream_t)stream;
@@ -938,10 +953,14 @@
     if (p->fused && d == 64 && p->Vp <= 4096 && c.batch <= 512 && !g_dry) {
         LogitsP G;
         G.H = h_last(*p); G.ldh = h_last_stride(*p); G.E = p->P.item_emb; G.C = p->logits;
-        G.B = c.batch; G.V = c.item_size; G.Vp = p->Vp;
+        G.B = c.batch; G.V = c.item_size; G.Vp = p->Vp; G.stats = p->head_stats;
         const long units = (long)cdiv(c.batch, 32) * cdiv(p->Vp, 32);
         ProfScope prof(BSAREC_K_LOGITS, s);
-        hipLaunchKernelGGL(logits_direct_kernel, dim3((unsigned)cdiv(units, 4)), dim3(256), 0, s, G);
+        if (stats) {
+            if (!p->head_stats || 32L * (cdiv(p->Vp, 32) - 1) >= c.item_size) return -21;
+            hipLaunchKernelGGL(logits_direct_kernel<true>, dim3((unsigned)(cdiv(c.batch, 32) * cdiv(cdiv(p->Vp, 32), 4))), dim3(256), 0, s, G);
+        } else
+            hipLaunchKernelGGL(logits_direct_kernel<false>, dim3((unsigned)cdiv(units, 4)), dim3(256), 0, s, G);
         return (int)hipGetLastError();
     }
     GemmP g = gemm_defaults(c.batch, p->Vp, d);
@@ -979,9 +998,18 @@
     return P;
 }
 
-static int loss_impl(bsarec_plan_t* p, const int64_t* answers, void* stream, bool with_mean) {
+static HeadFoldP head_fold_params(const bsarec_plan& p) {
+    HeadFoldP F;
+    memset(&F, 0, sizeof(F));
+    F.stats = p.head_stats; F.answers = p.fold_answers; F.logits = p.logits; F.ld = p.Vp; F.loss_rows = p.loss_rows;
+    F.ngroup = cdiv(cdiv(p.Vp, 32), 4); F.V = p.cfg.item_size; F.B = p.cfg.batch; F.inv_b = 1.0f / (float)p.cfg.batch;
+    return F;
+}
+
+static int loss_impl(bsarec_plan_t* p, const int64_t* answers, void* stream, bool with_mean, bool fold = false) {
     if (!p || !answers) return -10;
     hipStream_t s = (hipStream_t)stream;
+    p->head_folded = false;
     if (p->cfg.train_negatives > 0) {
         RET(sampled_refusal(*p));
         p->loss_kind = 2; p->ssm_answers = answers;
@@ -993,9 +1021,18 @@
         if (with_mean) LAUNCH(loss_mean_kernel, dim3(1), dim3(ROW_THREADS), 0, s, p->loss_rows, P.B, p->loss);
         return (int)hipGetLastError();
     }
-    RET(bsarec_logits(p, stream));
     p->loss_kind = 0;
     const bsarec_config_t& c = p->cfg;
+    if (head_fold_shape(*p) && !g_dry) {
+        RET(logits_impl(p, stream, true));
+        p->fold_answers = answers;
+        if (fold && !with_mean) { p->head_folded = true; return 0; }
+        LAUNCH(ce_rows_stats_kernel, dim3(c.batch), dim3(256), 0, s, head_fold_params(*p), p->dlogits);
+        HIPCHK(hipGetLastError());
+        if (with_mean) LAUNCH(loss_mean_kernel, dim3(1), dim3(ROW_THREADS), 0, s, p->loss_rows, c.batch, p->loss);
+        return (int)hipGetLastError();
+    }
+    RET(bsarec_logits(p, stream));
     const int V = c.item_size;
     const float inv_b = 1.0f / (float)c.batch;
 #define CE_VEC(N4) LAUNCH(ce_rows_vec_kernel<N4>, dim3(c.batch), dim3(ROW_THREADS), 0, s, p->logits, answers, V, p->Vp, inv_b, p->dlogits, p->loss_rows)
@@ -1097,17 +1134,24 @@
     } else if (direct_logits) {
         DwProblem q;
         memset(&q, 0, sizeof(q));
-        q.A = p.dlogits; q.B = hlast; q.lda = p.Vp; q.ldb = ldh; q.M = c.item_size; q.N = d; q.K = B;
+        const bool fold = p.head_folded && head_fold_shape(p);
+        p.head_folded = false;
+        const float* A = fold ? p.logits : p.dlogits;
+        q.A = A; q.B = hlast; q.lda = p.Vp; q.ldb = ldh; q.M = c.item_size; q.N = d; q.K = B;
         q.kchunk = (int)rup(B, 32); q.nslab = 1; q.slab = p.G.item_emb; q.bslab = nullptr; q.gelu = 0;
         DhP H;
         memset(&H, 0, sizeof(H));
-        H.A = p.dlogits; H.lda = p.Vp; H.E = p.P.item_emb; H.B = B; H.V = c.item_size; H.kchunk = p.vchunk;
+        H.A = A; H.lda = p.Vp; H.E = p.P.item_emb; H.B = B; H.V = c.item_size; H.kchunk = p.vchunk;
         H.nsplit = p.vsplit; H.slab = p.dlast_slab;
         const int tiles = cdiv(c.item_size, 64);
         if (!dw_problem_ok(q) || !dh_problem_ok(H)) return -21;
         const dim3 lb_grid(tiles + cdiv(cdiv(B, 32) * p.vsplit, 4));
-        if (p.bf) LAUNCH(logits_bwd_direct_kernel<true>, lb_grid, dim3(256), 0, s, q, tiles, H);
-        else LAUNCH(logits_bwd_direct_kernel<false>, lb_grid, dim3(256), 0, s, q, tiles, H);
+        const HeadFoldP F = head_fold_params(p);
+        if (fold) {
+            if (p.bf) LAUNCH((logits_bwd_direct_kernel<true, true>), lb_grid, dim3(256), 0, s, q, tiles, H, F);
+            else LAUNCH((logits_bwd_direct_kernel<false, true>), lb_grid, dim3(256), 0, s, q, tiles, H, F);
+        } else if (p.bf) LAUNCH((logits_bwd_direct_kernel<true, false>), lb_grid, dim3(256), 0, s, q, tiles, H, F);
+        else LAUNCH((logits_bwd_direct_kernel<false, false>), lb_grid, dim3(256), 0, s, q, tiles, H, F);
         HIPCHK(hipGetLastError());
     } else {
         PairP G;
@@ -1555,7 +1599,7 @@
     LazyStep lazy(p);
     GatherP gp{table, answers_table, perm, n_samples, (const long long*)cursor, ids_buf, answers_buf};
     RET(forward_impl(p, ids_buf, 1, stream, gp, true));
-    RET(loss_impl(p, answers_buf, stream, false));
+    RET(loss_impl(p, answers_buf, stream, false, !p->cfg.separate_ce));
     const TickP tk = make_tick(p->state, 1, a->lr, a->beta1, a->beta2, p->loss_rows, p->cfg.batch, p->loss, cursor, p->cfg.batch, 1);
     if (can_fuse_adam(*p, *a) && !p->cfg.separate_embed)
         return backward_impl(p, stream, tk, a);
diff --git a/bsarec_amd/csrc/dw_direct.h b/bsarec_amd/csrc/dw_direct.h
--- a/bsarec_amd/csrc/dw_direct.h
+++ b/bsarec_amd/csrc/dw_direct.h
@@ -52,9 +52,49 @@
     }
 }
 
-template <bool GELU, bool MASK, bool BF, int STAGES>
+
+#define HEAD_GROUP_MAX 32
+#define HEAD_TAB_ROWS 528
+struct HeadFoldP {
+    const float* stats;
+    const int64_t* answers;
+    const float* logits; long ld;
+    float* loss_rows;
+    int ngroup, V, B;
+    float inv_b;
+};
+template <int N>
+__device__ __forceinline__ void head_merge(const f32x2 (&v)[N], int n, float& M, float& S) {
+    M = v[0].x;
+#pragma unroll
+    for (int t = 1; t < N; ++t) M = fmaxf(M, v[t].x);
+    S = 0.f;
+#pragma unroll
+    for (int t = 0; t < N; ++t)
+        if (t < n) S = fmaf(v[t].y, expf(v[t].x - M), S);
+}
+__device__ __forceinline__ float head_row_lse(const float* stats, int ngroup, int row) {
+    const float* p = stats + (((long)(row >> 5) * ngroup) * 32 + (row & 31)) * 2;
+    f32x2 v[HEAD_GROUP_MAX];
+#pragma unroll
+    for (int t = 0; t < HEAD_GROUP_MAX; ++t) v[t] = gld2(p + min(t, ngroup - 1) * 64);
+    float M, S;
+    head_merge<HEAD_GROUP_MAX>(v, ngroup, M, S);
+    return M + logf(S);
+}
+__device__ __forceinline__ float head_g(float x, float lse, bool hit, bool real, float inv_b) {
+    const float g = (expf(x - lse) - (hit ? 1.0f : 0.0f)) * inv_b;
+    return real ? g : 0.f;
+}
+__device__ __forceinline__ int head_answer(const int64_t* answers, int row, int V) {
+    const int a = (int)answers[row];
+    return a < 0 ? 0 : (a >= V ? V - 1 : a);
+}
+
+template <bool GELU, bool MASK, bool BF, int STAGES, bool FOLD = false>
 __device__ __forceinline__ void dw_loop(__amdgpu_buffer_rsrc_t ra, __amdgpu_buffer_rsrc_t rb, int voa, int vob, int soa, int sob,
-                                        int rowa, int rowb, int nkb, int crow, int kend, f32x16 (&acc)[2][2], f32x2& bs) {
+                                        int rowa, int rowb, int nkb, int crow, int kend, f32x16 (&acc)[2][2], f32x2& bs,
+                                        const f32x2* tab = nullptr, int c0 = 0, int V = 0, float inv_b = 0.f) {
     DwStage<BF> st[STAGES];
 #pragma unroll
     for (int u = 0; u < STAGES; ++u) {
@@ -71,6 +111,11 @@
                 f32x2 a, b;
                 if constexpr (BF) { a = f32x2{bf_lo(cur.a[s]), bf_hi(cur.a[s])}; b = f32x2{bf_lo(cur.b[s]), bf_hi(cur.b[s])}; }
                 else { a = cur.a[s]; b = cur.b[s]; }
+                if constexpr (FOLD) {
+                    const f32x2 t = tab[crow + s];
+                    const int ans = __float_as_int(t.y);
+                    a.x = head_g(a.x, t.x, c0 == ans, c0 < V, inv_b); a.y = head_g(a.y, t.x, c0 + 1 == ans, c0 + 1 < V, inv_b);
+                }
                 if (MASK) {
                     const bool ok = crow + s < kend;
                     a.x = ok ? a.x : 0.f; a.y = ok ? a.y : 0.f; b.x = ok ? b.x : 0.f; b.y = ok ? b.y : 0.f;
@@ -144,9 +189,10 @@
 #pragma unroll
     for (int s = 0; s < 8; ++s) { st.a[s] = bld2(ra, voa, soa + s * rowa); st.b[s] = bld2(rb, vob, sob + s * rowb); }
 }
-template <bool MASK, int STAGES>
+template <bool MASK, int STAGES, bool FOLD = false>
 __device__ __forceinline__ void dw_loop_c(__amdgpu_buffer_rsrc_t ra, __amdgpu_buffer_rsrc_t rb, int voa, int vob, int soa, int sob,
-                                          int rowa, int rowb, int nkb, int crow, int kend, f32x16 (&acc)[2][2]) {
+                                          int rowa, int rowb, int nkb, int crow, int kend, f32x16 (&acc)[2][2],
+                                          const f32x2* tab = nullptr, int c0 = 0, int V = 0, float inv_b = 0.f) {
     DwStageC st[STAGES];
 #pragma unroll
     for (int u = 0; u < STAGES; ++u) {
@@ -162,6 +208,12 @@
 #pragma unroll
             for (int j = 0; j < 4; ++j) {
                 f32x2 x0 = cur.a[2 * j], x1 = cur.a[2 * j + 1], y0 = cur.b[2 * j], y1 = cur.b[2 * j + 1];
+                if constexpr (FOLD) {
+                    const f32x2 t0 = tab[crow + 2 * j], t1 = tab[crow + 2 * j + 1];
+                    const int a0_ = __float_as_int(t0.y), a1_ = __float_as_int(t1.y);
+                    x0.x = head_g(x0.x, t0.x, c0 == a0_, c0 < V, inv_b); x0.y = head_g(x0.y, t0.x, c0 + 1 == a0_, c0 + 1 < V, inv_b);
+                    x1.x = head_g(x1.x, t1.x, c0 == a1_, c0 < V, inv_b); x1.y = head_g(x1.y, t1.x, c0 + 1 == a1_, c0 + 1 < V, inv_b);
+                }
                 if (MASK) {
                     const bool ok0 = crow + 2 * j < kend, ok1 = crow + 2 * j + 1 < kend;
                     if (!ok0) { x0 = f32x2{0.f, 0.f}; y0 = x0; }
@@ -208,10 +260,19 @@
 #define DW_STAMP_AT(i)
 #endif
 
-template <int STAGES = DW_STAGES, bool BFM = false, bool CVT = false>
-__device__ __forceinline__ void dw_wg_body(const DwProblem& Q, int m0, int n0, int slab, float (*red)[66][64]) {
+template <int STAGES = DW_STAGES, bool BFM = false, bool CVT = false, bool FOLD = false>
+__device__ __forceinline__ void dw_wg_body(const DwProblem& Q, int m0, int n0, int slab, float (*red)[66][64],
+                                           f32x2* tab = nullptr, const HeadFoldP* F = nullptr) {
     const int wv = __builtin_amdgcn_readfirstlane((int)(threadIdx.x >> 6));
     const int lane = threadIdx.x & 63, l31 = lane & 31, half = lane >> 5;
+    if constexpr (FOLD) {
+        for (int r = threadIdx.x; r < HEAD_TAB_ROWS; r += 256) {
+            f32x2 t = {0.f, __int_as_float(-1)};
+            if (r < F->B) t = f32x2{head_row_lse(F->stats, F->ngroup, r), __int_as_float(head_answer(F->answers, r, F->V))};
+            tab[r] = t;
+        }
+        __syncthreads();
+    }
     const int sub = Q.kchunk >> 2;
     const int kbeg = slab * Q.kchunk + wv * sub, kend = min(Q.K, kbeg + sub);
     const int nkb = kend > kbeg ? (kend - kbeg + 7) >> 3 : 0;
@@ -246,8 +307,14 @@
             const int nkb16 = (kend - kbeg + 15) >> 4;
             const int voa_c = 8 * half * rowa + (m0 + 2 * l31) * 4, vob_c = 8 * half * rowb + (n0 + 2 * l31) * 4;
             const int crow_c = kbeg + 8 * half;
+            if constexpr (FOLD) {
+                const int c0 = m0 + 2 * l31;
+                if (kbeg + 16 * nkb16 <= kend) dw_loop_c<false, STAGES, true>(ra, rb, voa_c, vob_c, soa, sob, rowa, rowb, nkb16, crow_c, kend, acc, tab, c0, F->V, F->inv_b);
+                else dw_loop_c<true, STAGES, true>(ra, rb, voa_c, vob_c, soa, sob, rowa, rowb, nkb16, crow_c, kend, acc, tab, c0, F->V, F->inv_b);
+            } else {
             if (kbeg + 16 * nkb16 <= kend) dw_loop_c<false, STAGES>(ra, rb, voa_c, vob_c, soa, sob, rowa, rowb, nkb16, crow_c, kend, acc);
             else dw_loop_c<true, STAGES>(ra, rb, voa_c, vob_c, soa, sob, rowa, rowb, nkb16, crow_c, kend, acc);
+            }
         } else if constexpr (BFM) {
         if (Q.bf16 && !Q.gelu) {
             const int nkb16 = (kend - kbeg + 15) >> 4;
@@ -259,6 +326,10 @@
                 else dw_loop_m<false, false, DW_STAGES_M>(ra, rb, voa_m, vob_m, soa, sob, rowa, rowb, nkb16, crow_m, kend, acc, bs);
             } else dw_loop_m<true, true, DW_STAGES_M>(ra, rb, voa_m, vob_m, soa, sob, rowa, rowb, nkb16, crow_m, kend, acc, bs);
         } else if (Q.bf16) { DW_RUN(true) } else { DW_RUN(false) }
+        } else if constexpr (FOLD) {
+            const int c0 = m0 + 2 * l31;
+            if (full) dw_loop<false, false, false, STAGES, true>(ra, rb, voa, vob, soa, sob, rowa, rowb, nkb, crow, kend, acc, bs, tab, c0, F->V, F->inv_b);
+            else dw_loop<false, true, false, STAGES, true>(ra, rb, voa, vob, soa, sob, rowa, rowb, nkb, crow, kend, acc, bs, tab, c0, F->V, F->inv_b);
         } else { DW_RUN(false) }
 #undef DW_RUN
     }
@@ -338,8 +409,8 @@
     float* slab;
 };
 
-template <int STAGES = DW_STAGES, bool CVT = false>
-__device__ __forceinline__ void dh_wave_body(const DhP& G, int wg) {
+template <int STAGES = DW_STAGES, bool CVT = false, bool FOLD = false>
+__device__ __forceinline__ void dh_wave_body(const DhP& G, int wg, const HeadFoldP* F = nullptr) {
     const int wv = __builtin_amdgcn_readfirstlane((int)(threadIdx.x >> 6));
     const int lane = threadIdx.x & 63, l31 = lane & 31, half = lane >> 5;
     const int mtiles = (G.B + 31) >> 5;
@@ -351,6 +422,13 @@
     f32x16 acc0, acc1;
 #pragma unroll
     for (int r = 0; r < 16; ++r) { acc0[r] = 0.f; acc1[r] = 0.f; }
+    float lse = 0.f, inv_b = 0.f; int ans = -1;
+    auto fold_row = [&]() {
+        if constexpr (FOLD) {
+            lse = head_row_lse(F->stats, F->ngroup, m); ans = head_answer(F->answers, m, F->V); inv_b = F->inv_b;
+            if (split == 0 && half == 0 && 32 * mt + l31 < G.B) gst(F->loss_rows + m, lse - F->logits[(long)m * F->ld + ans]);
+        }
+    };
     if (nkb > 0) {
         const __amdgpu_buffer_rsrc_t ra = __builtin_amdgcn_make_buffer_rsrc((void*)G.A, 0, (int)((long)G.B * G.lda * 4), 0x00020000);
         const __amdgpu_buffer_rsrc_t rb = __builtin_amdgcn_make_buffer_rsrc((void*)G.E, 0, (int)((long)G.V * 256), 0x00020000);
@@ -368,6 +446,7 @@
             };
 #pragma unroll
             for (int u = 0; u < STAGES; ++u) issue(u);
+            fold_row();
             for (int kb = 0; kb < nkb16; kb += STAGES) {
 #pragma unroll
                 for (int u = 0; u < STAGES; ++u) {
@@ -375,6 +454,10 @@
                     f32x4 x0 = sa[u][0], x1 = sa[u][1];
 #pragma unroll
                     for (int e = 0; e < 4; ++e) {
+                        if constexpr (FOLD) {
+                            x0[e] = head_g(x0[e], lse, ccol + e == ans, true, inv_b);
+                            x1[e] = head_g(x1[e], lse, ccol + 4 + e == ans, true, inv_b);
+                        }
                         if (ccol + e >= kend) x0[e] = 0.f;
                         if (ccol + 4 + e >= kend) x1[e] = 0.f;
                     }
@@ -405,13 +488,16 @@
         };
 #pragma unroll
         for (int u = 0; u < STAGES; ++u) issue(u);
+        fold_row();
         for (int kb = 0; kb < nkb; kb += STAGES) {
 #pragma unroll
             for (int u = 0; u < STAGES; ++u) {
                 if (kb + u >= nkb) break;
 #pragma unroll
                 for (int s = 0; s < 4; ++s) {
-                    const float a = ccol + s < kend ? sa[u][s] : 0.f;
+                    float a = sa[u][s];
+                    if constexpr (FOLD) a = head_g(a, lse, ccol + s == ans, true, inv_b);
+                    a = ccol + s < kend ? a : 0.f;
                     const f32x2 b = sb[u][s];
                     acc0 = __builtin_amdgcn_mfma_f32_32x32x2f32(a, b.x, acc0, 0, 0, 0);
                     acc1 = __builtin_amdgcn_mfma_f32_32x32x2f32(a, b.y, acc1, 0, 0, 0);
@@ -432,23 +518,35 @@
     }
 }
 
-template <bool BFH>
+template <bool BFH, bool FOLD = false>
 __global__ void __launch_bounds__(256)
-logits_bwd_direct_kernel(const DwProblem Q, int tiles, const DhP H) {
+logits_bwd_direct_kernel(const DwProblem Q, int tiles, const DhP H, const HeadFoldP F) {
     __shared__ __attribute__((aligned(16))) float red[4][66][64];
-    if ((int)blockIdx.x < tiles) dw_wg_body<4, false, BFH>(Q, 64 * (int)blockIdx.x, 0, 0, red);
-    else dh_wave_body<4, BFH>(H, (int)blockIdx.x - tiles);
-}
-
-struct LogitsP { const float* H; long ldh; const float* E; float* C; int B, V, Vp; };
+    __shared__ f32x2 tab[FOLD ? HEAD_TAB_ROWS : 1];
+    if ((int)blockIdx.x < tiles) dw_wg_body<4, false, BFH, FOLD>(Q, 64 * (int)blockIdx.x, 0, 0, red, tab, &F);
+    else dh_wave_body<4, BFH, FOLD>(H, (int)blockIdx.x - tiles, &F);
+}
+
+struct LogitsP { const float* H; long ldh; const float* E; float* C; int B, V, Vp; float* stats; };
+template <bool STATS>
 __global__ void __launch_bounds__(256)
 logits_direct_kernel(const LogitsP G) {
     const int wv = __builtin_amdgcn_readfirstlane((int)(threadIdx.x >> 6));
     const int lane = threadIdx.x & 63, l31 = lane & 31, half = lane >> 5;
     const int ntile = (G.Vp + 31) >> 5, mtiles = (G.B + 31) >> 5;
-    const int unit = blockIdx.x * 4 + wv;
-    const int nt = unit % ntile, mt = unit / ntile;
-    if (mt >= mtiles) return;
+    int nt, mt;
+    bool active = true;
+    if constexpr (STATS) {
+        const int ngroup = (ntile + 3) >> 2;
+        mt = blockIdx.x / ngroup;
+        nt = (blockIdx.x % ngroup) * 4 + wv;
+        active = nt < ntile;
+        nt = min(nt, ntile - 1);
+    } else {
+        const int unit = blockIdx.x * 4 + wv;
+        nt = unit % ntile; mt = unit / ntile;
+        if (mt >= mtiles) return;
+    }
     const int m = min(32 * mt + l31, G.B - 1);
     const int v = min(32 * nt + l31, G.V - 1);
     const float* ap = G.H + (long)m * G.ldh + 32 * half;
@@ -466,11 +564,47 @@
 #pragma unroll
         for (int j = 0; j < 4; ++j) acc = __builtin_amdgcn_mfma_f32_32x32x2f32(a[i][j], b[i][j], acc, 0, 0, 0);
     const int col = 32 * nt + l31;
+    const bool real = col < G.V;
+    if constexpr (STATS) {
+        __shared__ f32x2 part[4][32];
+        float mo = -INFINITY, so = 0.f;
+#pragma unroll
+        for (int r = 0; r < 16; ++r) {
+            const float x = real ? acc[r] : -INFINITY;
+            const float mr = group_max<32>(x);
+            const float sr = group_sum<32>(expf(x - mr));
+            if (rho(r) + 4 * half == l31) { mo = mr; so = sr; }
+        }
+        if (((l31 >> 2) & 1) == half) part[wv][l31] = active ? f32x2{mo, so} : f32x2{-INFINITY, 0.f};
+        __syncthreads();
+        if (threadIdx.x < 32) {
+            const f32x2 v[4] = {part[0][l31], part[1][l31], part[2][l31], part[3][l31]};
+            float M, S;
+            head_merge<4>(v, 4, M, S);
+            gst2(G.stats + ((long)blockIdx.x * 32 + l31) * 2, f32x2{M, S});
+        }
+        if (!active) return;
+    }
     if (col >= G.Vp) return;
-    const bool real = col < G.V;
 #pragma unroll
     for (int r = 0; r < 16; ++r) {
         const int row = 32 * mt + rho(r) + 4 * half;
         if (row < G.B) gst(G.C + (long)row * G.Vp + col, real ? acc[r] : 0.f);
     }
 }
+
+__global__ void __launch_bounds__(256)
+ce_rows_stats_kernel(const HeadFoldP F, float* __restrict__ dlogits) {
+    const int b = blockIdx.x;
+    const float lse = head_row_lse(F.stats, F.ngroup, b);
+    const int ans = head_answer(F.answers, b, F.V);
+    const float* row = F.logits + (long)b * F.ld;
+    for (int v = 4 * (int)threadIdx.x; v < (int)F.ld; v += 1024) {
+        const f32x4 x = gld4(row + v);
+        f32x4 g;
+#pragma unroll
+        for (int j = 0; j < 4; ++j) g[j] = head_g(x[j], lse, v + j == ans, v + j < F.V, F.inv_b);
+        *reinterpret_cast<f32x4*>(dlogits + (long)b * F.ld + v) = g;
+    }
+    if (threadIdx.x == 0) gst(F.loss_rows + b, lse - row[ans]);
+}
diff --git a/include/bsarec_hip.h b/include/bsarec_hip.h
--- a/include/bsarec_hip.h
+++ b/include/bsarec_hip.h
@@ -39,6 +39,7 @@
     int train_sampler;
     int train_no_logq;
     int train_lazy_adam;
+    int separate_ce;
     int weight_image;
 } bsarec_config_t;
 
```

After: 1.695 million. 1.4% lower.
